# eltoto1219/vltk

Measured on AMD Instinct MI355X. Metric: images/sec FRCNN feature extraction, 800x1333 batch, higher is better.
Workload: dtype f16; 1 GPU; configs[1]: ResNet-101-C4 fp16 (the reference has no FPN: SURVEY.md D1), 32 synthetic 800x1333 images per GPU per step, R=300 RPN proposals through the Res5 head, max 100 detections/img, seeded synthetic weights; global_batch=32, parallelism=image-sharded x1, all-gather of output blocks

## Files before the change

include/vltk_hip.h:

```cpp
#ifndef VLTK_HIP_H
#define VLTK_HIP_H

#include <stddef.h>
#include <stdint.h>

#ifdef __cplusplus
extern "C" {
#endif

#define VK_OK 0
#define VK_EINVAL 1
#define VK_ENOTIMPL 2
#define VK_ENONFINITE 3
#define VK_EWEIGHTS 4
#define VK_EHIP 5
#define VK_ENOMEM 6

typedef enum { VK_F32 = 0, VK_F16 = 1, VK_I64 = 2, VK_I32 = 3, VK_BF16 = 4 } vk_dtype;
typedef enum { VK_ACT_NONE = 0, VK_ACT_RELU = 1, VK_ACT_GELU = 2 , VK_ACT_TANH = 3 } vk_act;

#define VK_MAX_ANCHOR_DIM 8
#define VK_MAX_NMS_THRESH 8

typedef struct vk_config {
    int32_t depth;
    int32_t num_groups;
    int32_t width_per_group;
    int32_t stem_out_channels;
    int32_t res2_out_channels;
    int32_t stride_in_1x1;
    int32_t caffe_maxpool;
    int32_t num_sizes;
    float   sizes[VK_MAX_ANCHOR_DIM];
    int32_t num_ratios;
    float   ratios[VK_MAX_ANCHOR_DIM];
    float   anchor_offset;
    int32_t rpn_hidden_channels;
    float   rpn_min_size;
    double  rpn_nms_thresh;
    int32_t pre_nms_topk;
    int32_t post_nms_topk;
    float   rpn_bbox_weights[4];
    int32_t num_classes;
    int32_t num_attrs;
    int32_t use_attr;
    int32_t pooler_resolution;
    int32_t res5_halve;
    int32_t cls_agnostic_bbox_reg;
    float   roi_bbox_weights[4];
    int32_t precision;
} vk_config;

typedef struct vk_roi_params {
    int32_t num_nms_thresh;
    double  nms_thresh[VK_MAX_NMS_THRESH];
    int32_t min_detections;
    int32_t max_detections;
} vk_roi_params;

#define VK_SELECT_CLASS_MAX 0
#define VK_SELECT_PER_CLASS 1
typedef struct vk_select_params {
    int32_t       mode;
    double        score_thresh;
    vk_roi_params roi;
} vk_select_params;

typedef struct vk_outputs {
    int64_t *obj_ids;
    float   *obj_probs;
    int64_t *attr_ids;
    float   *attr_probs;
    float   *boxes;
    int64_t *preds_per_image;
    float   *roi_features;
} vk_outputs;

#define VK_MAX_IGNOREY 64
typedef struct vk_ignorey {
    const void    *bands;
    const int32_t *counts;
    int32_t        max_per_image;
    int32_t        f64;
} vk_ignorey;

typedef struct vk_handle vk_handle;

const char *vk_last_error(void);
int vk_version(void);

int vk_create(const vk_config *cfg, int device, vk_handle **out);
int vk_load_weights(vk_handle *h, const char *name, const void *host_ptr,
                    const int64_t *shape, int ndim, vk_dtype dtype);
int vk_finalize(vk_handle *h);
int vk_destroy(vk_handle *h);

int vk_set_option(vk_handle *h, const char *key, int value);

int vk_num_weights(vk_handle *h, int *count);
int vk_weight_name(vk_handle *h, int index, const char **name);

int vk_forward(vk_handle *h, const float *images_dev, int N, int H, int W,
               const int32_t *image_hw, const float *scales_yx,
               const vk_roi_params *rp, const vk_outputs *out_dev, void *stream);

int vk_forward_begin(vk_handle *h, const float *images_dev, int N, int H, int W,
                     const int32_t *image_hw, const float *scales_yx,
                     const vk_roi_params *rp, const vk_outputs *out_dev, void *stream, int64_t *ticket);
int vk_forward_end(vk_handle *h, int64_t ticket);
int vk_forward_begin_ignorey(vk_handle *h, const float *images_dev, int N, int H, int W,
                             const int32_t *image_hw, const float *scales_yx,
                             const vk_roi_params *rp, const vk_outputs *out_dev, void *stream, int64_t *ticket,
                             const vk_ignorey *ignorey);
int vk_forward_begin_select(vk_handle *h, const float *images_dev, int N, int H, int W,
                            const int32_t *image_hw, const float *scales_yx,
                            const vk_select_params *sp, const vk_outputs *out_dev, void *stream, int64_t *ticket,
                            const vk_ignorey *ignorey);

int vk_forward_boxes_begin(vk_handle *h, const float *images_dev, int N, int H, int W,
                           const int32_t *image_hw, const float *scales_yx,
                           const float *boxes_dev, int B, const int32_t *counts,
                           const vk_outputs *out_dev, void *stream, int64_t *ticket);

int vk_given_boxes_ingest(const float *boxes_dev, const int32_t *counts_dev, const int32_t *image_hw_dev,
                          const float *scales_yx_dev, int N, int B, float *prop_boxes, float *rois, int32_t *levels,
                          int min_level, int max_level, float canonical_box_size, int canonical_level, int32_t *nonfinite,
                          void *stream);
int vk_given_box_outputs(const float *obj_prob, const int32_t *obj_cls, const float *attr_prob, const int32_t *attr_cls,
                         const float *prop_boxes, const int32_t *counts_dev, const float *scales_yx_dev, const float *feat,
                         int F, int N, int B, const vk_outputs *out_dev, void *stream);

int vk_get_stage(vk_handle *h, const char *name, const void **dev_ptr,
                 vk_dtype *dtype, int64_t *shape, int *ndim);

int vk_memcpy_d2d(void *dst_dev, const void *src_dev, size_t bytes, void *stream);

int vk_enable_stage_timing(vk_handle *h, int enable);
int vk_get_stage_timing(vk_handle *h, float *ms6);

#define VK_NUM_KERNEL_BUCKETS 12
int vk_enable_kernel_timing(vk_handle *h, int enable);
int vk_get_kernel_timing(vk_handle *h, int64_t *launches, double *ms, double *flops, double *bytes, int reset);


size_t vk_packed_weight_bytes(int cout, int cin, int kh, int kw, int groups, vk_dtype dt);
int vk_packed_cout(int cout);
int vk_conv_slice_channels(int cin, int groups);
int vk_pack_conv_weight(const float *w_oihw_host, const float *bn_host, const float *bias_host,
                        int cout, int cin, int kh, int kw, int groups, vk_dtype dt,
                        void *w_packed_host, float *bias_packed_host);

int vk_conv2d(const void *x, int N, int H, int W, int cin,
              const void *w_packed, const float *bias_packed, const void *residual,
              void *y, int cout, int ldy, int kh, int kw, int stride, int pad, int dil, int groups,
              int relu, vk_dtype dt, vk_dtype out_dt, void *stream);

#define VK_ROUTE_GENERIC 0
#define VK_ROUTE_RING 1
#define VK_ROUTE_DUO 2
#define VK_ROUTE_WS 3
#define VK_ROUTE_GEMM4 4
#define VK_ROUTE_PANEL 5
#define VK_ROUTE_BLK 6
int vk_conv_route(int N, int H, int W, int cin, int cin2, int has_residual, int fused_mean, int cout, int ldy, int kh, int kw,
                  int stride, int pad, int dil, int groups, int relu, vk_dtype dt, vk_dtype out_dt);

int vk_conv1x1_dual(const void *x1, int cin1, const void *x2, int cin2, long M,
                    const void *w_packed, const float *bias_packed, const void *residual,
                    void *y, int cout, int relu, void *stream);

int vk_bottleneck64(const void *x, int N, int H, int W, int cin, int proj,
                    const void *w1_packed, const float *b1_packed, const void *w2_packed, const float *b2_packed,
                    const void *w3_packed, const float *b3_packed, void *y, void *stream);

int vk_fuse_shortcut(int cin, int cin_shortcut, int cout, int stride, vk_dtype dt);
int vk_bottleneck64_eligible(int cin, int cmid, int cout, int stride, int dil, int groups, int proj, int fused_shortcut,
                             long N, int H, int W, vk_dtype dt);

size_t vk_conv1x1_meanpool_workspace_bytes(int N, int HW, int cout);
int vk_conv1x1_meanpool(const void *x, int N, int HW, int cin, const void *w_packed, const float *bias_packed,
                        const void *residual, int cout, int relu, float *out_mean,
                        void *workspace, size_t workspace_bytes, void *stream);


int vk_linear(const void *x, long M, int K, const void *w_packed, const float *bias_packed, const void *residual,
              void *y, int N, int ldy, int act, vk_dtype dt, vk_dtype out_dt, void *stream);
int vk_layernorm(const void *x, int ldx, const float *gamma, const float *beta, void *y, int ldy, int M, int C,
                 float eps, float scale, int accumulate, vk_dtype dt, void *stream);
int vk_embed_layernorm(const int64_t *input_ids, const int64_t *token_type_ids, int B, int L, const void *word,
                       const void *position, const void *token_type, const float *gamma, const float *beta,
                       void *y, int C, float eps, vk_dtype dt, void *stream);
int vk_attention(const void *q, int ldq, const void *k, int ldk, const void *v, int ldv, const float *mask,
                 void *out, int ldo, int B, int heads, int Lq, int Lk, int d, vk_dtype dt, void *stream);


int vk_roi_align(const void *const *maps, const int32_t *Hs, const int32_t *Ws, const float *scales, int levels,
                 int N, int C, const float *rois, const int32_t *roi_levels, int K, int P, int sampling_ratio,
                 int aligned, void *out, vk_dtype dt, void *stream);
int vk_assign_levels(const float *boxes, int ld, int K, int min_level, int max_level, float canonical_box_size,
                     int canonical_level, int32_t *levels_out, void *stream);
int vk_upsample2x_add(const void *lateral, const void *top, void *y, int N, int H, int W, int Ht, int Wt, int C,
                      vk_dtype dt, void *stream);
int vk_subsample2(const void *x, void *y, int N, int H, int W, int C, vk_dtype dt, void *stream);
int vk_relu_copy(const void *x, void *y, long n, vk_dtype dt, void *stream);

size_t vk_rpn_multilevel_workspace_bytes(int N, int levels, int pre_topk, int post_topk);
int vk_rpn_proposals_multilevel_ignorey(const float *const *logits, const int32_t *ld_logits, const float *const *deltas,
                                        const int32_t *ld_deltas, int levels, int N, const int32_t *Hs, const int32_t *Ws,
                                        int A, const float *const *cell_anchors, const int32_t *strides, float offset,
                                        const int32_t *image_hw, const float *bbox_weights4_host, float min_size,
                                        double nms_thresh, int pre_topk, int post_topk, float *out_boxes,
                                        float *out_logits, int32_t *out_counts, int32_t *nonfinite_flag, void *workspace,
                                        size_t workspace_bytes, void *stream, const vk_ignorey *ignorey);
int vk_rpn_proposals_ignorey(const float *logits, int ld_logits, const float *deltas, int ld_deltas,
                             int N, int Hf, int Wf, int A, const float *cell_anchors, int stride, float offset,
                             const int32_t *image_hw, const float *bbox_weights4_host, float min_size,
                             double nms_thresh, int pre_topk, int post_topk,
                             float *out_boxes, float *out_logits, int32_t *out_counts, int32_t *nonfinite_flag,
                             void *workspace, size_t workspace_bytes, void *stream, const vk_ignorey *ignorey);
int vk_rpn_proposals_multilevel(const float *const *logits, const int32_t *ld_logits, const float *const *deltas,
                                const int32_t *ld_deltas, int levels, int N, const int32_t *Hs, const int32_t *Ws, int A,
                                const float *const *cell_anchors, const int32_t *strides, float offset,
                                const int32_t *image_hw, const float *bbox_weights4_host, float min_size,
                                double nms_thresh, int pre_topk, int post_topk, float *out_boxes, float *out_logits,
                                int32_t *out_counts, int32_t *nonfinite_flag, void *workspace, size_t workspace_bytes,
                                void *stream);

int vk_nchw_to_nhwc(const float *x, int N, int C, int H, int W, void *y, vk_dtype dt, void *stream);
int vk_nhwc_to_nchw(const void *x, int N, int C, int H, int W, float *y, vk_dtype dt, void *stream);

size_t vk_packed_stem_bytes(int cout, vk_dtype dt);
int vk_pack_stem_weight(const float *w_oihw_host, const float *bn_host, int cout, vk_dtype dt,
                        void *w_packed_host, float *bias_packed_host);
int vk_stem(const float *x, int N, int H, int W, const void *w_packed, const float *bias_packed,
            int cout, int caffe_maxpool, void *y, vk_dtype dt, void *workspace, size_t workspace_bytes,
            void *stream);
size_t vk_stem_workspace_bytes(int N, int H, int W, int cout, vk_dtype dt);
void vk_stem_out_hw(int H, int W, int caffe_maxpool, int *Ho, int *Wo);

int vk_preprocess(const float *const *raw_dev_ptrs_host, const int32_t *raw_hw_host, const int32_t *new_hw_host,
                  int N, int Hmax, int Wmax, const float *mean3_host, const float *std3_host, float pad_value,
                  float *out_nchw_dev, void *stream);

int vk_maxpool3x3s2(const void *x, int N, int H, int W, int C, int caffe, void *y, vk_dtype dt, void *stream);

size_t vk_rpn_workspace_bytes(int N, int HWA, int pre_topk);
int vk_rpn_proposals(const float *logits, int ld_logits, const float *deltas, int ld_deltas,
                     int N, int Hf, int Wf, int A, const float *cell_anchors, int stride, float offset,
                     const int32_t *image_hw, const float *bbox_weights4_host, float min_size,
                     double nms_thresh, int pre_topk, int post_topk,
                     float *out_boxes, float *out_logits, int32_t *out_counts, int32_t *nonfinite_flag,
                     void *workspace, size_t workspace_bytes, void *stream);

int vk_nms(const float *boxes, const float *scores, int n, double thresh,
           int64_t *keep_out, int32_t *count_out, void *workspace, size_t workspace_bytes, void *stream);
size_t vk_nms_workspace_bytes(int n);

int vk_roi_pool(const void *feat, int N, int H, int W, int C, const float *rois, int K,
                float spatial_scale, int P, void *out, vk_dtype dt, void *stream);

int vk_mean_pool(const void *x, int K, int S, int C, float *out, vk_dtype dt, void *stream);

int vk_box_decode(const float *deltas, const float *boxes, int M, int k, const float *weights4_host,
                  float *out, void *stream);

int vk_make_rois(const float *boxes, int N, int R, float *rois, void *stream);
int vk_softmax_argmax(const float *logits, int ld, int K, int n_softmax, int n_argmax, float *prob_out,
                      int32_t *cls_out, int32_t *raw_argmax_out, void *stream);
int vk_concat_embed(const float *features, int F, const void *emb, int E, const int32_t *cls, int K, void *out,
                    vk_dtype dt, void *stream);
int vk_chosen_deltas(const void *x, int ldx, const void *w_rows, const float *bias, const int32_t *cls,
                     int cls_agnostic, int F, int K, float *out, vk_dtype dt, void *stream);

int vk_roi_outputs(const float *obj_logits, int ld_obj, const float *attr_logits, int ld_attr,
                   const float *box_deltas, int ld_box, int chosen_only,
                   const float *proposals, const int32_t *counts, const float *features, int F,
                   int N, int R, int C, int A, const int32_t *image_hw, const float *scales_yx_dev,
                   const float *weights4_host, const vk_roi_params *rp, const vk_outputs *out,
                   int64_t *keep_ids_out, int32_t *nonfinite_flag, void *stream);

int vk_class_boxes(const float *box_deltas, int ld_box, int cls_agnostic, const float *proposals, const int32_t *counts,
                   int N, int R, int C, const int32_t *image_hw, const float *weights4_host, float *out,
                   int32_t *nonfinite_flag, void *stream);
int vk_class_probs(const float *logits, int ld, int K, int n, float *out, int ld_out, void *stream);
int vk_per_class_select(const float *obj_scores, int ld_scores, const float *attr_logits, int ld_attr,
                        const float *box_deltas, int ld_box, int cls_agnostic,
                        const float *proposals, const int32_t *counts, const float *features, int F,
                        int N, int R, int C, int A, const int32_t *image_hw, const float *scales_yx_dev,
                        const float *weights4_host, const vk_select_params *sp, const vk_outputs *out,
                        int64_t *keep_ids_out, float *max_conf_out, int32_t *nonfinite_flag, void *stream);

#ifdef __cplusplus
}
#endif
#endif
```

vltk_amd/_lib.py:

```python
import ctypes as C
import os

_HERE = os.path.dirname(os.path.abspath(__file__))
LIB_PATH = os.path.join(_HERE, "libvltk_hip.so")
if os.environ.get("VLTK_AMD_LIB"):
    LIB_PATH = os.environ["VLTK_AMD_LIB"]
elif os.environ.get("VLTK_AMD_ABLATION_LIB") == "1":
    LIB_PATH = LIB_PATH.replace("libvltk_hip.so", "libvltk_hip_ablation.so")

VK_OK, VK_EINVAL, VK_ENOTIMPL, VK_ENONFINITE, VK_EWEIGHTS, VK_EHIP, VK_ENOMEM = range(7)
VK_F32, VK_F16, VK_I64, VK_I32, VK_BF16 = 0, 1, 2, 3, 4
VK_ACT_NONE, VK_ACT_RELU, VK_ACT_GELU, VK_ACT_TANH = 0, 1, 2, 3
VK_ROUTE_GENERIC, VK_ROUTE_RING, VK_ROUTE_DUO, VK_ROUTE_WS, VK_ROUTE_GEMM4, VK_ROUTE_PANEL, VK_ROUTE_BLK = range(7)
VK_MAX_ANCHOR_DIM = 8
VK_MAX_NMS_THRESH = 8
VK_MAX_IGNOREY = 64
VK_SELECT_CLASS_MAX, VK_SELECT_PER_CLASS = 0, 1

_EXC = {
    VK_EINVAL: ValueError,
    VK_ENOTIMPL: NotImplementedError,
    VK_ENONFINITE: AssertionError,
    VK_EWEIGHTS: OSError,
    VK_EHIP: RuntimeError,
    VK_ENOMEM: MemoryError,
}


class vk_config(C.Structure):
    _fields_ = [
        ("depth", C.c_int32), ("num_groups", C.c_int32), ("width_per_group", C.c_int32),
        ("stem_out_channels", C.c_int32), ("res2_out_channels", C.c_int32),
        ("stride_in_1x1", C.c_int32), ("caffe_maxpool", C.c_int32),
        ("num_sizes", C.c_int32), ("sizes", C.c_float * VK_MAX_ANCHOR_DIM),
        ("num_ratios", C.c_int32), ("ratios", C.c_float * VK_MAX_ANCHOR_DIM),
        ("anchor_offset", C.c_float), ("rpn_hidden_channels", C.c_int32),
        ("rpn_min_size", C.c_float), ("rpn_nms_thresh", C.c_double),
        ("pre_nms_topk", C.c_int32), ("post_nms_topk", C.c_int32),
        ("rpn_bbox_weights", C.c_float * 4),
        ("num_classes", C.c_int32), ("num_attrs", C.c_int32), ("use_attr", C.c_int32),
        ("pooler_resolution", C.c_int32), ("res5_halve", C.c_int32),
        ("cls_agnostic_bbox_reg", C.c_int32), ("roi_bbox_weights", C.c_float * 4),
        ("precision", C.c_int32),
    ]


class vk_roi_params(C.Structure):
    _fields_ = [
        ("num_nms_thresh", C.c_int32), ("nms_thresh", C.c_double * VK_MAX_NMS_THRESH),
        ("min_detections", C.c_int32), ("max_detections", C.c_int32),
    ]


class vk_select_params(C.Structure):
    _fields_ = [("mode", C.c_int32), ("score_thresh", C.c_double), ("roi", vk_roi_params)]


class vk_outputs(C.Structure):
    _fields_ = [
        ("obj_ids", C.c_void_p), ("obj_probs", C.c_void_p), ("attr_ids", C.c_void_p),
        ("attr_probs", C.c_void_p), ("boxes", C.c_void_p), ("preds_per_image", C.c_void_p),
        ("roi_features", C.c_void_p),
    ]


class vk_ignorey(C.Structure):
    _fields_ = [("bands", C.c_void_p), ("counts", C.c_void_p), ("max_per_image", C.c_int32), ("f64", C.c_int32)]


_P, _I, _F, _D, _SZ = C.c_void_p, C.c_int, C.c_float, C.c_double, C.c_size_t

SIGNATURES = {
    "vk_last_error": (C.c_char_p, []),
    "vk_version": (_I, []),
    "vk_create": (_I, [C.POINTER(vk_config), _I, C.POINTER(_P)]),
    "vk_load_weights": (_I, [_P, C.c_char_p, _P, C.POINTER(C.c_int64), _I, _I]),
    "vk_finalize": (_I, [_P]),
    "vk_destroy": (_I, [_P]),
    "vk_set_option": (_I, [_P, C.c_char_p, _I]),
    "vk_num_weights": (_I, [_P, C.POINTER(_I)]),
    "vk_weight_name": (_I, [_P, _I, C.POINTER(C.c_char_p)]),
    "vk_forward": (_I, [_P, _P, _I, _I, _I, _P, _P, C.POINTER(vk_roi_params), C.POINTER(vk_outputs), _P]),
    "vk_forward_begin": (_I, [_P, _P, _I, _I, _I, _P, _P, C.POINTER(vk_roi_params), C.POINTER(vk_outputs), _P,
                              C.POINTER(C.c_int64)]),
    "vk_forward_begin_ignorey": (_I, [_P, _P, _I, _I, _I, _P, _P, C.POINTER(vk_roi_params), C.POINTER(vk_outputs), _P,
                                      C.POINTER(C.c_int64), C.POINTER(vk_ignorey)]),
    "vk_forward_begin_select": (_I, [_P, _P, _I, _I, _I, _P, _P, C.POINTER(vk_select_params), C.POINTER(vk_outputs), _P,
                                     C.POINTER(C.c_int64), C.POINTER(vk_ignorey)]),
    "vk_forward_boxes_begin": (_I, [_P, _P, _I, _I, _I, _P, _P, _P, _I, _P, C.POINTER(vk_outputs), _P, C.POINTER(C.c_int64)]),
    "vk_forward_end": (_I, [_P, C.c_int64]),
    "vk_given_boxes_ingest": (_I, [_P, _P, _P, _P, _I, _I, _P, _P, _P, _I, _I, _F, _I, _P, _P]),
    "vk_given_box_outputs": (_I, [_P, _P, _P, _P, _P, _P, _P, _P, _I, _I, _I, C.POINTER(vk_outputs), _P]),
    "vk_get_stage": (_I, [_P, C.c_char_p, C.POINTER(_P), C.POINTER(_I), C.POINTER(C.c_int64), C.POINTER(_I)]),
    "vk_memcpy_d2d": (_I, [_P, _P, _SZ, _P]),
    "vk_enable_stage_timing": (_I, [_P, _I]),
    "vk_get_stage_timing": (_I, [_P, C.POINTER(_F)]),
    "vk_enable_kernel_timing": (_I, [_P, _I]),
    "vk_get_kernel_timing": (_I, [_P, C.POINTER(C.c_int64), C.POINTER(_D), C.POINTER(_D), C.POINTER(_D), _I]),
    "vk_packed_weight_bytes": (_SZ, [_I, _I, _I, _I, _I, _I]),
    "vk_conv_slice_channels": (_I, [_I, _I]),
    "vk_packed_cout": (_I, [_I]),
    "vk_pack_conv_weight": (_I, [_P, _P, _P, _I, _I, _I, _I, _I, _I, _P, _P]),
    "vk_conv_route": (_I, [_I] * 18),
    "vk_conv1x1_dual": (_I, [_P, _I, _P, _I, C.c_long, _P, _P, _P, _P, _I, _I, _P]),
    "vk_bottleneck64": (_I, [_P, _I, _I, _I, _I, _I, _P, _P, _P, _P, _P, _P, _P, _P]),
    "vk_fuse_shortcut": (_I, [_I, _I, _I, _I, _I]),
    "vk_bottleneck64_eligible": (_I, [_I, _I, _I, _I, _I, _I, _I, _I, C.c_long, _I, _I, _I]),
    "vk_conv1x1_meanpool_workspace_bytes": (_SZ, [_I, _I, _I]),
    "vk_conv1x1_meanpool": (_I, [_P, _I, _I, _I, _P, _P, _P, _I, _I, _P, _P, _SZ, _P]),
    "vk_linear": (_I, [_P, C.c_long, _I, _P, _P, _P, _P, _I, _I, _I, _I, _I, _P]),
    "vk_layernorm": (_I, [_P, _I, _P, _P, _P, _I, _I, _I, _F, _F, _I, _I, _P]),
    "vk_embed_layernorm": (_I, [_P, _P, _I, _I, _P, _P, _P, _P, _P, _P, _I, _F, _I, _P]),
    "vk_attention": (_I, [_P, _I, _P, _I, _P, _I, _P, _P, _I, _I, _I, _I, _I, _I, _I, _P]),
    "vk_roi_align": (_I, [_P, _P, _P, _P, _I, _I, _I, _P, _P, _I, _I, _I, _I, _P, _I, _P]),
    "vk_assign_levels": (_I, [_P, _I, _I, _I, _I, _F, _I, _P, _P]),
    "vk_upsample2x_add": (_I, [_P, _P, _P, _I, _I, _I, _I, _I, _I, _I, _P]),
    "vk_subsample2": (_I, [_P, _P, _I, _I, _I, _I, _I, _P]),
    "vk_relu_copy": (_I, [_P, _P, C.c_long, _I, _P]),
    "vk_rpn_multilevel_workspace_bytes": (_SZ, [_I, _I, _I, _I]),
    "vk_rpn_proposals_multilevel": (_I, [_P, _P, _P, _P, _I, _I, _P, _P, _I, _P, _P, _F, _P, _P, _F, _D, _I, _I, _P, _P, _P, _P, _P, _SZ, _P]),
    "vk_rpn_proposals_multilevel_ignorey": (_I, [_P, _P, _P, _P, _I, _I, _P, _P, _I, _P, _P, _F, _P, _P, _F, _D, _I, _I, _P, _P, _P, _P,
                                                 _P, _SZ, _P, C.POINTER(vk_ignorey)]),
    "vk_conv2d": (_I, [_P, _I, _I, _I, _I, _P, _P, _P, _P, _I, _I, _I, _I, _I, _I, _I, _I, _I, _I, _I, _P]),
    "vk_nchw_to_nhwc": (_I, [_P, _I, _I, _I, _I, _P, _I, _P]),
    "vk_nhwc_to_nchw": (_I, [_P, _I, _I, _I, _I, _P, _I, _P]),
    "vk_packed_stem_bytes": (_SZ, [_I, _I]),
    "vk_pack_stem_weight": (_I, [_P, _P, _I, _I, _P, _P]),
    "vk_stem": (_I, [_P, _I, _I, _I, _P, _P, _I, _I, _P, _I, _P, _SZ, _P]),
    "vk_stem_workspace_bytes": (_SZ, [_I, _I, _I, _I, _I]),
    "vk_stem_out_hw": (None, [_I, _I, _I, C.POINTER(_I), C.POINTER(_I)]),
    "vk_preprocess": (_I, [_P, _P, _P, _I, _I, _I, C.POINTER(_F), C.POINTER(_F), _F, _P, _P]),
    "vk_maxpool3x3s2": (_I, [_P, _I, _I, _I, _I, _I, _P, _I, _P]),
    "vk_rpn_workspace_bytes": (_SZ, [_I, _I, _I]),
    "vk_rpn_proposals": (_I, [_P, _I, _P, _I, _I, _I, _I, _I, _P, _I, _F, _P, C.POINTER(_F), _F, _D, _I, _I,
                              _P, _P, _P, _P, _P, _SZ, _P]),
    "vk_rpn_proposals_ignorey": (_I, [_P, _I, _P, _I, _I, _I, _I, _I, _P, _I, _F, _P, C.POINTER(_F), _F, _D, _I, _I,
                                      _P, _P, _P, _P, _P, _SZ, _P, C.POINTER(vk_ignorey)]),
    "vk_nms": (_I, [_P, _P, _I, _D, _P, _P, _P, _SZ, _P]),
    "vk_nms_workspace_bytes": (_SZ, [_I]),
    "vk_roi_pool": (_I, [_P, _I, _I, _I, _I, _P, _I, _F, _I, _P, _I, _P]),
    "vk_mean_pool": (_I, [_P, _I, _I, _I, _P, _I, _P]),
    "vk_box_decode": (_I, [_P, _P, _I, _I, C.POINTER(_F), _P, _P]),
    "vk_make_rois": (_I, [_P, _I, _I, _P, _P]),
    "vk_softmax_argmax": (_I, [_P, _I, _I, _I, _I, _P, _P, _P, _P]),
    "vk_concat_embed": (_I, [_P, _I, _P, _I, _P, _I, _P, _I, _P]),
    "vk_chosen_deltas": (_I, [_P, _I, _P, _P, _P, _I, _I, _I, _P, _I, _P]),
    "vk_roi_outputs": (_I, [_P, _I, _P, _I, _P, _I, _I, _P, _P, _P, _I, _I, _I, _I, _I, _P, _P, C.POINTER(_F),
                            C.POINTER(vk_roi_params), C.POINTER(vk_outputs), _P, _P, _P]),
    "vk_class_boxes": (_I, [_P, _I, _I, _P, _P, _I, _I, _I, _P, C.POINTER(_F), _P, _P, _P]),
    "vk_class_probs": (_I, [_P, _I, _I, _I, _P, _I, _P]),
    "vk_per_class_select": (_I, [_P, _I, _P, _I, _P, _I, _I, _P, _P, _P, _I, _I, _I, _I, _I, _P, _P, C.POINTER(_F),
                                 C.POINTER(vk_select_params), C.POINTER(vk_outputs), _P, _P, _P, _P]),
}

_lib = None


def load():
    global _lib
    if _lib is None:
        if not os.path.exists(LIB_PATH):
            raise RuntimeError(
                f"{LIB_PATH} not found: build it with `python -c 'import __graft_entry__ as g; g.build()'` "
                "(or `make -C vltk_amd/csrc`).  vltk_amd has no CPU fallback.")
        lib = C.CDLL(LIB_PATH)
        for name, (res, args) in SIGNATURES.items():
            fn = getattr(lib, name)
            fn.restype = res
            fn.argtypes = args
        _lib = lib
    return _lib


def check(status):
    if status != VK_OK:
        msg = load().vk_last_error().decode("utf-8", "replace")
        raise _EXC.get(status, RuntimeError)(msg)


def call(name, *args):
    check(getattr(load(), name)(*args))
```

vltk_amd/csrc/model.hip:

```cpp
#include <cmath>
#include <cstdlib>
#include <map>
#include <mutex>
#include <set>
#include <string>
#include <vector>

#include "vk_common.h"

namespace vk {

thread_local KernelTimer *g_timer = nullptr;

hipEvent_t KernelTimer::get() {
    if (pool.empty()) {
        hipEvent_t e = nullptr;
        (void)hipEventCreate(&e);
        all.push_back(e);
        return e;
    }
    hipEvent_t e = pool.back();
    pool.pop_back();
    return e;
}
void KernelTimer::collect() {
    const char *logp = getenv("VK_CONV_LOG");
    FILE *lf = logp ? fopen(logp, "a") : nullptr;
    std::vector<Rec> pending;
    for (auto &r : recs) {
        float t = 0.f;
        if (hipEventQuery(r.e1) != hipSuccess) {
            pending.push_back(r);
            continue;
        }
        if (hipEventElapsedTime(&t, r.e0, r.e1) == hipSuccess) {
            if (lf) fprintf(lf, "%d %d %d %d %d %d %.5f %.1f\n", r.bucket, r.M, r.cout, r.cin, r.k, r.stride, t, r.flops / (t * 1e-3) / 1e12);
            launches[r.bucket] += 1;
            ms[r.bucket] += t;
            flops[r.bucket] += r.flops;
            bytes[r.bucket] += r.bytes;
        }
        pool.push_back(r.e0);
        pool.push_back(r.e1);
    }
    if (lf) fclose(lf);
    recs.swap(pending);
    (void)hipGetLastError();
}
KernelTimer::~KernelTimer() {
    for (auto e : all) (void)hipEventDestroy(e);
}

int Timed::begin(hipStream_t stream) {
    if (!tm) return VK_OK;
    e0 = tm->get();
    e1 = tm->get();
    VK_CHECK_HIP(hipEventRecord(e0, stream));
    return VK_OK;
}
int Timed::end(hipStream_t stream, int bucket, double flops, int M, int cout, int cin, int k, int stride, double bytes) {
    if (!tm) return VK_OK;
    VK_CHECK_HIP(hipEventRecord(e1, stream));
    tm->recs.push_back({bucket, flops, e0, e1, M, cout, cin, k, stride, bytes});
    return VK_OK;
}

static std::atomic<DeviceState *> g_devices[VK_MAX_DEVICES];
static std::mutex g_devices_mu;

int device_state(DeviceState **out) {
    int dev = 0;
    VK_CHECK_HIP(hipGetDevice(&dev));
    VK_REQUIRE(dev >= 0 && dev < VK_MAX_DEVICES, VK_EINVAL, "device %d beyond VK_MAX_DEVICES", dev);
    DeviceState *d = g_devices[dev].load(std::memory_order_acquire);
    if (!d) {
        std::lock_guard<std::mutex> lock(g_devices_mu);
        d = g_devices[dev].load(std::memory_order_relaxed);
        if (!d) {
            hipDeviceProp_t prop;
            VK_CHECK_HIP(hipGetDeviceProperties(&prop, dev));
            char *p = nullptr;
            VK_CHECK_HIP(hipMalloc((void **)&p, 256 + 256 * sizeof(unsigned) + BN_TRASH_BYTES));
            VK_CHECK_HIP(hipMemset(p, 0, 256 + 256 * sizeof(unsigned)));
            d = new DeviceState;
            d->n_cu = prop.multiProcessorCount;
            d->zero_page = p;
            d->tile_ring = (unsigned *)(p + 256);
            d->bn_trash = p + 256 + 256 * sizeof(unsigned);
            d->tile_next = 0;
            g_devices[dev].store(d, std::memory_order_release);
        }
    }
    *out = d;
    return VK_OK;
}

static std::set<std::pair<int, const void *>> g_lds_set;
static std::mutex g_lds_mu;

int set_max_lds(const void *kernel, size_t bytes) {
    int dev = 0;
    VK_CHECK_HIP(hipGetDevice(&dev));
    std::lock_guard<std::mutex> lock(g_lds_mu);
    if (g_lds_set.count({dev, kernel})) return VK_OK;
    VK_CHECK_HIP(hipFuncSetAttribute(kernel, hipFuncAttributeMaxDynamicSharedMemorySize, (int)bytes));
    g_lds_set.insert({dev, kernel});
    return VK_OK;
}

static thread_local char g_err[1024] = "";
void set_error(const char *fmt, ...) {
    va_list ap;
    va_start(ap, fmt);
    vsnprintf(g_err, sizeof(g_err), fmt, ap);
    va_end(ap);
}

struct HostTensor {
    std::vector<int64_t> shape;
    std::vector<float> data;
    bool loaded = false;
};

struct ConvLayer {
    std::string prefix;
    int cin = 0, cout = 0, k = 1, stride = 1, pad = 0, dil = 1;
    bool bn = true, relu = false;
    void *w = nullptr;
    float *b = nullptr;
    int groups = 1;
    int dt = -1;
};

struct Block {
    ConvLayer conv1, conv2, conv3, shortcut;
    bool has_shortcut = false;
    bool fused_shortcut = false;
};

static const int kBlocks[3][4] = {{3, 4, 6, 3}, {3, 4, 23, 3}, {3, 8, 36, 3}};

}

using namespace vk;

struct vk_handle {
    vk_config cfg;
    int device = 0;
    vk_dtype dt = VK_F16;
    vk_dtype pdt = VK_F32;
    bool finalized = false;
    std::vector<std::string> names;
    std::map<std::string, HostTensor> host;

    ConvLayer stem;
    std::vector<Block> stages[3];
    std::vector<Block> res5;
    ConvLayer rpn_conv, rpn_heads;
    ConvLayer cls_score, fc_attr, attr_score;
    void *bbox_w = nullptr;
    float *bbox_b = nullptr;
    void *emb = nullptr;
    float *cell_anchors = nullptr;
    int A = 0, res4_c = 0, res5_c = 0, hid = 0, emb_dim = 0;
    std::vector<void *> owned;

    char *arena = nullptr;
    size_t arena_bytes = 0;
    char *pc_arena = nullptr;
    size_t pc_arena_bytes = 0;
    const void *bbox_lin_w = nullptr;
    const float *bbox_lin_b = nullptr;
    int head_chunk = 9600;
    int backbone_streams = 2;
    int backbone_split_min_batch = 8;
    int head_streams = 1;
    int head_split_min_rois = 512;

    struct Stage {
        const void *ptr;
        vk_dtype dt;
        int64_t shape[4];
        int ndim;
    };
    std::map<std::string, Stage> stages_out;
    KernelTimer *ktimer = nullptr;
    bool timing = false;
    hipEvent_t ev[6] = {nullptr, nullptr, nullptr, nullptr, nullptr, nullptr};
    hipStream_t side = nullptr;
    hipEvent_t ev_fork = nullptr, ev_join = nullptr;
    hipStream_t more_sides[2] = {nullptr, nullptr};
    hipEvent_t more_joins[2] = {nullptr, nullptr};
    bool ev_valid = false;
    static constexpr int VK_MAX_INFLIGHT = 4;
    int32_t *flag_host = nullptr;
    char *meta_host = nullptr;
    size_t meta_cap = 0;
    hipEvent_t ev_done[VK_MAX_INFLIGHT] = {nullptr, nullptr, nullptr, nullptr};
    int64_t next_ticket = 0, oldest_open = 0;
};

namespace vk {

static void add_conv_names(std::vector<std::string> &n, const std::string &p, bool bn) {
    n.push_back(p + ".weight");
    if (bn) {
        n.push_back(p + ".norm.weight");
        n.push_back(p + ".norm.bias");
        n.push_back(p + ".norm.running_mean");
        n.push_back(p + ".norm.running_var");
    } else {
        n.push_back(p + ".bias");
    }
}

static Block make_block(const std::string &p, int cin, int cmid, int cout, int stride, int dil, bool stride_in_1x1,
                        int groups, std::vector<std::string> &names) {
    Block b;
    const int s1 = stride_in_1x1 ? stride : 1, s3 = stride_in_1x1 ? 1 : stride;
    b.has_shortcut = cin != cout;
    if (b.has_shortcut) {
        b.shortcut = ConvLayer{p + ".shortcut", cin, cout, 1, stride, 0, 1, true, false};
        add_conv_names(names, b.shortcut.prefix, true);
    }
    b.conv1 = ConvLayer{p + ".conv1", cin, cmid, 1, s1, 0, 1, true, true};
    b.conv2 = ConvLayer{p + ".conv2", cmid, cmid, 3, s3, dil, dil, true, true};
    b.conv2.groups = groups;
    b.conv3 = ConvLayer{p + ".conv3", cmid, cout, 1, 1, 0, 1, true, true};
    add_conv_names(names, b.conv1.prefix, true);
    add_conv_names(names, b.conv2.prefix, true);
    add_conv_names(names, b.conv3.prefix, true);
    return b;
}

static int dev_alloc(vk_handle *h, size_t bytes, void **out) {
    void *p = nullptr;
    VK_CHECK_HIP(hipMalloc(&p, bytes ? bytes : 16));
    h->owned.push_back(p);
    *out = p;
    return VK_OK;
}

static int upload(vk_handle *h, const void *host, size_t bytes, void **out) {
    VK_TRY(dev_alloc(h, bytes, out));
    VK_CHECK_HIP(hipMemcpy(*out, host, bytes, hipMemcpyHostToDevice));
    return VK_OK;
}

static const HostTensor *get_t(vk_handle *h, const std::string &name, std::vector<int64_t> shape) {
    auto it = h->host.find(name);
    if (it == h->host.end() || !it->second.loaded) {
        set_error("missing weight '%s' (strict load)", name.c_str());
        return nullptr;
    }
    if (it->second.shape != shape) {
        std::string got, want;
        for (auto v : it->second.shape) got += std::to_string(v) + ",";
        for (auto v : shape) want += std::to_string(v) + ",";
        set_error("weight '%s' has shape [%s], expected [%s]", name.c_str(), got.c_str(), want.c_str());
        return nullptr;
    }
    return &it->second;
}

static int finalize_conv(vk_handle *h, ConvLayer &L) {
    const HostTensor *w = get_t(h, L.prefix + ".weight", {L.cout, L.cin / L.groups, L.k, L.k});
    if (!w) return VK_EWEIGHTS;
    std::vector<float> bn;
    const float *bnp = nullptr, *bias = nullptr;
    if (L.bn) {
        const char *parts[4] = {".norm.weight", ".norm.bias", ".norm.running_mean", ".norm.running_var"};
        bn.resize(4 * (size_t)L.cout);
        for (int i = 0; i < 4; ++i) {
            const HostTensor *t = get_t(h, L.prefix + parts[i], {L.cout});
            if (!t) return VK_EWEIGHTS;
            memcpy(bn.data() + (size_t)i * L.cout, t->data.data(), sizeof(float) * L.cout);
        }
        bnp = bn.data();
    } else {
        const HostTensor *t = get_t(h, L.prefix + ".bias", {L.cout});
        if (!t) return VK_EWEIGHTS;
        bias = t->data.data();
    }
    const vk_dtype ldt = L.dt >= 0 ? (vk_dtype)L.dt : h->dt;
    const size_t wb = vk_packed_weight_bytes(L.cout, L.cin, L.k, L.k, L.groups, ldt);
    std::vector<char> packed(wb);
    std::vector<float> pb(vk_packed_cout(L.cout));
    VK_TRY(vk_pack_conv_weight(w->data.data(), bnp, bias, L.cout, L.cin, L.k, L.k, L.groups, ldt, packed.data(), pb.data()));
    VK_TRY(upload(h, packed.data(), wb, &L.w));
    VK_TRY(upload(h, pb.data(), pb.size() * sizeof(float), (void **)&L.b));
    return VK_OK;
}

static int pack_conv_host(vk_handle *h, const ConvLayer &L, std::vector<char> &packed, std::vector<float> &pb) {
    const HostTensor *w = get_t(h, L.prefix + ".weight", {L.cout, L.cin / L.groups, L.k, L.k});
    if (!w) return VK_EWEIGHTS;
    std::vector<float> bn(4 * (size_t)L.cout);
    const char *parts[4] = {".norm.weight", ".norm.bias", ".norm.running_mean", ".norm.running_var"};
    for (int i = 0; i < 4; ++i) {
        const HostTensor *t = get_t(h, L.prefix + parts[i], {L.cout});
        if (!t) return VK_EWEIGHTS;
        memcpy(bn.data() + (size_t)i * L.cout, t->data.data(), sizeof(float) * L.cout);
    }
    packed.resize(vk_packed_weight_bytes(L.cout, L.cin, L.k, L.k, L.groups, h->dt));
    pb.resize(vk_packed_cout(L.cout));
    return vk_pack_conv_weight(w->data.data(), bn.data(), nullptr, L.cout, L.cin, L.k, L.k, L.groups, h->dt, packed.data(), pb.data());
}

static int finalize_block(vk_handle *h, Block &b) {
    VK_TRY(finalize_conv(h, b.conv1));
    VK_TRY(finalize_conv(h, b.conv2));
    b.fused_shortcut = b.has_shortcut && vk_fuse_shortcut(b.conv3.cin, b.shortcut.cin, b.conv3.cout, b.shortcut.stride, h->dt);
    if (!b.fused_shortcut) {
        if (b.has_shortcut) VK_TRY(finalize_conv(h, b.shortcut));
        return finalize_conv(h, b.conv3);
    }
    std::vector<char> w3, wsc;
    std::vector<float> b3, bsc;
    VK_TRY(pack_conv_host(h, b.conv3, w3, b3));
    VK_TRY(pack_conv_host(h, b.shortcut, wsc, bsc));
    const size_t r3 = (size_t)b.conv3.cin * 2, rsc = (size_t)b.shortcut.cin * 2, rows = b3.size();
    std::vector<char> cat(rows * (r3 + rsc));
    for (size_t r = 0; r < rows; ++r) {
        memcpy(cat.data() + r * (r3 + rsc), w3.data() + r * r3, r3);
        memcpy(cat.data() + r * (r3 + rsc) + r3, wsc.data() + r * rsc, rsc);
        b3[r] += bsc[r];
    }
    VK_TRY(upload(h, cat.data(), cat.size(), &b.conv3.w));
    VK_TRY(upload(h, b3.data(), b3.size() * sizeof(float), (void **)&b.conv3.b));
    return VK_OK;
}

static void to_dt(const float *src, size_t n, vk_dtype dt, void *dst) {
    if (dt == VK_F16) {
        _Float16 *d = (_Float16 *)dst;
        for (size_t i = 0; i < n; ++i) d[i] = (_Float16)src[i];
    } else if (dt == VK_BF16) {
        uint16_t *d = (uint16_t *)dst;
        for (size_t i = 0; i < n; ++i) {
            uint32_t u;
            memcpy(&u, &src[i], 4);
            if ((u & 0x7fffffffu) > 0x7f800000u)
                d[i] = (uint16_t)((u >> 16) | 0x40);
            else
                d[i] = (uint16_t)((u + 0x7fffu + ((u >> 16) & 1u)) >> 16);
        }
    } else {
        memcpy(dst, src, n * sizeof(float));
    }
}

static bool fused_mean_ok(const vk_handle *h, int P, size_t rows) {
    static const bool off = getenv("VK_NO_FUSED_MEAN") != nullptr;
    const long mid5 = (long)h->cfg.num_groups * h->cfg.width_per_group * 8;
    return !off && h->dt == VK_F16 && h->cfg.res5_halve == 0 && P * P >= 128 && P * P <= 255 && h->res5_c % 256 == 0 &&
           (long)rows * mid5 * 2 < (1L << 32);
}

struct Carver {
    char *base;
    size_t off = 0;
    explicit Carver(char *b) : base(b) {}
    void *take(size_t bytes) {
        void *p = base ? base + off : nullptr;
        off += align_up(bytes ? bytes : 16, 256);
        return p;
    }
};

struct Plan {
    int N, H, W, Hp, Wp, H1, W1, Hs[3], Ws[3], Hf, Wf, R, K, P, chunk;
    void *img_pad, *stem_out, *bufA, *bufB, *bufSC, *bufT1, *bufT2;
    void *rpn_hid;
    float *rpn_out, *prop_boxes, *prop_logits, *rois;
    int32_t *prop_counts, *image_hw, *nonfinite;
    float *scales;
    void *bands;
    int32_t *band_counts;
    void *rpn_ws;
    size_t rpn_ws_bytes;
    void *pooled, *h_t1, *h_t2, *h_a, *h_b, *h_sc;
    float *pool_part;
    float *feat;
    void *featT, *concat, *attr_hid;
    float *cls_logits, *attr_logits, *obj_prob, *attr_prob, *chosen;
    int32_t *obj_cls, *attr_cls, *max_class;
    int64_t *keep_ids;
    size_t total;
};

static void conv_out_hw(int H, int W, int k, int s, int p, int d, int *Ho, int *Wo) {
    *Ho = (H + 2 * p - (d * (k - 1) + 1)) / s + 1;
    *Wo = (W + 2 * p - (d * (k - 1) + 1)) / s + 1;
}

static Plan make_plan(vk_handle *h, char *base, int N, int H, int W, int D, int R) {
    Plan p;
    memset(&p, 0, sizeof(p));
    const vk_config &c = h->cfg;
    const size_t es = dtype_size(h->dt);
    p.N = N;
    p.H = H;
    p.W = W;
    conv_out_hw(H, W, 7, 2, 3, 1, &p.H1, &p.W1);
    p.Hp = std::max(H + 6, 2 * p.H1 + 6);
    p.Wp = std::max(W + 6, 2 * p.W1 + 6);
    p.Wp = (p.Wp + 1) & ~1;
    int h2, w2;
    vk_stem_out_hw(H, W, c.caffe_maxpool, &h2, &w2);
    p.Hs[0] = h2;
    p.Ws[0] = w2;
    for (int s = 1; s < 3; ++s) conv_out_hw(p.Hs[s - 1], p.Ws[s - 1], 1, 2, 0, 1, &p.Hs[s], &p.Ws[s]);
    p.Hf = p.Hs[2];
    p.Wf = p.Ws[2];
    p.R = R;
    p.K = N * p.R;
    p.P = c.pooler_resolution;
    p.chunk = std::min(h->head_chunk > 0 ? h->head_chunk : p.K, p.K);

    Carver cv(base);
    p.img_pad = cv.take((size_t)N * p.Hp * p.Wp * 4 * es);
    p.stem_out = cv.take((size_t)N * p.H1 * p.W1 * c.stem_out_channels * es);
    size_t max_out = 0, max_mid = 0;
    int cout = c.res2_out_channels, cmid = c.num_groups * c.width_per_group;
    for (int s = 0; s < 3; ++s) {
        const size_t px_out = (size_t)N * p.Hs[s] * p.Ws[s];
        const size_t px_in = s == 0 ? px_out : (size_t)N * p.Hs[s - 1] * p.Ws[s - 1];
        max_out = std::max(max_out, px_out * cout * es);
        max_mid = std::max(max_mid, (c.stride_in_1x1 ? px_out : px_in) * cmid * es);
        cout *= 2;
        cmid *= 2;
    }
    p.bufA = cv.take(max_out);
    p.bufB = cv.take(max_out);
    p.bufSC = cv.take(max_out);
    p.bufT1 = cv.take(max_mid);
    p.bufT2 = cv.take(max_mid);
    const size_t Mf = (size_t)N * p.Hf * p.Wf;
    p.rpn_hid = cv.take(Mf * h->hid * es);
    p.rpn_out = (float *)cv.take(Mf * (size_t)((5 * h->A + 7) / 8 * 8) * sizeof(float));
    p.prop_boxes = (float *)cv.take((size_t)p.K * 4 * sizeof(float));
    p.prop_logits = (float *)cv.take((size_t)p.K * sizeof(float));
    p.rois = (float *)cv.take((size_t)p.K * 5 * sizeof(float));
    p.prop_counts = (int32_t *)cv.take((size_t)N * sizeof(int32_t));
    p.image_hw = (int32_t *)cv.take((size_t)N * 2 * sizeof(int32_t));
    p.scales = (float *)cv.take((size_t)N * 2 * sizeof(float));
    p.nonfinite = (int32_t *)cv.take(sizeof(int32_t));
    p.rpn_ws_bytes = vk_rpn_workspace_bytes(N, p.Hf * p.Wf * h->A, c.pre_nms_topk);
    p.rpn_ws = cv.take(p.rpn_ws_bytes);
    const size_t rows = (size_t)p.chunk * p.P * p.P;
    const int mid5 = c.num_groups * c.width_per_group * 8;
    p.pooled = cv.take(rows * h->res4_c * es);
    p.h_t1 = cv.take(rows * mid5 * es);
    p.h_t2 = cv.take(rows * mid5 * es);
    p.h_a = cv.take(rows * h->res5_c * es);
    p.h_b = cv.take(rows * h->res5_c * es);
    p.h_sc = cv.take(rows * h->res5_c * es);
    p.pool_part = nullptr;
    if (fused_mean_ok(h, p.P, rows)) p.pool_part = (float *)cv.take(conv_duo_pool_part_bytes((long)rows + 128, h->res5_c));
    p.feat = (float *)cv.take((size_t)p.K * h->res5_c * sizeof(float));
    const size_t pes = dtype_size(h->pdt);
    p.featT = cv.take((size_t)p.K * h->res5_c * pes);
    p.concat = cv.take((size_t)p.K * (h->res5_c + h->emb_dim) * pes);
    p.attr_hid = cv.take((size_t)p.K * (h->res5_c / 4) * pes);
    p.cls_logits = (float *)cv.take((size_t)p.K * ((c.num_classes + 1 + 7) / 8 * 8) * sizeof(float));
    p.attr_logits = (float *)cv.take((size_t)p.K * ((c.num_attrs + 1 + 7) / 8 * 8) * sizeof(float));
    p.obj_prob = (float *)cv.take((size_t)p.K * sizeof(float));
    p.attr_prob = (float *)cv.take((size_t)p.K * sizeof(float));
    p.chosen = (float *)cv.take((size_t)p.K * 4 * sizeof(float));
    p.obj_cls = (int32_t *)cv.take((size_t)p.K * sizeof(int32_t));
    p.attr_cls = (int32_t *)cv.take((size_t)p.K * sizeof(int32_t));
    p.max_class = (int32_t *)cv.take((size_t)p.K * sizeof(int32_t));
    p.keep_ids = (int64_t *)cv.take((size_t)N * D * sizeof(int64_t));
    p.bands = cv.take((size_t)N * VK_MAX_IGNOREY * 2 * sizeof(double));
    p.band_counts = (int32_t *)cv.take((size_t)N * sizeof(int32_t));
    p.total = cv.off;
    return p;
}

static int run_conv(vk_handle *h, const ConvLayer &L, const void *x, int N, int H, int W, const void *res, void *y,
                    bool relu, vk_dtype out_dt, int ldy, hipStream_t s, int *Ho = nullptr, int *Wo = nullptr,
                    const void *x2 = nullptr, int cin2 = 0, float *pool_part = nullptr, bool concurrent = false) {
    ConvArgs a;
    memset(&a, 0, sizeof(a));
    a.concurrent = concurrent ? 1 : 0;
    a.x = x;
    a.x2 = x2;
    a.Cin2 = cin2;
    a.pool_part = pool_part;
    a.w = L.w;
    a.bias = L.b;
    a.res = res;
    a.y = y;
    a.N = N;
    a.H = H;
    a.W = W;
    a.Cin = L.cin;
    conv_out_hw(H, W, L.k, L.stride, L.pad, L.dil, &a.Ho, &a.Wo);
    a.Cout = L.cout;
    a.ldy = ldy > 0 ? ldy : (L.cout + 7) / 8 * 8;
    a.kh = a.kw = L.k;
    a.stride = L.stride;
    a.pad = L.pad;
    a.dil = L.dil;
    a.groups = L.groups;
    a.relu = relu;
    a.stem = 0;
    a.dt = L.dt >= 0 ? (vk_dtype)L.dt : h->dt;
    a.out_dt = out_dt;
    if (Ho) *Ho = a.Ho;
    if (Wo) *Wo = a.Wo;
    return launch_conv(a, s);
}

static int run_block(vk_handle *h, const Block &b, const void *x, int N, int H, int W, void *t1, void *t2, void *sc,
                     void *y, hipStream_t s, int *Ho, int *Wo, float *pool_part = nullptr, int n0 = 0, int nb = -1) {
    int h1, w1, h2, w2;
    const bool cc = nb >= 0;
    if (nb >= 0) {
        const size_t es = dtype_size(h->dt);
        int ho, wo;
        conv_out_hw(H, W, b.conv1.k, b.conv1.stride, b.conv1.pad, b.conv1.dil, &h1, &w1);
        conv_out_hw(h1, w1, b.conv2.k, b.conv2.stride, b.conv2.pad, b.conv2.dil, &h2, &w2);
        conv_out_hw(h2, w2, 1, 1, 0, 1, &ho, &wo);
        x = (const char *)x + (size_t)n0 * H * W * b.conv1.cin * es;
        t1 = (char *)t1 + (size_t)n0 * h1 * w1 * b.conv1.cout * es;
        t2 = (char *)t2 + (size_t)n0 * h2 * w2 * b.conv2.cout * es;
        sc = (char *)sc + (size_t)n0 * ho * wo * b.conv3.cout * es;
        y = (char *)y + (size_t)n0 * ho * wo * b.conv3.cout * es;
        N = nb;
    }
    if (!pool_part && vk_bottleneck64_eligible(b.conv1.cin, b.conv1.cout, b.conv3.cout, b.conv1.stride * b.conv2.stride, b.conv2.dil,
                                               b.conv2.groups, b.has_shortcut, b.fused_shortcut, N, H, W, h->dt)) {
        if (Ho) *Ho = H;
        if (Wo) *Wo = W;
        return launch_bneck_fused(x, N, H, W, b.conv1.cin, b.has_shortcut, b.conv1.w, b.conv1.b, b.conv2.w, b.conv2.b, b.conv3.w, b.conv3.b, y,
                                  cc, s);
    }
    const void *res = x;
    if (b.has_shortcut && !b.fused_shortcut) {
        VK_TRY(run_conv(h, b.shortcut, x, N, H, W, nullptr, sc, false, h->dt, 0, s, nullptr, nullptr, nullptr, 0, nullptr, cc));
        res = sc;
    }
    VK_TRY(run_conv(h, b.conv1, x, N, H, W, nullptr, t1, true, h->dt, 0, s, &h1, &w1, nullptr, 0, nullptr, cc));
    VK_TRY(run_conv(h, b.conv2, t1, N, h1, w1, nullptr, t2, true, h->dt, 0, s, &h2, &w2, nullptr, 0, nullptr, cc));
    if (b.fused_shortcut)
        return run_conv(h, b.conv3, t2, N, h2, w2, nullptr, y, true, h->dt, 0, s, Ho, Wo, x, b.shortcut.cin, pool_part, cc);
    VK_TRY(run_conv(h, b.conv3, t2, N, h2, w2, res, y, true, h->dt, 0, s, Ho, Wo, nullptr, 0, pool_part, cc));
    return VK_OK;
}

static void set_stage(vk_handle *h, const char *name, const void *ptr, vk_dtype dt, std::initializer_list<int64_t> shape) {
    vk_handle::Stage st;
    st.ptr = ptr;
    st.dt = dt;
    st.ndim = 0;
    for (auto v : shape) st.shape[st.ndim++] = v;
    h->stages_out[name] = st;
}

}

extern "C" {

const char *vk_last_error(void) { return g_err; }
int vk_version(void) { return 1; }

int vk_packed_cout(int cout) { return (cout + CONV_COUT_ALIGN - 1) / CONV_COUT_ALIGN * CONV_COUT_ALIGN; }

int vk_conv_slice_channels(int cin, int groups) {
    if (groups <= 1) return cin;
    if (cin <= 0 || cin % groups != 0) return -1;
    const int cpg = cin / groups;
    if (cpg & (cpg - 1)) return -1;
    return std::min(std::max(cpg, 64), cin);
}

size_t vk_packed_weight_bytes(int cout, int cin, int kh, int kw, int groups, vk_dtype dt) {
    const int sw = vk_conv_slice_channels(cin, groups);
    return sw <= 0 ? 0 : (size_t)vk_packed_cout(cout) * kh * kw * sw * dtype_size(dt);
}

int vk_pack_conv_weight(const float *w, const float *bn, const float *bias, int cout, int cin, int kh, int kw, int groups,
                        vk_dtype dt, void *w_packed, float *bias_packed) {
    VK_REQUIRE(dt == VK_F16 || dt == VK_F32 || dt == VK_BF16, VK_EINVAL, "pack: dtype must be f16, bf16 or f32");
    VK_REQUIRE(groups >= 1, VK_EINVAL, "pack: groups=%d", groups);
    const int sw = vk_conv_slice_channels(cin, groups);
    VK_REQUIRE(sw > 0, VK_EINVAL, "pack: cin=%d / groups=%d must be a power of two", cin, groups);
    VK_REQUIRE(groups == 1 || cin == cout, VK_EINVAL, "pack: grouped convolution needs cin == cout (got %d, %d)", cin, cout);
    VK_REQUIRE((sw * (int)dtype_size(dt)) % CONV_KTILE_BYTES == 0, VK_EINVAL,
               "pack: %d channels per tap is not a whole number of 128-byte K-tiles for this dtype", sw);
    const int cp = vk_packed_cout(cout);
    const int cpg = cin / groups;
    const size_t K = (size_t)kh * kw * sw;
    std::vector<float> row(K);
    for (int co = 0; co < cp; ++co) {
        double s = 1.0;
        float b = 0.f;
        std::fill(row.begin(), row.end(), 0.f);
        if (co < cout) {
            if (bn) {
                const double g = bn[co], be = bn[cout + co], mu = bn[2 * (size_t)cout + co], var = bn[3 * (size_t)cout + co];
                s = g / std::sqrt(var + 1e-5);
                b = (float)(be - mu * s);
            } else if (bias) {
                b = bias[co];
            }
            const int slice0 = groups == 1 ? 0 : (co / 64 * 64) / sw * sw;
            const int g0 = groups == 1 ? 0 : co / cpg * cpg;
            for (int c = 0; c < cpg; ++c)
                for (int y = 0; y < kh; ++y)
                    for (int x = 0; x < kw; ++x)
                        row[((size_t)y * kw + x) * sw + (g0 + c - slice0)] =
                            (float)((double)w[(((size_t)co * cpg + c) * kh + y) * kw + x] * s);
        }
        bias_packed[co] = b;
        to_dt(row.data(), K, dt, (char *)w_packed + (size_t)co * K * dtype_size(dt));
    }
    return VK_OK;
}

size_t vk_packed_stem_bytes(int cout, vk_dtype dt) {
    const int ktiles = dt == VK_F16 ? 4 : 7;
    return (size_t)vk_packed_cout(cout) * ktiles * CONV_KTILE_BYTES;
}

int vk_pack_stem_weight(const float *w, const float *bn, int cout, vk_dtype dt, void *w_packed, float *bias_packed) {
    VK_REQUIRE(dt == VK_F16 || dt == VK_F32, VK_EINVAL, "pack_stem: dtype must be f16 or f32");
    const int cp = vk_packed_cout(cout);
    const int ktiles = dt == VK_F16 ? 4 : 7;
    const size_t K = (size_t)ktiles * CONV_KTILE_BYTES / dtype_size(dt);
    std::vector<float> row(K);
    for (int co = 0; co < cp; ++co) {
        std::fill(row.begin(), row.end(), 0.f);
        float b = 0.f;
        if (co < cout) {
            double s = 1.0;
            if (bn) {
                const double g = bn[co], be = bn[cout + co], mu = bn[2 * (size_t)cout + co], var = bn[3 * (size_t)cout + co];
                s = g / std::sqrt(var + 1e-5);
                b = (float)(be - mu * s);
            }
            for (int c = 0; c < 3; ++c)
                for (int y = 0; y < 7; ++y)
                    for (int x = 0; x < 7; ++x)
                        row[(size_t)y * 32 + x * 4 + c] = (float)((double)w[(((size_t)co * 3 + c) * 7 + y) * 7 + x] * s);
        }
        bias_packed[co] = b;
        to_dt(row.data(), K, dt, (char *)w_packed + (size_t)co * K * dtype_size(dt));
    }
    return VK_OK;
}

static void fill_conv_args(ConvArgs &a, int N, int H, int W, int cin, int cout, int ldy, int k, int stride, int pad, int dil, int groups,
                           int relu, vk_dtype dt, vk_dtype out_dt) {
    memset(&a, 0, sizeof(a));
    a.N = N;
    a.H = H;
    a.W = W;
    a.Cin = cin;
    conv_out_hw(H, W, k, stride, pad, dil, &a.Ho, &a.Wo);
    a.Cout = cout;
    a.ldy = ldy;
    a.kh = a.kw = k;
    a.stride = stride;
    a.pad = pad;
    a.dil = dil;
    a.groups = groups;
    a.relu = relu;
    a.dt = dt;
    a.out_dt = out_dt;
}

int vk_conv2d(const void *x, int N, int H, int W, int cin, const void *w_packed, const float *bias_packed,
              const void *residual, void *y, int cout, int ldy, int kh, int kw, int stride, int pad, int dil, int groups,
              int relu, vk_dtype dt, vk_dtype out_dt, void *stream) {
    VK_REQUIRE(kh == kw && kh >= 1 && stride >= 1 && dil >= 1 && pad >= 0 && groups >= 1, VK_EINVAL, "conv2d: bad geometry");
    ConvArgs a;
    fill_conv_args(a, N, H, W, cin, cout, ldy, kh, stride, pad, dil, groups, relu, dt, out_dt);
    VK_REQUIRE(a.Ho > 0 && a.Wo > 0 && N > 0, VK_EINVAL, "conv2d: empty output");
    a.x = x;
    a.w = w_packed;
    a.bias = bias_packed;
    a.res = residual;
    a.y = y;
    return launch_conv(a, (hipStream_t)stream);
}

int vk_conv_route(int N, int H, int W, int cin, int cin2, int has_residual, int fused_mean, int cout, int ldy, int kh, int kw,
                  int stride, int pad, int dil, int groups, int relu, vk_dtype dt, vk_dtype out_dt) {
    if (!(kh == kw && kh >= 1 && stride >= 1 && dil >= 1 && pad >= 0 && groups >= 1 && cin2 >= 0)) {
        set_error("conv_route: bad geometry");
        return -VK_EINVAL;
    }
    static const char here = 0;
    ConvArgs a;
    fill_conv_args(a, N, H, W, cin, cout, ldy, kh, stride, pad, dil, groups, relu, dt, out_dt);
    if (!(a.Ho > 0 && a.Wo > 0 && N > 0)) {
        set_error("conv_route: empty output");
        return -VK_EINVAL;
    }
    a.x = a.w = &here;
    a.res = has_residual ? &here : nullptr;
    a.x2 = cin2 > 0 ? &here : nullptr;
    a.Cin2 = cin2;
    a.pool_part = fused_mean ? (float *)&here : nullptr;
    return conv_route_checked(a);
}

int vk_conv1x1_dual(const void *x1, int cin1, const void *x2, int cin2, long M, const void *w_packed, const float *bias_packed,
                    const void *residual, void *y, int cout, int relu, void *stream) {
    VK_REQUIRE(x1 && x2 && M > 0 && M < (1L << 31), VK_EINVAL, "conv1x1_dual: bad arguments");
    ConvArgs a;
    fill_conv_args(a, 1, 1, (int)M, cin1, cout, cout, 1, 1, 0, 1, 1, relu, VK_F16, VK_F16);
    a.x = x1;
    a.x2 = x2;
    a.Cin2 = cin2;
    a.w = w_packed;
    a.bias = bias_packed;
    a.res = residual;
    a.y = y;
    return launch_conv(a, (hipStream_t)stream);
}

int vk_linear(const void *x, long M, int K, const void *w_packed, const float *bias_packed, const void *residual, void *y, int N, int ldy,
              int act, vk_dtype dt, vk_dtype out_dt, void *stream) {
    VK_REQUIRE(x && w_packed && bias_packed && y && M > 0 && M < (1L << 31), VK_EINVAL, "linear: bad arguments");
    ConvArgs a;
    fill_conv_args(a, 1, 1, (int)M, K, N, ldy, 1, 1, 0, 1, 1, act, dt, out_dt);
    a.x = x;
    a.w = w_packed;
    a.bias = bias_packed;
    a.res = residual;
    a.y = y;
    return launch_conv(a, (hipStream_t)stream);
}

int vk_fuse_shortcut(int cin, int cin_shortcut, int cout, int stride, vk_dtype dt) {
    static const bool off = getenv("VK_NO_FUSED_SHORTCUT") != nullptr;
    return !off && dt == VK_F16 && stride == 1 && cout % 256 == 0 && cin % 32 == 0 && cin_shortcut % 32 == 0;
}

int vk_bottleneck64_eligible(int cin, int cmid, int cout, int stride, int dil, int groups, int proj, int fused_shortcut, long N,
                             int H, int W, vk_dtype dt) {
    return stride == 1 && dil == 1 && (!proj || fused_shortcut) &&
           bneck_fused_eligible(cin, cmid, cout, stride, groups, proj != 0, N, H, W, dt);
}

int vk_bottleneck64(const void *x, int N, int H, int W, int cin, int proj, const void *w1, const float *b1, const void *w2,
                    const float *b2, const void *w3, const float *b3, void *y, void *stream) {
    VK_REQUIRE(x && w1 && b1 && w2 && b2 && w3 && b3 && y && N > 0 && H > 0 && W > 0, VK_EINVAL, "bottleneck64: bad arguments");
    VK_REQUIRE((cin == 256 && !proj) || (cin == 64 && proj), VK_EINVAL, "bottleneck64: cin must be 256 (identity) or 64 (projection)");
    VK_REQUIRE(bneck_fused_eligible(cin, 64, 256, 1, 1, proj != 0, N, H, W, VK_F16) || getenv("VK_BNECK_FUSED"), VK_EINVAL,
               "bottleneck64: tensor beyond the 32-bit byte offsets");
    VK_REQUIRE((long)N * H * W * 512 < (1L << 32) - (1L << 20), VK_EINVAL, "bottleneck64: tensor beyond the 32-bit byte offsets");
    return launch_bneck_fused(x, N, H, W, cin, proj != 0, w1, b1, w2, b2, w3, b3, y, false, (hipStream_t)stream);
}

size_t vk_conv1x1_meanpool_workspace_bytes(int N, int HW, int cout) { return conv_duo_pool_part_bytes((long)N * HW, cout); }

int vk_conv1x1_meanpool(const void *x, int N, int HW, int cin, const void *w_packed, const float *bias_packed,
                        const void *residual, int cout, int relu, float *out_mean, void *workspace, size_t workspace_bytes,
                        void *stream) {
    VK_REQUIRE(x && out_mean && workspace && N > 0 && HW > 0, VK_EINVAL, "conv1x1_meanpool: bad arguments");
    VK_REQUIRE(workspace_bytes >= vk_conv1x1_meanpool_workspace_bytes(N, HW, cout), VK_EINVAL, "conv1x1_meanpool: workspace too small");
    ConvArgs a;
    fill_conv_args(a, N, 1, HW, cin, cout, cout, 1, 1, 0, 1, 1, relu, VK_F16, VK_F16);
    a.x = x;
    a.w = w_packed;
    a.bias = bias_packed;
    a.res = residual;
    a.pool_part = (float *)workspace;
    VK_TRY(launch_conv(a, (hipStream_t)stream));
    return launch_pool_finish((const float *)workspace, N, HW, cin, cout, false, out_mean, (hipStream_t)stream);
}

static void stem_geom(int H, int W, int *H1, int *W1, int *Hp, int *Wp) {
    conv_out_hw(H, W, 7, 2, 3, 1, H1, W1);
    *Hp = std::max(H + 6, 2 * *H1 + 6);
    *Wp = (std::max(W + 6, 2 * *W1 + 6) + 1) & ~1;
}

size_t vk_stem_workspace_bytes(int N, int H, int W, int cout, vk_dtype dt) {
    int H1, W1, Hp, Wp;
    stem_geom(H, W, &H1, &W1, &Hp, &Wp);
    return align_up((size_t)N * Hp * Wp * 4 * dtype_size(dt), 256) + align_up((size_t)N * H1 * W1 * cout * dtype_size(dt), 256);
}

static int stem_impl(const float *x, int N, int H, int W, const void *w, const float *b, int cout, int caffe, void *y,
                     vk_dtype dt, void *img_pad, void *stem_out, hipStream_t s, int32_t *nonfinite = nullptr) {
    int H1, W1, Hp, Wp;
    stem_geom(H, W, &H1, &W1, &Hp, &Wp);
    VK_TRY(launch_stem_pack(x, img_pad, N, H, W, Hp, Wp, dt, s, nonfinite));
    if (stem_pool_eligible(cout, dt)) return launch_stem_pool(img_pad, N, Hp, Wp, H1, W1, w, b, caffe, y, s);
    ConvArgs a;
    memset(&a, 0, sizeof(a));
    a.x = img_pad;
    a.w = w;
    a.bias = b;
    a.y = stem_out;
    a.N = N;
    a.H = Hp;
    a.W = Wp;
    a.Cin = 4;
    a.Ho = H1;
    a.Wo = W1;
    a.Cout = cout;
    a.ldy = (cout + 7) / 8 * 8;
    a.kh = a.kw = 7;
    a.stride = 2;
    a.pad = 0;
    a.dil = 1;
    a.relu = 1;
    a.stem = 1;
    a.dt = a.out_dt = dt;
    VK_TRY(launch_conv(a, s));
    return launch_maxpool(stem_out, y, N, H1, W1, cout, caffe, dt, s);
}

int vk_stem(const float *x, int N, int H, int W, const void *w_packed, const float *bias_packed, int cout,
            int caffe_maxpool, void *y, vk_dtype dt, void *workspace, size_t workspace_bytes, void *stream) {
    VK_REQUIRE(dt == VK_F16 || dt == VK_F32, VK_EINVAL, "stem: bad dtype");
    VK_REQUIRE(cout % 8 == 0, VK_EINVAL, "stem: cout must be a multiple of 8");
    VK_REQUIRE(H >= 16 && W >= 16, VK_EINVAL, "stem: image %dx%d too small", H, W);
    VK_REQUIRE(workspace && workspace_bytes >= vk_stem_workspace_bytes(N, H, W, cout, dt), VK_EINVAL, "stem: workspace too small");
    int H1, W1, Hp, Wp;
    stem_geom(H, W, &H1, &W1, &Hp, &Wp);
    char *img_pad = (char *)workspace;
    char *stem_out = img_pad + align_up((size_t)N * Hp * Wp * 4 * dtype_size(dt), 256);
    return stem_impl(x, N, H, W, w_packed, bias_packed, cout, caffe_maxpool, y, dt, img_pad, stem_out, (hipStream_t)stream);
}

int vk_create(const vk_config *cfg, int device, vk_handle **out) {
    VK_REQUIRE(cfg && out, VK_EINVAL, "create: null argument");
    VK_REQUIRE(cfg->depth == 50 || cfg->depth == 101 || cfg->depth == 152, VK_EINVAL, "create: depth %d unsupported", cfg->depth);
    VK_REQUIRE(cfg->num_groups >= 1 && cfg->width_per_group >= 1 &&
                   (cfg->num_groups == 1 || (cfg->width_per_group & (cfg->width_per_group - 1)) == 0),
               VK_EINVAL, "create: NUM_GROUPS=%d needs WIDTH_PER_GROUP (%d) to be a power of two", cfg->num_groups, cfg->width_per_group);
    VK_REQUIRE(cfg->stride_in_1x1 != 0 || cfg->res5_halve != 0, VK_EINVAL,
               "create: STRIDE_IN_1X1=false with RES5HALVE=false leaves a stride-2 conv2 in res5 (frcnn.py:1351-1355): "
               "the reference's residual add fails on the shapes");
    VK_REQUIRE(cfg->precision == VK_F16 || cfg->precision == VK_F32, VK_EINVAL, "create: precision must be VK_F16 or VK_F32");
    VK_REQUIRE(cfg->num_sizes >= 1 && cfg->num_sizes <= VK_MAX_ANCHOR_DIM && cfg->num_ratios >= 1 &&
                   cfg->num_ratios <= VK_MAX_ANCHOR_DIM, VK_EINVAL, "create: bad anchor configuration");
    VK_REQUIRE(cfg->pre_nms_topk >= 1 && cfg->pre_nms_topk <= 8192, VK_EINVAL, "create: PRE_NMS_TOPK_TEST must be in 1..8192");
    VK_REQUIRE(cfg->post_nms_topk >= 1 && cfg->post_nms_topk <= 1024 && cfg->post_nms_topk <= cfg->pre_nms_topk, VK_EINVAL,
               "create: POST_NMS_TOPK_TEST must be in 1..min(1024, PRE_NMS_TOPK_TEST)");
    VK_REQUIRE(cfg->use_attr != 0, VK_EINVAL, "create: ROI_BOX_HEAD.ATTR=false is not supported");
    VK_REQUIRE(cfg->stem_out_channels == 64, VK_EINVAL, "create: STEM_OUT_CHANNELS must be 64");
    VK_CHECK_HIP(hipSetDevice(device));
    vk_handle *h = new vk_handle();
    h->cfg = *cfg;
    h->device = device;
    h->dt = (vk_dtype)cfg->precision;
    if (getenv("VK_PREDICTOR_FP16")) h->pdt = h->dt;
    const char *env = getenv("VK_HEAD_CHUNK");
    if (env && atoi(env) > 0) h->head_chunk = atoi(env);
    if (const char *bs = getenv("VK_BACKBONE_STREAMS"))
        if (bs[0] >= '1' && bs[0] <= '4') h->backbone_streams = bs[0] - '0';
    if (const char *hs = getenv("VK_HEAD_STREAMS"))
        if (hs[0] == '1' || hs[0] == '2') h->head_streams = hs[0] - '0';
    const int di = cfg->depth == 50 ? 0 : (cfg->depth == 101 ? 1 : 2);
    add_conv_names(h->names, "backbone.stem.conv1", true);
    h->stem = ConvLayer{"backbone.stem.conv1", 3, cfg->stem_out_channels, 7, 2, 3, 1, true, true};
    int cin = cfg->stem_out_channels, cout = cfg->res2_out_channels, cmid = cfg->num_groups * cfg->width_per_group;
    const char *sn[3] = {"res2", "res3", "res4"};
    for (int s = 0; s < 3; ++s) {
        for (int b = 0; b < kBlocks[di][s]; ++b) {
            const int stride = (b == 0 && s > 0) ? 2 : 1;
            h->stages[s].push_back(make_block(std::string("backbone.") + sn[s] + "." + std::to_string(b), cin, cmid, cout,
                                              stride, 1, cfg->stride_in_1x1 != 0, cfg->num_groups, h->names));
            cin = cout;
        }
        cout *= 2;
        cmid *= 2;
    }
    h->res4_c = cin;
    h->A = cfg->num_sizes * cfg->num_ratios;
    h->names.push_back("proposal_generator.anchor_generator.cell_anchors.0");
    h->hid = cfg->rpn_hidden_channels == -1 ? h->res4_c : cfg->rpn_hidden_channels;
    h->rpn_conv = ConvLayer{"proposal_generator.rpn_head.conv", h->res4_c, h->hid, 3, 1, 1, 1, false, true};
    add_conv_names(h->names, h->rpn_conv.prefix, false);
    add_conv_names(h->names, "proposal_generator.rpn_head.objectness_logits", false);
    add_conv_names(h->names, "proposal_generator.rpn_head.anchor_deltas", false);
    h->rpn_heads = ConvLayer{"proposal_generator.rpn_head.(objectness_logits|anchor_deltas)", h->hid, 5 * h->A, 1, 1, 0, 1, false, false};
    h->res5_c = cfg->res2_out_channels * 8;
    const int mid5 = cfg->num_groups * cfg->width_per_group * 8;
    cin = h->res4_c;
    for (int b = 0; b < 3; ++b) {
        const bool halve = cfg->res5_halve != 0;
        h->res5.push_back(make_block("roi_heads.res5." + std::to_string(b), cin, mid5, h->res5_c, (halve && b == 0) ? 2 : 1,
                                     halve ? 1 : 2, cfg->stride_in_1x1 != 0, cfg->num_groups, h->names));
        cin = h->res5_c;
    }
    const int C = cfg->num_classes, F = h->res5_c;
    h->emb_dim = F / 8;
    const std::string bp = "roi_heads.box_predictor.";
    h->cls_score = ConvLayer{bp + "cls_score", F, C + 1, 1, 1, 0, 1, false, false};
    h->fc_attr = ConvLayer{bp + "fc_attr", F + h->emb_dim, F / 4, 1, 1, 0, 1, false, true};
    h->attr_score = ConvLayer{bp + "attr_score", F / 4, cfg->num_attrs + 1, 1, 1, 0, 1, false, false};
    for (const char *n : {"cls_score", "bbox_pred"}) add_conv_names(h->names, bp + n, false);
    h->names.push_back(bp + "cls_embedding.weight");
    for (const char *n : {"fc_attr", "attr_score"}) add_conv_names(h->names, bp + n, false);
    *out = h;
    return VK_OK;
}

int vk_num_weights(vk_handle *h, int *count) {
    VK_REQUIRE(h && count, VK_EINVAL, "null argument");
    *count = (int)h->names.size();
    return VK_OK;
}

int vk_weight_name(vk_handle *h, int index, const char **name) {
    VK_REQUIRE(h && name && index >= 0 && index < (int)h->names.size(), VK_EINVAL, "weight index out of range");
    *name = h->names[index].c_str();
    return VK_OK;
}

int vk_load_weights(vk_handle *h, const char *name, const void *host_ptr, const int64_t *shape, int ndim, vk_dtype dtype) {
    VK_REQUIRE(h && name && host_ptr && (shape || ndim == 0), VK_EINVAL, "load_weights: null argument");
    VK_REQUIRE(!h->finalized, VK_EINVAL, "load_weights: model already finalized");
    std::string key(name);
    size_t pos;
    if ((pos = key.find("gamma")) != std::string::npos) key.replace(pos, 5, "weight");
    if ((pos = key.find("beta")) != std::string::npos) key.replace(pos, 4, "bias");
    if (key.size() > 19 && key.compare(key.size() - 19, 19, "num_batches_tracked") == 0) return VK_OK;
    bool known = false;
    for (auto &n : h->names) known |= (n == key);
    VK_REQUIRE(known, VK_EWEIGHTS, "unexpected key '%s' in state_dict (strict load)", key.c_str());
    VK_REQUIRE(dtype == VK_F32, VK_EINVAL, "load_weights: '%s' must be float32", key.c_str());
    HostTensor t;
    size_t n = 1;
    for (int i = 0; i < ndim; ++i) {
        t.shape.push_back(shape[i]);
        n *= (size_t)shape[i];
    }
    t.data.assign((const float *)host_ptr, (const float *)host_ptr + n);
    t.loaded = true;
    h->host[key] = std::move(t);
    return VK_OK;
}

int vk_finalize(vk_handle *h) {
    VK_REQUIRE(h, VK_EINVAL, "finalize: null handle");
    VK_REQUIRE(!h->finalized, VK_EINVAL, "finalize: already finalized");
    VK_CHECK_HIP(hipSetDevice(h->device));
    for (auto &n : h->names) {
        auto it = h->host.find(n);
        VK_REQUIRE(it != h->host.end() && it->second.loaded, VK_EWEIGHTS, "missing key '%s' in state_dict (strict load)", n.c_str());
    }
    const vk_config &c = h->cfg;
    {
        const HostTensor *w = get_t(h, "backbone.stem.conv1.weight", {c.stem_out_channels, 3, 7, 7});
        if (!w) return VK_EWEIGHTS;
        std::vector<float> bn(4 * (size_t)c.stem_out_channels);
        const char *parts[4] = {".norm.weight", ".norm.bias", ".norm.running_mean", ".norm.running_var"};
        for (int i = 0; i < 4; ++i) {
            const HostTensor *t = get_t(h, std::string("backbone.stem.conv1") + parts[i], {c.stem_out_channels});
            if (!t) return VK_EWEIGHTS;
            memcpy(bn.data() + (size_t)i * c.stem_out_channels, t->data.data(), sizeof(float) * c.stem_out_channels);
        }
        std::vector<char> packed(vk_packed_stem_bytes(c.stem_out_channels, h->dt));
        std::vector<float> pb(vk_packed_cout(c.stem_out_channels));
        VK_TRY(vk_pack_stem_weight(w->data.data(), bn.data(), c.stem_out_channels, h->dt, packed.data(), pb.data()));
        VK_TRY(upload(h, packed.data(), packed.size(), &h->stem.w));
        VK_TRY(upload(h, pb.data(), pb.size() * sizeof(float), (void **)&h->stem.b));
    }
    for (int s = 0; s < 3; ++s)
        for (auto &b : h->stages[s]) VK_TRY(finalize_block(h, b));
    for (auto &b : h->res5) VK_TRY(finalize_block(h, b));
    VK_TRY(finalize_conv(h, h->rpn_conv));
    {
        const int A = h->A, hid = h->hid;
        const HostTensor *wo = get_t(h, "proposal_generator.rpn_head.objectness_logits.weight", {A, hid, 1, 1});
        const HostTensor *bo = get_t(h, "proposal_generator.rpn_head.objectness_logits.bias", {A});
        const HostTensor *wd = get_t(h, "proposal_generator.rpn_head.anchor_deltas.weight", {4 * A, hid, 1, 1});
        const HostTensor *bd = get_t(h, "proposal_generator.rpn_head.anchor_deltas.bias", {4 * A});
        if (!wo || !bo || !wd || !bd) return VK_EWEIGHTS;
        std::vector<float> w(wo->data), b(bo->data);
        w.insert(w.end(), wd->data.begin(), wd->data.end());
        b.insert(b.end(), bd->data.begin(), bd->data.end());
        std::vector<char> packed(vk_packed_weight_bytes(5 * A, hid, 1, 1, 1, h->dt));
        std::vector<float> pb(vk_packed_cout(5 * A));
        VK_TRY(vk_pack_conv_weight(w.data(), nullptr, b.data(), 5 * A, hid, 1, 1, 1, h->dt, packed.data(), pb.data()));
        VK_TRY(upload(h, packed.data(), packed.size(), &h->rpn_heads.w));
        VK_TRY(upload(h, pb.data(), pb.size() * sizeof(float), (void **)&h->rpn_heads.b));
        const HostTensor *ca = get_t(h, "proposal_generator.anchor_generator.cell_anchors.0", {A, 4});
        if (!ca) return VK_EWEIGHTS;
        VK_TRY(upload(h, ca->data.data(), ca->data.size() * sizeof(float), (void **)&h->cell_anchors));
    }
    const std::string bp = "roi_heads.box_predictor.";
    for (ConvLayer *L : {&h->cls_score, &h->fc_attr, &h->attr_score}) {
        auto it = h->host.find(L->prefix + ".weight");
        if (it != h->host.end() && it->second.shape.size() == 2) {
            it->second.shape.push_back(1);
            it->second.shape.push_back(1);
        }
        L->dt = h->pdt;
        VK_TRY(finalize_conv(h, *L));
    }
    {
        const int C = c.num_classes, F = h->res5_c;
        const int nb = c.cls_agnostic_bbox_reg ? 1 : C;
        const HostTensor *w = get_t(h, bp + "bbox_pred.weight", {4 * nb, F});
        const HostTensor *b = get_t(h, bp + "bbox_pred.bias", {4 * nb});
        const HostTensor *e = get_t(h, bp + "cls_embedding.weight", {C + 1, h->emb_dim});
        if (!w || !b || !e) return VK_EWEIGHTS;
        std::vector<char> tmp(w->data.size() * dtype_size(h->pdt));
        to_dt(w->data.data(), w->data.size(), h->pdt, tmp.data());
        VK_TRY(upload(h, tmp.data(), tmp.size(), &h->bbox_w));
        VK_TRY(upload(h, b->data.data(), b->data.size() * sizeof(float), (void **)&h->bbox_b));
        tmp.resize(e->data.size() * dtype_size(h->pdt));
        to_dt(e->data.data(), e->data.size(), h->pdt, tmp.data());
        VK_TRY(upload(h, tmp.data(), tmp.size(), &h->emb));
    }
    h->host.clear();
    h->finalized = true;
    return VK_OK;
}

int vk_set_option(vk_handle *h, const char *key, int value) {
    VK_REQUIRE(h && key, VK_EINVAL, "set_option: null argument");
    if (!strcmp(key, "head_chunk")) {
        VK_REQUIRE(value >= 0, VK_EINVAL, "head_chunk must be >= 0 (0 = all RoIs at once)");
        h->head_chunk = value;
        return VK_OK;
    }
    if (!strcmp(key, "backbone_streams")) {
        VK_REQUIRE(value >= 1 && value <= 4, VK_EINVAL, "backbone_streams must be 1..4");
        h->backbone_streams = value;
        return VK_OK;
    }
    if (!strcmp(key, "head_streams")) {
        VK_REQUIRE(value == 1 || value == 2, VK_EINVAL, "head_streams must be 1 or 2");
        h->head_streams = value;
        return VK_OK;
    }
    if (!strcmp(key, "head_split_min_rois")) {
        VK_REQUIRE(value >= 2, VK_EINVAL, "head_split_min_rois must be >= 2");
        h->head_split_min_rois = value;
        return VK_OK;
    }
    if (!strcmp(key, "backbone_split_min_batch")) {
        VK_REQUIRE(value >= 2, VK_EINVAL, "backbone_split_min_batch must be >= 2");
        h->backbone_split_min_batch = value;
        return VK_OK;
    }
    VK_REQUIRE(false, VK_EINVAL, "unknown option '%s'", key);
}

int vk_destroy(vk_handle *h) {
    if (!h) return VK_OK;
    (void)hipSetDevice(h->device);
    (void)hipDeviceSynchronize();
    for (void *p : h->owned) (void)hipFree(p);
    if (h->arena) (void)hipFree(h->arena);
    if (h->pc_arena) (void)hipFree(h->pc_arena);
    for (auto &e : h->ev)
        if (e) (void)hipEventDestroy(e);
    for (auto &e : h->ev_done)
        if (e) (void)hipEventDestroy(e);
    if (h->flag_host) (void)hipHostFree(h->flag_host);
    if (h->meta_host) (void)hipHostFree(h->meta_host);
    if (h->ev_fork) (void)hipEventDestroy(h->ev_fork);
    if (h->ev_join) (void)hipEventDestroy(h->ev_join);
    if (h->side) (void)hipStreamDestroy(h->side);
    for (int i = 0; i < 2; ++i) {
        if (h->more_joins[i]) (void)hipEventDestroy(h->more_joins[i]);
        if (h->more_sides[i]) (void)hipStreamDestroy(h->more_sides[i]);
    }
    delete h->ktimer;
    delete h;
    return VK_OK;
}

int vk_enable_stage_timing(vk_handle *h, int enable) {
    VK_REQUIRE(h, VK_EINVAL, "null handle");
    h->timing = enable != 0;
    if (h->timing && !h->ev[0])
        for (auto &e : h->ev) VK_CHECK_HIP(hipEventCreate(&e));
    return VK_OK;
}

int vk_get_stage_timing(vk_handle *h, float *ms6) {
    VK_REQUIRE(h && ms6, VK_EINVAL, "null argument");
    VK_REQUIRE(h->timing && h->ev_valid, VK_EINVAL, "stage timing was not recorded");
    VK_CHECK_HIP(hipEventSynchronize(h->ev[5]));
    for (int i = 0; i < 5; ++i) VK_CHECK_HIP(hipEventElapsedTime(&ms6[i], h->ev[i], h->ev[i + 1]));
    VK_CHECK_HIP(hipEventElapsedTime(&ms6[5], h->ev[0], h->ev[5]));
    return VK_OK;
}

int vk_memcpy_d2d(void *dst_dev, const void *src_dev, size_t bytes, void *stream) {
    VK_REQUIRE(dst_dev && src_dev, VK_EINVAL, "memcpy_d2d: null pointer");
    VK_CHECK_HIP(hipMemcpyAsync(dst_dev, src_dev, bytes, hipMemcpyDeviceToDevice, (hipStream_t)stream));
    return VK_OK;
}

int vk_get_stage(vk_handle *h, const char *name, const void **dev_ptr, vk_dtype *dtype, int64_t *shape, int *ndim) {
    VK_REQUIRE(h && name && dev_ptr && dtype && shape && ndim, VK_EINVAL, "null argument");
    auto it = h->stages_out.find(name);
    VK_REQUIRE(it != h->stages_out.end(), VK_EINVAL, "unknown stage '%s' (or no forward has run)", name);
    *dev_ptr = it->second.ptr;
    *dtype = it->second.dt;
    *ndim = it->second.ndim;
    for (int i = 0; i < it->second.ndim; ++i) shape[i] = it->second.shape[i];
    return VK_OK;
}

int vk_forward(vk_handle *h, const float *images_dev, int N, int H, int W, const int32_t *image_hw,
               const float *scales_yx, const vk_roi_params *rp, const vk_outputs *out, void *stream) {
    int64_t ticket = -1;
    VK_TRY(vk_forward_begin(h, images_dev, N, H, W, image_hw, scales_yx, rp, out, stream, &ticket));
    return vk_forward_end(h, ticket);
}

}

namespace vk {


static int fwd_open(vk_handle *h, int N, int H, int W, int R, int D, const int32_t *image_hw, const float *scales_yx,
                    const int32_t *counts, const vk_ignorey *ig, hipStream_t s, Plan *out) {
    Plan need = make_plan(h, nullptr, N, H, W, D, R);
    if (need.total > h->arena_bytes) {
        if (h->arena) {
            VK_CHECK_HIP(hipDeviceSynchronize());
            VK_CHECK_HIP(hipFree(h->arena));
            h->arena = nullptr;
            h->arena_bytes = 0;
        }
        VK_CHECK_HIP(hipMalloc((void **)&h->arena, need.total));
        h->arena_bytes = need.total;
    }
    Plan &p = *out;
    p = make_plan(h, h->arena, N, H, W, D, R);
    h->stages_out.clear();
    if (h->timing) VK_CHECK_HIP(hipEventRecord(h->ev[0], s));

    const size_t hw_bytes = sizeof(int32_t) * 2 * (size_t)N, sc_bytes = sizeof(float) * 2 * (size_t)N;
    const size_t cnt_bytes = sizeof(int32_t) * (size_t)N;
    const size_t band_off = align_up(hw_bytes + sc_bytes + 2 * cnt_bytes, 8);
    const size_t band_bytes = ig ? (size_t)N * ig->max_per_image * 2 * (ig->f64 ? sizeof(double) : sizeof(float)) : 0;
    const size_t meta_need = ig ? band_off + band_bytes : hw_bytes + sc_bytes + cnt_bytes;
    if (meta_need > h->meta_cap) {
        VK_CHECK_HIP(hipDeviceSynchronize());
        if (h->meta_host) VK_CHECK_HIP(hipHostFree(h->meta_host));
        h->meta_host = nullptr;
        h->meta_cap = align_up(meta_need, 4096);
        VK_CHECK_HIP(hipHostMalloc((void **)&h->meta_host, h->meta_cap * vk_handle::VK_MAX_INFLIGHT, hipHostMallocDefault));
    }
    char *meta = h->meta_host + (size_t)(h->next_ticket % vk_handle::VK_MAX_INFLIGHT) * h->meta_cap;
    memcpy(meta, image_hw, hw_bytes);
    VK_CHECK_HIP(hipMemcpyAsync(p.image_hw, meta, hw_bytes, hipMemcpyHostToDevice, s));
    if (scales_yx) {
        memcpy(meta + hw_bytes, scales_yx, sc_bytes);
        VK_CHECK_HIP(hipMemcpyAsync(p.scales, meta + hw_bytes, sc_bytes, hipMemcpyHostToDevice, s));
    }
    if (counts) {
        memcpy(meta + hw_bytes + sc_bytes, counts, sizeof(int32_t) * (size_t)N);
        VK_CHECK_HIP(hipMemcpyAsync(p.prop_counts, meta + hw_bytes + sc_bytes, sizeof(int32_t) * (size_t)N, hipMemcpyHostToDevice, s));
    }
    if (ig) {
        memcpy(meta + hw_bytes + sc_bytes + cnt_bytes, ig->counts, cnt_bytes);
        VK_CHECK_HIP(hipMemcpyAsync(p.band_counts, meta + hw_bytes + sc_bytes + cnt_bytes, cnt_bytes, hipMemcpyHostToDevice, s));
        memcpy(meta + band_off, ig->bands, band_bytes);
        VK_CHECK_HIP(hipMemcpyAsync(p.bands, meta + band_off, band_bytes, hipMemcpyHostToDevice, s));
    }
    VK_CHECK_HIP(hipMemsetAsync(p.nonfinite, 0, sizeof(int32_t), s));
    return VK_OK;
}

static int fwd_backbone(vk_handle *h, const Plan &p, const float *images_dev, hipStream_t s, const void **res4_out) {
    const vk_config &c = h->cfg;
    const int N = p.N;
    VK_TRY(stem_impl(images_dev, N, p.H, p.W, h->stem.w, h->stem.b, c.stem_out_channels, c.caffe_maxpool, p.bufA, h->dt,
                     p.img_pad, p.stem_out, s, p.nonfinite));
    void *cur = p.bufA, *nxt = p.bufB;
    int ch = p.Hs[0], cw = p.Ws[0];
    for (int st = 0; st < 3; ++st) {
        const bool split = h->backbone_streams >= 2 && st >= 1 && N >= h->backbone_streams && N >= h->backbone_split_min_batch && h->dt == VK_F16;
        const int ns = split ? h->backbone_streams : 1;
        hipStream_t gs_[4] = {s, nullptr, nullptr, nullptr};
        hipEvent_t gj_[4] = {nullptr, nullptr, nullptr, nullptr};
        if (split) {
            if (!h->side) {
                VK_CHECK_HIP(hipStreamCreateWithFlags(&h->side, hipStreamNonBlocking));
                VK_CHECK_HIP(hipEventCreateWithFlags(&h->ev_fork, hipEventDisableTiming));
                VK_CHECK_HIP(hipEventCreateWithFlags(&h->ev_join, hipEventDisableTiming));
            }
            for (int i = 0; i < ns - 2; ++i)
                if (!h->more_sides[i]) {
                    VK_CHECK_HIP(hipStreamCreateWithFlags(&h->more_sides[i], hipStreamNonBlocking));
                    VK_CHECK_HIP(hipEventCreateWithFlags(&h->more_joins[i], hipEventDisableTiming));
                }
            gs_[1] = h->side;
            gj_[1] = h->ev_join;
            for (int i = 2; i < ns; ++i) {
                gs_[i] = h->more_sides[i - 2];
                gj_[i] = h->more_joins[i - 2];
            }
            VK_CHECK_HIP(hipEventRecord(h->ev_fork, s));
            for (int i = 1; i < ns; ++i) VK_CHECK_HIP(hipStreamWaitEvent(gs_[i], h->ev_fork, 0));
        }
        for (auto &b : h->stages[st]) {
            int ho, wo;
            if (split) {
                for (int i = 0; i < ns; ++i) {
                    const int n0 = (int)((long)N * i / ns), n1 = (int)((long)N * (i + 1) / ns);
                    VK_TRY(run_block(h, b, cur, N, ch, cw, p.bufT1, p.bufT2, p.bufSC, nxt, gs_[i], &ho, &wo, nullptr, n0, n1 - n0));
                }
            } else {
                VK_TRY(run_block(h, b, cur, N, ch, cw, p.bufT1, p.bufT2, p.bufSC, nxt, s, &ho, &wo));
            }
            std::swap(cur, nxt);
            ch = ho;
            cw = wo;
        }
        if (split) {
            for (int i = 1; i < ns; ++i) {
                VK_CHECK_HIP(hipEventRecord(gj_[i], gs_[i]));
                VK_CHECK_HIP(hipStreamWaitEvent(s, gj_[i], 0));
            }
        }
    }
    VK_REQUIRE(ch == p.Hf && cw == p.Wf, VK_EINVAL, "internal: res4 geometry mismatch (%dx%d vs %dx%d)", ch, cw, p.Hf, p.Wf);
    *res4_out = cur;
    set_stage(h, "res4", cur, h->dt, {N, p.Hf, p.Wf, h->res4_c});
    if (h->timing) VK_CHECK_HIP(hipEventRecord(h->ev[1], s));
    return VK_OK;
}

static int fwd_head(vk_handle *h, const Plan &p, const void *res4, hipStream_t s) {
    const vk_config &c = h->cfg;
    const int N = p.N, P = p.P;
    auto ensure_side = [&]() -> int {
        if (!h->side) {
            VK_CHECK_HIP(hipStreamCreateWithFlags(&h->side, hipStreamNonBlocking));
            VK_CHECK_HIP(hipEventCreateWithFlags(&h->ev_fork, hipEventDisableTiming));
            VK_CHECK_HIP(hipEventCreateWithFlags(&h->ev_join, hipEventDisableTiming));
        }
        return VK_OK;
    };
    const size_t es5 = dtype_size(h->dt);
    for (int k0 = 0; k0 < p.K; k0 += p.chunk) {
        const int kc = std::min(p.chunk, p.K - k0);
        const bool split = h->head_streams == 2 && kc >= 2 && kc >= h->head_split_min_rois && h->dt == VK_F16;
        const int ka = split ? kc / 2 : kc;
        if (split) {
            VK_TRY(ensure_side());
            VK_CHECK_HIP(hipEventRecord(h->ev_fork, s));
            VK_CHECK_HIP(hipStreamWaitEvent(h->side, h->ev_fork, 0));
        }
        const void *x = p.pooled;
        int hh = P, ww = P;
        for (int half = 0; half < (split ? 2 : 1); ++half) {
            const int n0 = half ? ka : 0, nb = half ? kc - ka : ka;
            hipStream_t hs = half ? h->side : s;
            VK_TRY(vk_roi_pool(res4, N, p.Hf, p.Wf, h->res4_c, p.rois + 5 * (size_t)(k0 + n0), nb, 1.0f / 16.0f, P,
                               (char *)p.pooled + (size_t)n0 * P * P * h->res4_c * es5, h->dt, hs));
            float *pp = p.pool_part ? (float *)((char *)p.pool_part + (half ? conv_duo_pool_part_bytes((long)ka * P * P, h->res5_c) : 0)) : nullptr;
            void *a = p.h_a, *b2 = p.h_b;
            x = p.pooled;
            hh = P;
            ww = P;
            for (size_t bi = 0; bi < h->res5.size(); ++bi) {
                int ho, wo;
                const bool last = bi + 1 == h->res5.size();
                VK_TRY(run_block(h, h->res5[bi], x, kc, hh, ww, p.h_t1, p.h_t2, p.h_sc, a, hs, &ho, &wo, last ? pp : nullptr,
                                 split ? n0 : 0, split ? nb : -1));
                hh = ho;
                ww = wo;
                x = a;
                std::swap(a, b2);
            }
            if (p.pool_part)
                VK_TRY(launch_pool_finish(pp, nb, hh * ww, h->res5.back().conv3.cin, h->res5_c, h->res5.back().fused_shortcut,
                                          p.feat + (size_t)(k0 + n0) * h->res5_c, hs));
        }
        if (split) {
            VK_CHECK_HIP(hipEventRecord(h->ev_join, h->side));
            VK_CHECK_HIP(hipStreamWaitEvent(s, h->ev_join, 0));
        }
        if (!p.pool_part) VK_TRY(vk_mean_pool(x, kc, hh * ww, h->res5_c, p.feat + (size_t)k0 * h->res5_c, h->dt, s));
    }
    if (p.chunk >= p.K) set_stage(h, "pooled", p.pooled, h->dt, {p.K, P, P, h->res4_c});
    set_stage(h, "feature_pooled", p.feat, VK_F32, {p.K, h->res5_c});

    const int C = c.num_classes, F = h->res5_c, E = h->emb_dim, AT = c.num_attrs;
    const int ld_cls = (C + 1 + 7) / 8 * 8, ld_attr = (AT + 1 + 7) / 8 * 8;
    VK_TRY(launch_concat_embed(p.feat, nullptr, nullptr, F, 0, p.K, p.featT, h->pdt, s));
    VK_TRY(run_conv(h, h->cls_score, p.featT, p.K, 1, 1, nullptr, p.cls_logits, false, VK_F32, ld_cls, s));
    VK_TRY(launch_softmax_argmax(p.cls_logits, ld_cls, p.K, C + 1, C, p.obj_prob, p.obj_cls, p.max_class, s));
    VK_TRY(launch_concat_embed(p.feat, h->emb, p.max_class, F, E, p.K, p.concat, h->pdt, s));
    VK_TRY(run_conv(h, h->fc_attr, p.concat, p.K, 1, 1, nullptr, p.attr_hid, true, h->pdt, 0, s));
    VK_TRY(run_conv(h, h->attr_score, p.attr_hid, p.K, 1, 1, nullptr, p.attr_logits, false, VK_F32, ld_attr, s));
    VK_TRY(launch_softmax_argmax(p.attr_logits, ld_attr, p.K, AT, AT, p.attr_prob, p.attr_cls, nullptr, s));
    set_stage(h, "obj_logits", p.cls_logits, VK_F32, {p.K, ld_cls});
    set_stage(h, "attr_logits", p.attr_logits, VK_F32, {p.K, ld_attr});
    return VK_OK;
}

static int fwd_close(vk_handle *h, const int32_t *nonfinite, hipStream_t s, int64_t *ticket) {
    if (h->timing && nonfinite) {
        VK_CHECK_HIP(hipEventRecord(h->ev[5], s));
        h->ev_valid = true;
    }
    if (!h->flag_host) {
        VK_CHECK_HIP(hipHostMalloc((void **)&h->flag_host, sizeof(int32_t) * vk_handle::VK_MAX_INFLIGHT, hipHostMallocDefault));
        for (auto &e : h->ev_done) VK_CHECK_HIP(hipEventCreateWithFlags(&e, hipEventDisableTiming));
    }
    const int slot = (int)(h->next_ticket % vk_handle::VK_MAX_INFLIGHT);
    if (nonfinite)
        VK_CHECK_HIP(hipMemcpyAsync(&h->flag_host[slot], nonfinite, sizeof(int32_t), hipMemcpyDeviceToHost, s));
    else
        h->flag_host[slot] = 0;
    VK_CHECK_HIP(hipEventRecord(h->ev_done[slot], s));
    *ticket = h->next_ticket++;
    return VK_OK;
}

struct TimerScope {
    explicit TimerScope(KernelTimer *t) { g_timer = t; }
    ~TimerScope() { g_timer = nullptr; }
};

}

extern "C" {

int vk_forward_begin(vk_handle *h, const float *images_dev, int N, int H, int W, const int32_t *image_hw,
                     const float *scales_yx, const vk_roi_params *rp, const vk_outputs *out, void *stream, int64_t *ticket) {
    return vk_forward_begin_ignorey(h, images_dev, N, H, W, image_hw, scales_yx, rp, out, stream, ticket, nullptr);
}

static int check_select_params(const vk_select_params *sp, const char *who) {
    const vk_roi_params &rp = sp->roi;
    VK_REQUIRE(rp.num_nms_thresh == 1, VK_EINVAL, "%s: per-class selection takes one NMS threshold, got a list of %d", who, rp.num_nms_thresh);
    VK_REQUIRE(sp->score_thresh >= 0.0 && sp->score_thresh <= 1.0, VK_EINVAL, "%s: score_thresh=%g must be in [0, 1]", who, sp->score_thresh);
    VK_REQUIRE(rp.min_detections <= rp.max_detections, VK_EINVAL, "%s: min_detections=%d exceeds max_detections=%d", who,
               rp.min_detections, rp.max_detections);
    return VK_OK;
}

static int fwd_per_class(vk_handle *h, const Plan &p, const vk_select_params *sp, const float *scales_dev, const vk_outputs *out,
                         hipStream_t s) {
    const vk_config &c = h->cfg;
    const int C = c.num_classes, F = h->res5_c, K = p.K, D = sp->roi.max_detections;
    const int nrow = 4 * (c.cls_agnostic_bbox_reg ? 1 : C);
    const int ld_cls = (C + 1 + 7) / 8 * 8, ld_box = (nrow + 7) / 8 * 8;
    if (!h->bbox_lin_w) {
        const int cp = vk_packed_cout(nrow);
        if (cp == nrow) {
            h->bbox_lin_w = h->bbox_w;
            h->bbox_lin_b = h->bbox_b;
        } else {
            const size_t row = (size_t)F * dtype_size(h->pdt);
            void *w = nullptr, *b = nullptr;
            VK_TRY(dev_alloc(h, (size_t)cp * row, &w));
            VK_TRY(dev_alloc(h, (size_t)cp * sizeof(float), &b));
            VK_CHECK_HIP(hipMemsetAsync(w, 0, (size_t)cp * row, s));
            VK_CHECK_HIP(hipMemsetAsync(b, 0, (size_t)cp * sizeof(float), s));
            VK_CHECK_HIP(hipMemcpyAsync(w, h->bbox_w, (size_t)nrow * row, hipMemcpyDeviceToDevice, s));
            VK_CHECK_HIP(hipMemcpyAsync(b, h->bbox_b, (size_t)nrow * sizeof(float), hipMemcpyDeviceToDevice, s));
            h->bbox_lin_w = w;
            h->bbox_lin_b = (const float *)b;
        }
    }
    Carver cv(nullptr);
    const size_t o_scores = cv.off;
    cv.take((size_t)K * ld_cls * sizeof(float));
    const size_t o_deltas = cv.off;
    cv.take((size_t)K * ld_box * sizeof(float));
    const size_t o_best = cv.off;
    cv.take((size_t)K * sizeof(unsigned long long));
    const size_t o_conf = cv.off;
    cv.take((size_t)K * sizeof(float));
    if (cv.off > h->pc_arena_bytes) {
        if (h->pc_arena) {
            VK_CHECK_HIP(hipDeviceSynchronize());
            VK_CHECK_HIP(hipFree(h->pc_arena));
            h->pc_arena = nullptr;
            h->pc_arena_bytes = 0;
        }
        VK_CHECK_HIP(hipMalloc((void **)&h->pc_arena, cv.off));
        h->pc_arena_bytes = cv.off;
    }
    float *scores = (float *)(h->pc_arena + o_scores), *deltas = (float *)(h->pc_arena + o_deltas);
    float *max_conf = (float *)(h->pc_arena + o_conf);

    VK_TRY(launch_class_probs(p.cls_logits, ld_cls, K, C + 1, scores, ld_cls, s));
    ConvArgs g;
    fill_conv_args(g, 1, 1, K, F, nrow, ld_box, 1, 1, 0, 1, 1, 0, h->pdt, VK_F32);
    g.x = p.featT;
    g.w = h->bbox_lin_w;
    g.bias = h->bbox_lin_b;
    g.y = deltas;
    VK_TRY(launch_conv(g, s));
    set_stage(h, "obj_scores", scores, VK_F32, {K, ld_cls});
    set_stage(h, "box_deltas", deltas, VK_F32, {K, ld_box});
    set_stage(h, "attr_prob", p.attr_prob, VK_F32, {K});
    if (h->timing) VK_CHECK_HIP(hipEventRecord(h->ev[4], s));

    PerClassArgs a;
    memset(&a, 0, sizeof(a));
    a.scores = scores;
    a.ld_scores = ld_cls;
    a.deltas = deltas;
    a.ld_box = ld_box;
    a.agnostic = c.cls_agnostic_bbox_reg ? 1 : 0;
    a.proposals = p.prop_boxes;
    a.counts = p.prop_counts;
    a.features = p.feat;
    a.attr_prob = p.attr_prob;
    a.attr_cls = p.attr_cls;
    a.F = F;
    a.R = p.R;
    a.D = D;
    a.C = C;
    a.image_hw = p.image_hw;
    a.scales_yx = scales_dev;
    a.wx = c.roi_bbox_weights[0];
    a.wy = c.roi_bbox_weights[1];
    a.ww = c.roi_bbox_weights[2];
    a.wh = c.roi_bbox_weights[3];
    a.clampv = (float)std::log(1000.0 / 16.0);
    a.thresh = sp->roi.nms_thresh[0];
    a.score_thresh = sp->score_thresh;
    a.mind = sp->roi.min_detections;
    a.maxd = sp->roi.max_detections;
    a.best = (unsigned long long *)(h->pc_arena + o_best);
    a.max_conf = max_conf;
    a.out = *out;
    a.keep_ids = p.keep_ids;
    a.nonfinite = p.nonfinite;
    VK_TRY(launch_per_class_select(a, p.N, s));
    set_stage(h, "max_conf", max_conf, VK_F32, {p.N, p.R});
    set_stage(h, "keep_ids", p.keep_ids, VK_I64, {p.N, D});
    return VK_OK;
}

static int forward_detect(vk_handle *h, const float *images_dev, int N, int H, int W, const int32_t *image_hw,
                          const float *scales_yx, const vk_roi_params *rp, const vk_select_params *sel, const vk_outputs *out,
                          void *stream, int64_t *ticket, const vk_ignorey *ignorey);

int vk_forward_begin_ignorey(vk_handle *h, const float *images_dev, int N, int H, int W, const int32_t *image_hw,
                             const float *scales_yx, const vk_roi_params *rp, const vk_outputs *out, void *stream, int64_t *ticket,
                             const vk_ignorey *ignorey) {
    return forward_detect(h, images_dev, N, H, W, image_hw, scales_yx, rp, nullptr, out, stream, ticket, ignorey);
}

int vk_forward_begin_select(vk_handle *h, const float *images_dev, int N, int H, int W, const int32_t *image_hw,
                            const float *scales_yx, const vk_select_params *sp, const vk_outputs *out, void *stream, int64_t *ticket,
                            const vk_ignorey *ignorey) {
    VK_REQUIRE(sp, VK_EINVAL, "forward: null argument");
    VK_REQUIRE(sp->mode == VK_SELECT_CLASS_MAX || sp->mode == VK_SELECT_PER_CLASS, VK_EINVAL, "forward: unknown selection mode %d", sp->mode);
    if (sp->mode == VK_SELECT_PER_CLASS) VK_TRY(check_select_params(sp, "forward"));
    return forward_detect(h, images_dev, N, H, W, image_hw, scales_yx, &sp->roi, sp->mode == VK_SELECT_PER_CLASS ? sp : nullptr, out,
                          stream, ticket, ignorey);
}

static int forward_detect(vk_handle *h, const float *images_dev, int N, int H, int W, const int32_t *image_hw,
                          const float *scales_yx, const vk_roi_params *rp, const vk_select_params *sel, const vk_outputs *out,
                          void *stream, int64_t *ticket, const vk_ignorey *ignorey) {
    VK_REQUIRE(h && images_dev && image_hw && rp && out && ticket, VK_EINVAL, "forward: null argument");
    const vk_ignorey *ig = scales_yx && ignorey && ignorey->max_per_image > 0 ? ignorey : nullptr;
    if (ig) {
        VK_REQUIRE(ig->max_per_image <= VK_MAX_IGNOREY, VK_EINVAL, "ignorey: max_per_image=%d must be in 0..%d", ig->max_per_image,
                   VK_MAX_IGNOREY);
        VK_REQUIRE(ig->bands && ig->counts, VK_EINVAL, "ignorey: null bands / counts");
        VK_REQUIRE(ig->f64 == 0 || ig->f64 == 1, VK_EINVAL, "ignorey: f64=%d must be 0 or 1", ig->f64);
        for (int n = 0; n < N; ++n) {
            const int J = ig->counts[n];
            VK_REQUIRE(J >= 0 && J <= ig->max_per_image, VK_EINVAL, "ignorey: counts[%d]=%d must be in 0..%d", n, J, ig->max_per_image);
            for (int k = 0; k < 2 * J; ++k) {
                const size_t at = ((size_t)n * ig->max_per_image) * 2 + k;
                const double v = ig->f64 ? static_cast<const double *>(ig->bands)[at] : (double)static_cast<const float *>(ig->bands)[at];
                VK_REQUIRE(std::isfinite(v) && std::fabs(v) < 2147483648.0, VK_EINVAL, "ignorey: image %d band %d holds %g (must be finite, "
                           "|value| < 2^31)", n, k / 2, v);
            }
        }
    }
    VK_REQUIRE(h->next_ticket - h->oldest_open < vk_handle::VK_MAX_INFLIGHT, VK_EINVAL,
               "forward_begin: %d forwards are already in flight; end the oldest first", vk_handle::VK_MAX_INFLIGHT);
    VK_REQUIRE(h->finalized, VK_EINVAL, "forward: vk_finalize has not been called");
    VK_REQUIRE(N >= 1 && H >= 32 && W >= 32, VK_EINVAL, "forward: bad input size N=%d H=%d W=%d", N, H, W);
    VK_REQUIRE(rp->num_nms_thresh >= 1 && rp->num_nms_thresh <= VK_MAX_NMS_THRESH, VK_EINVAL, "forward: 1..%d nms thresholds", VK_MAX_NMS_THRESH);
    VK_REQUIRE(rp->max_detections >= 1 && rp->max_detections <= h->cfg.post_nms_topk, VK_EINVAL,
               "forward: max_detections=%d must be in 1..POST_NMS_TOPK_TEST", rp->max_detections);
    for (int n = 0; n < N; ++n)
        VK_REQUIRE(image_hw[2 * n] >= 1 && image_hw[2 * n + 1] >= 1, VK_EINVAL, "forward: image_shapes[%d]=(%d,%d) must be positive",
                   n, image_hw[2 * n], image_hw[2 * n + 1]);
    VK_CHECK_HIP(hipSetDevice(h->device));
    hipStream_t s = (hipStream_t)stream;
    const vk_config &c = h->cfg;
    const int D = rp->max_detections;
    TimerScope timer_scope(h->ktimer);
    const bool tm = h->timing;

    Plan p;
    VK_TRY(fwd_open(h, N, H, W, c.post_nms_topk, D, image_hw, scales_yx, nullptr, ig, s, &p));
    const void *res4 = nullptr;
    VK_TRY(fwd_backbone(h, p, images_dev, s, &res4));

    const int ld_rpn = (5 * h->A + 7) / 8 * 8;
    VK_TRY(run_conv(h, h->rpn_conv, res4, N, p.Hf, p.Wf, nullptr, p.rpn_hid, true, h->dt, 0, s));
    VK_TRY(run_conv(h, h->rpn_heads, p.rpn_hid, N, p.Hf, p.Wf, nullptr, p.rpn_out, false, VK_F32, ld_rpn, s));
    set_stage(h, "rpn_out", p.rpn_out, VK_F32, {N, p.Hf, p.Wf, ld_rpn});
    if (tm) VK_CHECK_HIP(hipEventRecord(h->ev[2], s));

    vk_ignorey ig_dev{};
    if (ig) {
        ig_dev.bands = p.bands;
        ig_dev.counts = p.band_counts;
        ig_dev.max_per_image = ig->max_per_image;
        ig_dev.f64 = ig->f64;
    }
    VK_TRY(vk_rpn_proposals_ignorey(p.rpn_out, ld_rpn, p.rpn_out + h->A, ld_rpn, N, p.Hf, p.Wf, h->A, h->cell_anchors, 16,
                                    c.anchor_offset, p.image_hw, c.rpn_bbox_weights, c.rpn_min_size, c.rpn_nms_thresh,
                                    c.pre_nms_topk, c.post_nms_topk, p.prop_boxes, p.prop_logits, p.prop_counts, p.nonfinite,
                                    p.rpn_ws, p.rpn_ws_bytes, s, ig ? &ig_dev : nullptr));
    VK_TRY(launch_make_rois(p.prop_boxes, N, p.R, p.rois, s));
    set_stage(h, "proposal_boxes", p.prop_boxes, VK_F32, {N, p.R, 4});
    set_stage(h, "proposal_logits", p.prop_logits, VK_F32, {N, p.R});
    set_stage(h, "proposal_counts", p.prop_counts, VK_I32, {N});
    if (tm) VK_CHECK_HIP(hipEventRecord(h->ev[3], s));

    VK_TRY(fwd_head(h, p, res4, s));
    if (sel) {
        VK_TRY(fwd_per_class(h, p, sel, scales_yx ? p.scales : nullptr, out, s));
        return fwd_close(h, p.nonfinite, s, ticket);
    }
    const int F = h->res5_c;
    VK_TRY(launch_chosen_deltas(p.featT, F, h->bbox_w, h->bbox_b, p.obj_cls, c.cls_agnostic_bbox_reg, F, p.K, p.chosen, h->pdt, s));
    set_stage(h, "chosen_deltas", p.chosen, VK_F32, {p.K, 4});
    if (tm) VK_CHECK_HIP(hipEventRecord(h->ev[4], s));

    RoiFinalArgs a;
    memset(&a, 0, sizeof(a));
    a.obj_prob = p.obj_prob;
    a.obj_cls = p.obj_cls;
    a.attr_prob = p.attr_prob;
    a.attr_cls = p.attr_cls;
    a.box_deltas = p.chosen;
    a.ld_box = 4;
    a.delta_mode = 1;
    a.proposals = p.prop_boxes;
    a.counts = p.prop_counts;
    a.features = p.feat;
    a.F = F;
    a.R = p.R;
    a.D = D;
    a.image_hw = p.image_hw;
    a.scales_yx = scales_yx ? p.scales : nullptr;
    a.wx = c.roi_bbox_weights[0];
    a.wy = c.roi_bbox_weights[1];
    a.ww = c.roi_bbox_weights[2];
    a.wh = c.roi_bbox_weights[3];
    a.clampv = (float)std::log(1000.0 / 16.0);
    a.n_thresh = rp->num_nms_thresh;
    for (int i = 0; i < rp->num_nms_thresh; ++i) a.thresh[i] = rp->nms_thresh[i];
    a.mind = rp->min_detections;
    a.maxd = rp->max_detections;
    a.out = *out;
    a.keep_ids = p.keep_ids;
    a.nonfinite = p.nonfinite;
    VK_TRY(launch_roi_final(a, N, s));
    set_stage(h, "keep_ids", p.keep_ids, VK_I64, {N, D});
    return fwd_close(h, p.nonfinite, s, ticket);
}

int vk_forward_boxes_begin(vk_handle *h, const float *images_dev, int N, int H, int W, const int32_t *image_hw,
                           const float *scales_yx, const float *boxes_dev, int B, const int32_t *counts, const vk_outputs *out,
                           void *stream, int64_t *ticket) {
    VK_REQUIRE(images_dev && image_hw && counts && out && ticket, VK_EINVAL, "forward_boxes: null argument");
    VK_REQUIRE(N >= 1 && H >= 32 && W >= 32, VK_EINVAL, "forward_boxes: bad input size N=%d H=%d W=%d", N, H, W);
    VK_REQUIRE(B >= 0 && B <= 1024, VK_EINVAL, "forward_boxes: B=%d boxes per image must be in 0..1024", B);
    VK_REQUIRE(B == 0 || boxes_dev, VK_EINVAL, "forward_boxes: null boxes with B=%d", B);
    VK_REQUIRE(out->preds_per_image, VK_EINVAL, "forward_boxes: null preds_per_image");
    VK_REQUIRE(B == 0 || (out->obj_ids && out->obj_probs && out->attr_ids && out->attr_probs && out->boxes && out->roi_features),
               VK_EINVAL, "forward_boxes: null output array");
    VK_REQUIRE(B == 0 || ((uintptr_t)out->roi_features & 15) == 0, VK_EINVAL, "forward_boxes: roi_features must be 16-byte aligned");
    for (int n = 0; n < N; ++n) {
        VK_REQUIRE(counts[n] >= 0 && counts[n] <= B, VK_EINVAL, "forward_boxes: counts[%d]=%d must be in 0..B=%d", n, counts[n], B);
        VK_REQUIRE(image_hw[2 * n] >= 1 && image_hw[2 * n + 1] >= 1, VK_EINVAL,
                   "forward_boxes: image_shapes[%d]=(%d,%d) must be positive", n, image_hw[2 * n], image_hw[2 * n + 1]);
    }
    VK_REQUIRE(h, VK_EINVAL, "forward_boxes: null handle");
    VK_REQUIRE(h->next_ticket - h->oldest_open < vk_handle::VK_MAX_INFLIGHT, VK_EINVAL,
               "forward_boxes_begin: %d forwards are already in flight; end the oldest first", vk_handle::VK_MAX_INFLIGHT);
    VK_REQUIRE(h->finalized, VK_EINVAL, "forward_boxes: vk_finalize has not been called");
    VK_CHECK_HIP(hipSetDevice(h->device));
    hipStream_t s = (hipStream_t)stream;
    if (B == 0) {
        h->stages_out.clear();
        h->ev_valid = false;
        VK_CHECK_HIP(hipMemsetAsync(out->preds_per_image, 0, sizeof(int64_t) * (size_t)N, s));
        return fwd_close(h, nullptr, s, ticket);
    }
    TimerScope timer_scope(h->ktimer);
    const bool tm = h->timing;

    Plan p;
    VK_TRY(fwd_open(h, N, H, W, B, B, image_hw, scales_yx, counts, nullptr, s, &p));
    const void *res4 = nullptr;
    VK_TRY(fwd_backbone(h, p, images_dev, s, &res4));
    if (tm) VK_CHECK_HIP(hipEventRecord(h->ev[2], s));

    VK_TRY(launch_given_boxes_ingest(boxes_dev, p.prop_counts, p.image_hw, scales_yx ? p.scales : nullptr, N, B, p.prop_boxes,
                                     p.rois, p.nonfinite, s));
    set_stage(h, "proposal_boxes", p.prop_boxes, VK_F32, {N, B, 4});
    set_stage(h, "proposal_counts", p.prop_counts, VK_I32, {N});
    if (tm) VK_CHECK_HIP(hipEventRecord(h->ev[3], s));

    VK_TRY(fwd_head(h, p, res4, s));
    if (tm) VK_CHECK_HIP(hipEventRecord(h->ev[4], s));

    VK_TRY(launch_given_box_outputs(p.obj_prob, p.obj_cls, p.attr_prob, p.attr_cls, p.prop_boxes, p.prop_counts,
                                    scales_yx ? p.scales : nullptr, p.feat, h->res5_c, N, B, *out, s));
    return fwd_close(h, p.nonfinite, s, ticket);
}

int vk_forward_end(vk_handle *h, int64_t ticket) {
    VK_REQUIRE(h, VK_EINVAL, "forward_end: null handle");
    VK_REQUIRE(ticket == h->oldest_open && ticket < h->next_ticket, VK_EINVAL,
               "forward_end: ticket %lld is not the oldest forward in flight (%lld)", (long long)ticket, (long long)h->oldest_open);
    const int slot = (int)(ticket % vk_handle::VK_MAX_INFLIGHT);
    h->oldest_open++;
    VK_CHECK_HIP(hipSetDevice(h->device));
    VK_CHECK_HIP(hipEventSynchronize(h->ev_done[slot]));
    if (h->ktimer) h->ktimer->collect();
    VK_REQUIRE(h->flag_host[slot] == 0, VK_ENONFINITE, "Box tensor contains infinite or NaN!");
    return VK_OK;
}

int vk_enable_kernel_timing(vk_handle *h, int enable) {
    VK_REQUIRE(h, VK_EINVAL, "null handle");
    if (enable && !h->ktimer) h->ktimer = new KernelTimer();
    if (!enable && h->ktimer) {
        delete h->ktimer;
        h->ktimer = nullptr;
    }
    return VK_OK;
}

int vk_get_kernel_timing(vk_handle *h, int64_t *launches, double *ms, double *flops, double *bytes, int reset) {
    VK_REQUIRE(h && launches && ms && flops && bytes, VK_EINVAL, "null argument");
    VK_REQUIRE(h->ktimer, VK_EINVAL, "kernel timing is not enabled");
    for (int i = 0; i < VK_NUM_KERNEL_BUCKETS; ++i) {
        launches[i] = h->ktimer->launches[i];
        ms[i] = h->ktimer->ms[i];
        flops[i] = h->ktimer->flops[i];
        bytes[i] = h->ktimer->bytes[i];
        if (reset) {
            h->ktimer->bytes[i] = 0;
            h->ktimer->launches[i] = 0;
            h->ktimer->ms[i] = 0;
            h->ktimer->flops[i] = 0;
        }
    }
    return VK_OK;
}

int vk_make_rois(const float *boxes, int N, int R, float *rois, void *stream) {
    VK_REQUIRE(boxes && rois && N > 0 && R > 0, VK_EINVAL, "make_rois: bad arguments");
    return launch_make_rois(boxes, N, R, rois, (hipStream_t)stream);
}

int vk_softmax_argmax(const float *logits, int ld, int K, int n_softmax, int n_argmax, float *prob_out, int32_t *cls_out,
                      int32_t *raw_argmax_out, void *stream) {
    VK_REQUIRE(logits && prob_out && cls_out && K >= 0 && n_softmax >= 1 && n_argmax >= 1 && n_argmax <= n_softmax && ld >= n_softmax,
               VK_EINVAL, "softmax_argmax: bad arguments");
    return launch_softmax_argmax(logits, ld, K, n_softmax, n_argmax, prob_out, cls_out, raw_argmax_out, (hipStream_t)stream);
}

int vk_concat_embed(const float *features, int F, const void *emb, int E, const int32_t *cls, int K, void *out, vk_dtype dt,
                    void *stream) {
    VK_REQUIRE(features && out && F > 0 && E >= 0 && K >= 0 && (E == 0 || (emb && cls)), VK_EINVAL, "concat_embed: bad arguments");
    VK_REQUIRE(dt == VK_F16 || dt == VK_F32, VK_EINVAL, "concat_embed: dtype must be f16 or f32");
    return launch_concat_embed(features, emb, cls, F, E, K, out, dt, (hipStream_t)stream);
}

int vk_chosen_deltas(const void *x, int ldx, const void *w_rows, const float *bias, const int32_t *cls, int cls_agnostic, int F,
                     int K, float *out, vk_dtype dt, void *stream) {
    VK_REQUIRE(x && w_rows && bias && out && (cls || cls_agnostic) && F > 0 && ldx >= F && K >= 0, VK_EINVAL, "chosen_deltas: bad arguments");
    VK_REQUIRE(dt == VK_F16 || dt == VK_F32, VK_EINVAL, "chosen_deltas: dtype must be f16 or f32");
    return launch_chosen_deltas(x, ldx, w_rows, bias, cls, cls_agnostic, F, K, out, dt, (hipStream_t)stream);
}

int vk_roi_outputs(const float *obj_logits, int ld_obj, const float *attr_logits, int ld_attr, const float *box_deltas,
                   int ld_box, int chosen_only, const float *proposals, const int32_t *counts, const float *features, int F,
                   int N, int R, int C, int A, const int32_t *image_hw, const float *scales_yx_dev,
                   const float *weights4_host, const vk_roi_params *rp, const vk_outputs *out, int64_t *keep_ids_out,
                   int32_t *nonfinite_flag, void *stream) {
    VK_REQUIRE(obj_logits && box_deltas && proposals && counts && features && image_hw && rp && out && nonfinite_flag, VK_EINVAL,
               "roi_outputs: null argument");
    VK_REQUIRE(rp->num_nms_thresh >= 1 && rp->num_nms_thresh <= VK_MAX_NMS_THRESH, VK_EINVAL, "roi_outputs: 1..%d nms thresholds", VK_MAX_NMS_THRESH);
    hipStream_t s = (hipStream_t)stream;
    const int K = N * R;
    char *scratch = nullptr;
    const size_t per = align_up((size_t)K * 4, 256);
    VK_CHECK_HIP(hipMalloc((void **)&scratch, per * 4));
    float *obj_prob = (float *)scratch, *attr_prob = (float *)(scratch + per);
    int32_t *obj_cls = (int32_t *)(scratch + 2 * per), *attr_cls = (int32_t *)(scratch + 3 * per);
    int st = launch_softmax_argmax(obj_logits, ld_obj, K, C + 1, C, obj_prob, obj_cls, nullptr, s);
    if (st == VK_OK && attr_logits) st = launch_softmax_argmax(attr_logits, ld_attr, K, A, A, attr_prob, attr_cls, nullptr, s);
    if (st == VK_OK) {
        RoiFinalArgs a;
        memset(&a, 0, sizeof(a));
        a.obj_prob = obj_prob;
        a.obj_cls = obj_cls;
        a.attr_prob = attr_logits ? attr_prob : nullptr;
        a.attr_cls = attr_logits ? attr_cls : nullptr;
        a.box_deltas = box_deltas;
        a.ld_box = ld_box;
        a.delta_mode = chosen_only ? 1 : 0;
        a.proposals = proposals;
        a.counts = counts;
        a.features = features;
        a.F = F;
        a.R = R;
        a.D = rp->max_detections;
        a.image_hw = image_hw;
        a.scales_yx = scales_yx_dev;
        a.wx = weights4_host[0];
        a.wy = weights4_host[1];
        a.ww = weights4_host[2];
        a.wh = weights4_host[3];
        a.clampv = (float)std::log(1000.0 / 16.0);
        a.n_thresh = rp->num_nms_thresh;
        for (int i = 0; i < rp->num_nms_thresh; ++i) a.thresh[i] = rp->nms_thresh[i];
        a.mind = rp->min_detections;
        a.maxd = rp->max_detections;
        a.out = *out;
        a.keep_ids = keep_ids_out;
        a.nonfinite = nonfinite_flag;
        st = launch_roi_final(a, N, s);
    }
    hipError_t e = hipStreamSynchronize(s);
    (void)hipFree(scratch);
    if (st != VK_OK) return st;
    VK_CHECK_HIP(e);
    return VK_OK;
}

int vk_class_probs(const float *logits, int ld, int K, int n, float *out, int ld_out, void *stream) {
    VK_REQUIRE(logits && out && K >= 0 && n >= 1 && ld >= n && ld_out >= n, VK_EINVAL, "class_probs: bad arguments");
    return launch_class_probs(logits, ld, K, n, out, ld_out, (hipStream_t)stream);
}

int vk_class_boxes(const float *box_deltas, int ld_box, int cls_agnostic, const float *proposals, const int32_t *counts, int N, int R,
                   int C, const int32_t *image_hw, const float *weights4_host, float *out, int32_t *nonfinite_flag, void *stream) {
    VK_REQUIRE(box_deltas && proposals && counts && image_hw && weights4_host && out, VK_EINVAL, "class_boxes: null argument");
    PerClassArgs a;
    memset(&a, 0, sizeof(a));
    a.deltas = box_deltas;
    a.ld_box = ld_box;
    a.agnostic = cls_agnostic ? 1 : 0;
    a.proposals = proposals;
    a.counts = counts;
    a.R = R;
    a.C = C;
    a.image_hw = image_hw;
    a.wx = weights4_host[0];
    a.wy = weights4_host[1];
    a.ww = weights4_host[2];
    a.wh = weights4_host[3];
    a.clampv = (float)std::log(1000.0 / 16.0);
    a.nonfinite = nonfinite_flag;
    return launch_class_boxes(a, N, out, (hipStream_t)stream);
}

int vk_per_class_select(const float *obj_scores, int ld_scores, const float *attr_logits, int ld_attr, const float *box_deltas,
                        int ld_box, int cls_agnostic, const float *proposals, const int32_t *counts, const float *features, int F,
                        int N, int R, int C, int A, const int32_t *image_hw, const float *scales_yx_dev,
                        const float *weights4_host, const vk_select_params *sp, const vk_outputs *out, int64_t *keep_ids_out,
                        float *max_conf_out, int32_t *nonfinite_flag, void *stream) {
    VK_REQUIRE(obj_scores && box_deltas && proposals && counts && features && image_hw && weights4_host && sp && out && nonfinite_flag,
               VK_EINVAL, "per_class_select: null argument");
    VK_REQUIRE(sp->mode == VK_SELECT_PER_CLASS, VK_EINVAL, "per_class_select: mode=%d is not VK_SELECT_PER_CLASS", sp->mode);
    VK_TRY(check_select_params(sp, "per_class_select"));
    VK_REQUIRE(N >= 1 && N <= 65535 && R >= 1 && R <= 1024 && C >= 1, VK_EINVAL, "per_class_select: N=%d R=%d C=%d (R at most 1024)", N, R, C);
    VK_REQUIRE(sp->roi.max_detections >= 1 && sp->roi.max_detections <= R, VK_EINVAL, "per_class_select: max_detections=%d must be in 1..R=%d",
               sp->roi.max_detections, R);
    VK_REQUIRE(F >= 4 && F % 4 == 0, VK_EINVAL, "per_class_select: F=%d must be a positive multiple of 4", F);
    VK_REQUIRE(!attr_logits || (A >= 1 && ld_attr >= A), VK_EINVAL, "per_class_select: A=%d ld_attr=%d", A, ld_attr);
    hipStream_t s = (hipStream_t)stream;
    const int K = N * R;
    char *scratch = nullptr;
    const size_t per = align_up((size_t)K * 8, 256);
    VK_CHECK_HIP(hipMalloc((void **)&scratch, per * 3));
    float *attr_prob = (float *)(scratch + per);
    int32_t *attr_cls = (int32_t *)(scratch + 2 * per);
    int st = VK_OK;
    if (attr_logits) st = launch_softmax_argmax(attr_logits, ld_attr, K, A, A, attr_prob, attr_cls, nullptr, s);
    if (st == VK_OK) {
        PerClassArgs a;
        memset(&a, 0, sizeof(a));
        a.scores = obj_scores;
        a.ld_scores = ld_scores;
        a.deltas = box_deltas;
        a.ld_box = ld_box;
        a.agnostic = cls_agnostic ? 1 : 0;
        a.proposals = proposals;
        a.counts = counts;
        a.features = features;
        a.attr_prob = attr_logits ? attr_prob : nullptr;
        a.attr_cls = attr_logits ? attr_cls : nullptr;
        a.F = F;
        a.R = R;
        a.D = sp->roi.max_detections;
        a.C = C;
        a.image_hw = image_hw;
        a.scales_yx = scales_yx_dev;
        a.wx = weights4_host[0];
        a.wy = weights4_host[1];
        a.ww = weights4_host[2];
        a.wh = weights4_host[3];
        a.clampv = (float)std::log(1000.0 / 16.0);
        a.thresh = sp->roi.nms_thresh[0];
        a.score_thresh = sp->score_thresh;
        a.mind = sp->roi.min_detections;
        a.maxd = sp->roi.max_detections;
        a.best = (unsigned long long *)scratch;
        a.max_conf = max_conf_out;
        a.out = *out;
        a.keep_ids = keep_ids_out;
        a.nonfinite = nonfinite_flag;
        st = launch_per_class_select(a, N, s);
    }
    hipError_t e = hipStreamSynchronize(s);
    (void)hipFree(scratch);
    if (st != VK_OK) return st;
    VK_CHECK_HIP(e);
    return VK_OK;
}

}
```

vltk_amd/frcnn.py:

```python
import ctypes as C
import os
import warnings
from collections import OrderedDict

import numpy as np
import torch

from . import _lib as L
from .config import CONFIG_NAME, WEIGHTS_NAME, Config
from .layers import DTYPES, TORCH_DTYPES, stream
from .parallel import OutputBlock, output_spec


SELECTIONS = ("class_max", "per_class")


class ROIOutputs:

    def __init__(self, cfg):
        self.score_thresh = cfg.ROI_HEADS.SCORE_THRESH_TEST
        self.min_detections = cfg.MIN_DETECTIONS
        self.max_detections = cfg.MAX_DETECTIONS
        nms_thresh = cfg.ROI_HEADS.NMS_THRESH_TEST
        self.nms_thresh = list(nms_thresh) if isinstance(nms_thresh, (list, tuple)) else [nms_thresh]
        self.selection = "class_max"

    def params(self):
        thr = list(self.nms_thresh)
        if len(thr) > L.VK_MAX_NMS_THRESH:
            raise ValueError(f"at most {L.VK_MAX_NMS_THRESH} NMS thresholds")
        rp = L.vk_roi_params()
        rp.num_nms_thresh = len(thr)
        for i, t in enumerate(thr):
            rp.nms_thresh[i] = float(t)
        rp.min_detections, rp.max_detections = int(self.min_detections), int(self.max_detections)
        return rp

    def select_params(self):
        sel = getattr(self, "selection", "class_max")
        if sel not in SELECTIONS:
            raise ValueError(f"roi_outputs.selection={sel!r} must be one of {SELECTIONS}")
        if sel == "class_max":
            return None
        thr = list(self.nms_thresh)
        if len(thr) != 1:
            raise ValueError(f'selection="per_class" takes one nms_thresh, got the list {thr}')
        if int(self.min_detections) > int(self.max_detections):
            raise ValueError(f"min_detections={int(self.min_detections)} exceeds max_detections={int(self.max_detections)}")
        score = float(self.score_thresh)
        if not 0.0 <= score <= 1.0:
            raise ValueError(f"score_thresh={score} must be in [0, 1]")
        sp = L.vk_select_params()
        sp.mode, sp.score_thresh, sp.roi = L.VK_SELECT_PER_CLASS, score, self.params()
        return sp


def _c_config(cfg, dt):
    c = L.vk_config()
    r = cfg.RESNETS
    c.depth, c.num_groups, c.width_per_group = r.DEPTH, r.NUM_GROUPS, r.WIDTH_PER_GROUP
    c.stem_out_channels, c.res2_out_channels = r.STEM_OUT_CHANNELS, r.RES2_OUT_CHANNELS
    c.stride_in_1x1 = int(bool(r.STRIDE_IN_1X1))
    c.caffe_maxpool = int(bool(cfg.MODEL.MAX_POOL))
    sizes, ratios = cfg.ANCHOR_GENERATOR.SIZES, cfg.ANCHOR_GENERATOR.ASPECT_RATIOS
    if len(sizes) != 1 or len(ratios) != 1:
        raise ValueError("only the single-level (C4) anchor generator is supported")
    c.num_sizes, c.num_ratios = len(sizes[0]), len(ratios[0])
    for i, v in enumerate(sizes[0]):
        c.sizes[i] = v
    for i, v in enumerate(ratios[0]):
        c.ratios[i] = v
    c.anchor_offset = cfg.ANCHOR_GENERATOR.OFFSET
    c.rpn_hidden_channels = cfg.PROPOSAL_GENERATOR.HIDDEN_CHANNELS
    c.rpn_min_size = cfg.PROPOSAL_GENERATOR.MIN_SIZE
    c.rpn_nms_thresh = cfg.RPN.NMS_THRESH
    c.pre_nms_topk, c.post_nms_topk = cfg.RPN.PRE_NMS_TOPK_TEST, cfg.RPN.POST_NMS_TOPK_TEST
    for i, v in enumerate(cfg.RPN.BBOX_REG_WEIGHTS):
        c.rpn_bbox_weights[i] = v
    c.num_classes, c.num_attrs = cfg.ROI_HEADS.NUM_CLASSES, cfg.ROI_BOX_HEAD.NUM_ATTRS
    c.use_attr = int(bool(cfg.ROI_BOX_HEAD.ATTR))
    c.pooler_resolution = cfg.ROI_BOX_HEAD.POOLER_RESOLUTION
    c.res5_halve = int(bool(cfg.ROI_BOX_HEAD.RES5HALVE))
    c.cls_agnostic_bbox_reg = int(bool(cfg.ROI_BOX_HEAD.CLS_AGNOSTIC_BBOX_REG))
    for i, v in enumerate(cfg.ROI_BOX_HEAD.BBOX_REG_WEIGHTS):
        c.roi_bbox_weights[i] = v
    c.precision = dt
    return c


MAX_GIVEN_BOXES = 1024


def _validate_proposals(proposals, N):
    if isinstance(proposals, (torch.Tensor, np.ndarray)):
        t = torch.as_tensor(proposals)
        if t.dim() != 3 or t.shape[2] != 4:
            raise ValueError(f"proposals as one array must be [N, K, 4], got shape {tuple(t.shape)}")
        if t.shape[0] != N:
            raise ValueError(f"proposals: {t.shape[0]} images of boxes for {N} images")
        if t.shape[1] > MAX_GIVEN_BOXES:
            raise ValueError(f"proposals: {t.shape[1]} boxes per image, at most {MAX_GIVEN_BOXES}")
        return t, np.full(N, t.shape[1], dtype=np.int32)
    items = list(proposals)
    if len(items) != N:
        raise ValueError(f"proposals: {len(items)} images of boxes for {N} images")
    ts = []
    for i, b in enumerate(items):
        t = b if isinstance(b, torch.Tensor) else torch.as_tensor(np.asarray(b, dtype=np.float32))
        if t.numel() == 0 and t.dim() == 1:
            t = t.reshape(0, 4)
        if t.dim() != 2 or t.shape[1] != 4:
            raise ValueError(f"proposals[{i}] must be [K, 4], got {tuple(t.shape)}")
        if t.shape[0] > MAX_GIVEN_BOXES:
            raise ValueError(f"proposals[{i}]: {t.shape[0]} boxes, at most {MAX_GIVEN_BOXES}")
        ts.append(t)
    return ts, np.asarray([t.shape[0] for t in ts], dtype=np.int32).reshape(N)


def pack_proposals(proposals, N, device=None):
    ts, counts = _validate_proposals(proposals, N)
    if isinstance(ts, torch.Tensor):
        return ts.to(device=device, dtype=torch.float32).contiguous(), counts
    B = int(counts.max(initial=0))
    if all(t.device.type == "cpu" for t in ts):
        host = np.zeros((N, B, 4), dtype=np.float32)
        for i, t in enumerate(ts):
            host[i, :t.shape[0]] = t.detach().to(torch.float32).numpy()
        return torch.from_numpy(host).to(device), counts
    out = torch.zeros((N, B, 4), dtype=torch.float32, device=device)
    for i, t in enumerate(ts):
        out[i, :t.shape[0]] = t.detach().to(device=out.device, dtype=torch.float32)
    return out, counts


MAX_IGNOREY = L.VK_MAX_IGNOREY


def _validate_ignorey(ignorey, N):
    if isinstance(ignorey, (torch.Tensor, np.ndarray)):
        t = torch.as_tensor(ignorey)
        if t.dim() != 3 or t.shape[2] != 2:
            raise ValueError(f"ignorey as one array must be [N, J, 2], got shape {tuple(t.shape)}")
        if t.shape[0] != N:
            raise ValueError(f"ignorey: {t.shape[0]} images of bands for {N} images")
        items = list(t.detach().cpu())
    else:
        items = list(ignorey)
        if len(items) != N:
            raise ValueError(f"ignorey: {len(items)} images of bands for {N} images")
    ts = []
    for i, b in enumerate(items):
        t = torch.as_tensor(b).detach().cpu()
        if t.numel() == 0 and t.dim() == 1:
            t = t.reshape(0, 2)
        if t.dim() != 2 or t.shape[1] != 2:
            raise ValueError(f"ignorey[{i}] must be [J, 2] (y0, y1 rows), got {tuple(t.shape)}")
        if t.shape[0] > MAX_IGNOREY:
            raise ValueError(f"ignorey[{i}]: {t.shape[0]} bands, at most {MAX_IGNOREY}")
        if t.dtype == torch.bool or t.is_complex():
            raise ValueError(f"ignorey[{i}]: dtype {t.dtype} is not a real number")
        ts.append(t)
    return ts, any(t.dtype == torch.float64 for t in ts)


def pack_ignorey(ignorey, scales_yx, N):
    ts, f64 = _validate_ignorey(ignorey, N)
    if scales_yx is None:
        warnings.warn("ignorey is ignored without scales_yx, as in the reference (frcnn.py:328)", UserWarning, stacklevel=3)
        return None
    counts = np.asarray([t.shape[0] for t in ts], dtype=np.int32).reshape(N)
    J = int(counts.max(initial=0))
    if J == 0:
        return None
    dt = torch.float64 if f64 else torch.float32
    sc = torch.from_numpy(np.ascontiguousarray(np.asarray(scales_yx, dtype=np.float32).reshape(N, 2)))
    bands = np.zeros((N, J, 2), dtype=np.float64 if f64 else np.float32)
    for n, t in enumerate(ts):
        if t.shape[0] == 0:
            continue
        g = (t.to(dt) * 1 / sc[n, 1]).numpy()
        if not (np.isfinite(g).all() and (np.abs(g) < 2.0 ** 31).all()):
            raise ValueError(f"ignorey[{n}]: bands / scales_yx[{n}][1] must be finite and below 2^31 in magnitude, got {g.tolist()}")
        bands[n, :t.shape[0]] = g
    return bands, counts, f64


def check_given_width(width, max_detections):
    if max_detections is not None and int(max_detections) < width:
        raise ValueError(f"max_detections={int(max_detections)} is smaller than the {width} boxes given for one image; "
                         "given boxes are never truncated")


class _Ticket:

    __slots__ = ("ticket", "block", "images", "done", "error")

    def __init__(self, ticket, block, images):
        self.ticket, self.block = ticket, block
        self.images = images
        self.done, self.error = False, None


class PendingForward:

    def __init__(self, model, state, hw, given_width=None):
        self.model, self._state, self.hw = model, state, hw
        self.given_width = given_width

    @classmethod
    def finished(cls, model, block, hw, given_width=None):
        st = _Ticket(-1, block, None)
        st.done = True
        return cls(model, st, hw, given_width)

    @property
    def ticket(self):
        return self._state.ticket

    @property
    def block(self):
        return self._state.block

    def wait_raw(self):
        st = self._state
        if not st.done:
            self.model._end(st)
        if st.error is not None:
            raise st.error
        self.model._last_padded = st.block
        return st.block

    def wait(self, **kwargs):
        if self.given_width is not None:
            check_given_width(self.given_width, kwargs.get("max_detections"))
        return FRCNN._format(self.wait_raw(), self.hw, **kwargs)

    def __del__(self):
        try:
            if not self._state.done and self.model._h:
                self.model._close_through(self._state)
        except Exception:
            pass


class FRCNN:
    given_boxes = True

    def __new__(cls, cfg=None, *a, **k):
        if cls is FRCNN and cfg is not None and len(cfg.RPN.IN_FEATURES) > 1:
            from .frcnn_fpn import FRCNNFPN
            return object.__new__(FRCNNFPN)
        return object.__new__(cls)

    def __init__(self, cfg, precision=None, device=None):
        self._init_host(cfg, precision, device)
        self._h = C.c_void_p()
        L.call("vk_create", C.byref(_c_config(cfg, self.dt)), self.device.index, C.byref(self._h))

    def _init_host(self, cfg, precision, device):
        if not torch.cuda.is_available():
            raise RuntimeError("vltk_amd.FRCNN needs an AMD GPU (HIP device); there is no CPU fallback")
        L.load()
        self.config = cfg
        self.min_detections = cfg.min_detections
        self.max_detections = cfg.max_detections
        dev = torch.device(device if device is not None else cfg.MODEL.DEVICE)
        if dev.type != "cuda" or dev.index is None:
            dev = torch.device("cuda", torch.cuda.current_device())
        self.device = dev
        self.precision = precision or os.environ.get("VLTK_AMD_PRECISION", "fp16")
        if self.precision not in ("fp16", "fp32"):
            raise KeyError(self.precision)
        self.dt, self.tdt = DTYPES[self.precision]
        self.roi_outputs = ROIOutputs(cfg)
        self.training = False
        self._open = []
        self._finalized = False

    def eval(self):
        self.training = False
        return self

    def train(self, mode=True):
        self.training = bool(mode)
        return self

    def to(self, *a, **k):
        return self

    def __del__(self):
        h = getattr(self, "_h", None)
        if h:
            try:
                L.load().vk_destroy(h)
            except Exception:
                pass
            self._h = None

    def expected_keys(self):
        n = C.c_int()
        L.call("vk_num_weights", self._h, C.byref(n))
        out = []
        for i in range(n.value):
            s = C.c_char_p()
            L.call("vk_weight_name", self._h, i, C.byref(s))
            out.append(s.value.decode())
        return out

    def load_state_dict(self, state_dict, strict=True):
        if self._finalized:
            raise RuntimeError("weights were already loaded into this model")
        for k, v in state_dict.items():
            a = v.detach().cpu().numpy() if isinstance(v, torch.Tensor) else np.asarray(v)
            if a.dtype == np.int64:
                dt = L.VK_I64
            else:
                a = np.ascontiguousarray(a, dtype=np.float32)
                dt = L.VK_F32
            shape = (C.c_int64 * max(a.ndim, 1))(*a.shape)
            L.call("vk_load_weights", self._h, k.encode(), a.ctypes.data_as(C.c_void_p), shape, a.ndim, dt)
        L.call("vk_finalize", self._h)
        self._finalized = True
        return self

    @classmethod
    def from_pretrained(cls, pretrained_model_name_or_path, *model_args, **kwargs):
        config = kwargs.pop("config", None)
        state_dict = kwargs.pop("state_dict", None)
        precision = kwargs.pop("precision", None)
        if not isinstance(config, Config):
            config = Config.from_pretrained(config if config is not None else pretrained_model_name_or_path)
        if state_dict is None:
            path = pretrained_model_name_or_path
            if os.path.isdir(path):
                path = os.path.join(path, WEIGHTS_NAME)
                if not os.path.isfile(path):
                    raise EnvironmentError(
                        "Error no file named {} found in directory {} ".format(WEIGHTS_NAME, pretrained_model_name_or_path))
            elif not os.path.isfile(path):
                raise EnvironmentError(f"Can't load weights for '{pretrained_model_name_or_path}'.")
            try:
                state_dict = torch.load(path, map_location="cpu", weights_only=True)
            except Exception:
                raise OSError("Unable to load weights from pytorch checkpoint file. ")
        model = cls(config, precision=precision)
        model.load_state_dict(state_dict)
        return model.eval()

    def set_option(self, key, value):
        L.call("vk_set_option", self._h, key.encode(), int(value))

    def enable_stage_timing(self, on=True):
        L.call("vk_enable_stage_timing", self._h, int(on))

    def stage_timing_ms(self):
        ms = (C.c_float * 6)()
        L.call("vk_get_stage_timing", self._h, ms)
        return dict(zip(("backbone", "rpn_head", "proposals", "roi_heads", "predictor_outputs", "total"), list(ms)))

    def enable_kernel_timing(self, on=True):
        L.call("vk_enable_kernel_timing", self._h, int(on))

    def kernel_timing(self, reset=False):
        n = (C.c_int64 * 12)()
        ms = (C.c_double * 12)()
        fl = (C.c_double * 12)()
        by = (C.c_double * 12)()
        L.call("vk_get_kernel_timing", self._h, n, ms, fl, by, int(reset))
        names = ("conv_mfma256", "conv_mfma_f16", "conv_mfma_f16_f32out", "other", "conv3x3_panel", "conv_duo", "two_stream_backbone", "conv3x3_blk", "conv_ws",
                 "conv_mfma256_dual", "conv_gemm4", "bneck64")
        return {k: {"launches": int(n[i]), "ms": float(ms[i]), "flops": float(fl[i]), "bytes": float(by[i])}
                for i, k in enumerate(names)}

    def get_stage(self, name):
        ptr, dt, nd = C.c_void_p(), C.c_int(), C.c_int()
        shape = (C.c_int64 * 4)()
        L.call("vk_get_stage", self._h, name.encode(), C.byref(ptr), C.byref(dt), shape, C.byref(nd))
        shp = [int(shape[i]) for i in range(nd.value)]
        out = torch.empty(shp, dtype=TORCH_DTYPES[dt.value], device=self.device)
        nbytes = out.numel() * out.element_size()
        L.call("vk_memcpy_d2d", out.data_ptr(), ptr.value, nbytes, stream(self.device))
        torch.cuda.synchronize(self.device)
        return out

    def __call__(self, *a, **k):
        return self.forward(*a, **k)

    def forward(self, images, image_shapes, gt_boxes=None, proposals=None, scales_yx=None, ignorey=None, **kwargs):
        if proposals is not None and self.given_boxes:
            counts = _validate_proposals(proposals, len(images))[1]
            check_given_width(int(counts.max(initial=0)), kwargs.get("max_detections"))
        return self.forward_async(images, image_shapes, gt_boxes, proposals, scales_yx, ignorey).wait(**kwargs)

    def _prepare(self, images, image_shapes, proposals, scales_yx, ignorey):
        if self.training:
            raise NotImplementedError()
        if ignorey is not None and proposals is not None:
            raise ValueError("ignorey removes / trims RPN proposals: there are none with proposals=")
        if not self._finalized:
            raise RuntimeError("no weights loaded: call load_state_dict / from_pretrained first")
        images = torch.as_tensor(images)
        if images.dim() != 4 or images.shape[1] != 3:
            raise ValueError(f"images must be [N,3,H,W], got {tuple(images.shape)}")
        N = images.shape[0]
        sc = None
        if scales_yx is not None:
            sc = np.ascontiguousarray(np.asarray(torch.as_tensor(scales_yx).cpu(), dtype=np.float32).reshape(N, 2))
        ig = pack_ignorey(ignorey, sc, N) if ignorey is not None else None
        given = pack_proposals(proposals, N, self.device) if proposals is not None else None
        images = images.to(device=self.device, dtype=torch.float32).contiguous()
        hw = np.ascontiguousarray(np.asarray(torch.as_tensor(image_shapes).cpu()).reshape(N, 2), dtype=np.int32)
        return images, hw, sc, given, ig

    def forward_async(self, images, image_shapes, gt_boxes=None, proposals=None, scales_yx=None, ignorey=None):
        images, hw, sc, given, ig = self._prepare(images, image_shapes, proposals, scales_yx, ignorey)
        N, _, H, W = images.shape
        F = self.config.RESNETS.RES2_OUT_CHANNELS * 8
        dev, s = self.device, stream(self.device)
        scp = sc.ctypes.data_as(C.c_void_p) if sc is not None else None
        ticket = C.c_int64(-1)
        if given is not None:
            boxes, counts = given
            B = boxes.shape[1]
            bufs = OutputBlock(output_spec(N, B, F), device=dev)
            out = L.vk_outputs(*[bufs[k].data_ptr() for k in bufs])
            L.call("vk_forward_boxes_begin", self._h, images.data_ptr(), N, H, W, hw.ctypes.data_as(C.c_void_p), scp,
                   boxes.data_ptr() if B else None, B, counts.ctypes.data_as(C.c_void_p), C.byref(out), s, C.byref(ticket))
            st = _Ticket(ticket.value, bufs, (images, boxes))
            self._open.append(st)
            return PendingForward(self, st, hw, given_width=B)
        sp = self.roi_outputs.select_params()
        rp = self.roi_outputs.params()
        bufs = OutputBlock(output_spec(N, rp.max_detections, F), device=dev)
        out = L.vk_outputs(*[bufs[k].data_ptr() for k in bufs])
        if sp is not None:
            igs = None
            if ig is not None:
                bands, bcounts, f64 = ig
                igs = C.byref(L.vk_ignorey(bands.ctypes.data, bcounts.ctypes.data, bands.shape[1], int(f64)))
            L.call("vk_forward_begin_select", self._h, images.data_ptr(), N, H, W, hw.ctypes.data_as(C.c_void_p), scp,
                   C.byref(sp), C.byref(out), s, C.byref(ticket), igs)
        elif ig is None:
            L.call("vk_forward_begin", self._h, images.data_ptr(), N, H, W, hw.ctypes.data_as(C.c_void_p), scp, C.byref(rp),
                   C.byref(out), s, C.byref(ticket))
        else:
            bands, bcounts, f64 = ig
            igs = L.vk_ignorey(bands.ctypes.data, bcounts.ctypes.data, bands.shape[1], int(f64))
            L.call("vk_forward_begin_ignorey", self._h, images.data_ptr(), N, H, W, hw.ctypes.data_as(C.c_void_p), scp,
                   C.byref(rp), C.byref(out), s, C.byref(ticket), C.byref(igs))
        st = _Ticket(ticket.value, bufs, images)
        self._open.append(st)
        return PendingForward(self, st, hw)

    def _end(self, st):
        try:
            L.call("vk_forward_end", self._h, C.c_int64(st.ticket))
        except ValueError:
            raise
        except Exception as e:
            st.error = e
        st.done, st.images = True, None
        if st in self._open:
            self._open.remove(st)

    def _close_through(self, st):
        while self._open:
            head = self._open[0]
            self._end(head)
            if head is st:
                break

    inference = forward

    def forward_padded(self):
        return self._last_padded

    @staticmethod
    def _format(bufs, hw, padding=None, max_detections=None, return_tensors=None, pad_value=0, location=None, **_):
        assert return_tensors in {"pt", "np", None}
        assert padding in {"max_detections", "max_batch", None}
        ppi = bufs["preds_per_image"].cpu()
        counts = ppi.tolist()
        N = len(counts)
        keys = ("obj_ids", "obj_probs", "attr_ids", "attr_probs", "boxes", "roi_features")
        if padding is None and return_tensors is None:
            out = OrderedDict((k, [bufs[k][i, :counts[i]] for i in range(N)]) for k in keys[:5])
            out["preds_per_image"] = ppi
            out["roi_features"] = [bufs["roi_features"][i, :counts[i]] for i in range(N)]
            return OrderedDict((k, out[k]) for k in
                               ("obj_ids", "obj_probs", "attr_ids", "attr_probs", "boxes", "preds_per_image", "roi_features"))
        D = bufs["obj_ids"].shape[1]
        if padding == "max_detections":
            width = int(max_detections) if max_detections is not None else D
        elif padding == "max_batch":
            width = max(counts) if counts else 0
        else:
            width = None

        def fix(t):
            if width is None:
                if len(set(counts)) > 1:
                    raise ValueError("return_tensors without padding needs equal detections per image")
                t = t[:, :counts[0]] if counts else t
            elif width <= t.shape[1]:
                t = t[:, :width].clone()
            else:
                pad = torch.zeros((t.shape[0], width - t.shape[1]) + tuple(t.shape[2:]), dtype=t.dtype, device=t.device)
                t = torch.cat([t, pad], dim=1)
            if pad_value != 0 and width is not None:
                for i, c in enumerate(counts):
                    t[i, c:] = pad_value
            if location == "cpu" or return_tensors == "np":
                t = t.cpu()
            return t.numpy() if return_tensors == "np" else t

        out = OrderedDict((k, fix(bufs[k])) for k in keys)
        sizes = torch.as_tensor(hw.astype(np.int64))
        out["preds_per_image"] = ppi.numpy() if return_tensors == "np" else ppi
        out["sizes"] = sizes.numpy() if return_tensors == "np" else sizes
        nb = out["boxes"].copy() if return_tensors == "np" else out["boxes"].clone()
        hwf = hw.astype(np.float32)
        if return_tensors == "np":
            nb[:, :, 0::2] /= hwf[:, 1].reshape(-1, 1, 1)
            nb[:, :, 1::2] /= hwf[:, 0].reshape(-1, 1, 1)
        else:
            s = torch.as_tensor(hwf, device=nb.device)
            nb[:, :, 0::2] /= s[:, 1].view(-1, 1, 1)
            nb[:, :, 1::2] /= s[:, 0].view(-1, 1, 1)
        out["normalized_boxes"] = nb
        return OrderedDict((k, out[k]) for k in ("obj_ids", "obj_probs", "attr_ids", "attr_probs", "boxes", "sizes",
                                                 "preds_per_image", "roi_features", "normalized_boxes"))
```

vltk_amd/pipeline.py:

```python
import queue
import threading

import numpy as np
import torch
import torch.distributed as dist

from .extraction import ExtractionWriter
from .parallel import OutputBlock, gather_outputs_async, output_spec, shard_indices

_STOP = object()


def _world(group=None):
    if dist.is_available() and dist.is_initialized():
        return dist.get_rank(group), dist.get_world_size(group)
    return 0, 1


class ExtractionPipeline:

    def __init__(self, model, preprocess, savefile, batch_size=32, visual_dim=2048, dataset=None, processor_args=None,
                 model_config=None, group=None, depth=2, boxes=None, ignorey=None):
        self.model, self.preprocess = model, preprocess
        self.boxes = None if boxes is None else {str(k): v for k, v in boxes.items()}
        self.ignorey = None if ignorey is None else {str(k): v for k, v in ignorey.items()}
        self.B, self.F = int(batch_size), int(visual_dim)
        self.D = int(model.roi_outputs.max_detections)
        self.group = group
        self.rank, self.world = _world(group)
        self.depth = max(2, int(depth))
        self.savefile = savefile
        self.writer = None
        if self.rank == 0:
            self.writer = ExtractionWriter(savefile, self.D, self.F, dataset=dataset, processor_args=processor_args,
                                           model_config=model_config)
        self.spec = output_spec(self.B, self.D, self.F)
        self.images_done = 0

    def _load(self, items, n_steps, q):
        try:
            it = iter(items)
            last = None
            for _ in range(n_steps):
                ids, raws = [], []
                for _ in range(self.B):
                    nxt = next(it, None)
                    if nxt is None:
                        break
                    ids.append(str(nxt[0]))
                    raws.append(np.ascontiguousarray(nxt[1]))
                    last = raws[-1]
                n_valid = len(ids)
                if last is None:
                    raise ValueError("a rank received no image at all: fewer images than ranks")
                while len(raws) < self.B:
                    raws.append(last)
                q.put((ids, raws, n_valid))
            q.put(_STOP)
        except BaseException as e:
            q.put(e)

    def _write(self, q, free):
        try:
            while True:
                job = q.get()
                if job is _STOP:
                    return
                slot, host, event, ids_per_rank = job
                event.synchronize()
                nb = host.numel() // self.world
                for r in range(self.world):
                    ids = ids_per_rank[r]
                    if ids:
                        blk = OutputBlock(self.spec, flat=host[r * nb:(r + 1) * nb])
                        n = len(ids)
                        boxes = np.round(blk["boxes"][:n].numpy())
                        self.writer.write_batch(ids, blk["obj_ids"][:n].numpy().astype(np.float32),
                                                blk["attr_ids"][:n].numpy().astype(np.float32), boxes,
                                                blk["roi_features"][:n].numpy())
                free.put(slot)
        except BaseException as e:
            self._writer_error = e
            while True:
                job = q.get()
                if job is _STOP:
                    return
                free.put(job[0])

    def run(self, items, n_items=None):
        if n_items is None:
            if self.world > 1:
                raise ValueError("n_items (the global image count) is required with more than one rank")
            n_items = len(items)
        spans = [shard_indices(n_items, r, self.world) for r in range(self.world)]
        if n_items < self.world:
            raise ValueError(f"{n_items} image(s) for {self.world} ranks: every rank needs at least one image")
        n_steps = max((hi - lo + self.B - 1) // self.B for lo, hi in spans)
        dev = self.model.device
        load_q = queue.Queue(maxsize=2)
        loader = threading.Thread(target=self._load, args=(items, n_steps, load_q), daemon=True)
        loader.start()
        write_q, free = queue.Queue(), queue.Queue()
        self._writer_error = None
        wthread = None
        host, gbuf = [], []
        nbytes = OutputBlock(self.spec, device="cpu").flat.numel()
        if self.rank == 0:
            for s in range(self.depth):
                h = torch.empty(self.world * nbytes, dtype=torch.uint8)
                host.append(h.pin_memory() if dev.type == "cuda" else h)
                free.put(s)
            wthread = threading.Thread(target=self._write, args=(write_q, free), daemon=True)
            wthread.start()
        if self.world > 1:
            gbuf = [torch.empty(self.world * nbytes, dtype=torch.uint8, device=dev) for _ in range(self.depth)]
        on_gpu = dev.type == "cuda"
        copy_stream = torch.cuda.Stream(device=dev) if on_gpu else None
        upload_stream = torch.cuda.Stream(device=dev) if on_gpu else None

        def finish(p, ids, n_valid, step):
            blk = p.wait_raw()
            if self.boxes is not None:
                blk = self._widen(blk)
            slot = step % self.depth
            if self.rank == 0:
                slot = free.get()
                if self._writer_error is not None:
                    raise self._writer_error
            handle = gather_outputs_async(blk, self.group, out=gbuf[slot] if gbuf else None)
            flat, _ = handle.wait_flat()
            if self.rank == 0:
                if copy_stream is not None:
                    copy_stream.wait_stream(torch.cuda.current_stream(dev))
                    with torch.cuda.stream(copy_stream):
                        host[slot].copy_(flat, non_blocking=True)
                        flat.record_stream(copy_stream)
                        ev = torch.cuda.Event()
                        ev.record(copy_stream)
                else:
                    host[slot].copy_(flat)
                    ev = _DoneEvent()
                ids_per_rank = []
                for r, (lo, hi) in enumerate(spans):
                    a, b = min(lo + step * self.B, hi), min(lo + (step + 1) * self.B, hi)
                    ids_per_rank.append(ids[:n_valid] if r == self.rank else self._ids_of(r, a, b))
                write_q.put((slot, host[slot], ev, ids_per_rank))
            self.images_done += n_valid

        try:
            prev = None
            for step in range(n_steps):
                job = load_q.get()
                if isinstance(job, BaseException):
                    raise job
                ids, raws, n_valid = job
                if on_gpu:
                    with torch.cuda.stream(upload_stream):
                        dev_raws = [torch.from_numpy(r).to(dev) for r in raws]
                    torch.cuda.current_stream(dev).wait_stream(upload_stream)
                    for t in dev_raws:
                        t.record_stream(torch.cuda.current_stream(dev))
                else:
                    dev_raws = [torch.from_numpy(r) for r in raws]
                _, images, sizes, scales_yx = self.preprocess(dev_raws, list(range(self.B)))
                kw = {}
                if self.boxes is not None:
                    kw["proposals"] = [self.boxes[i] for i in ids] + [self.boxes[ids[-1]]] * (self.B - n_valid)
                if self.ignorey is not None:
                    none = np.zeros((0, 2), dtype=np.float32)
                    kw["ignorey"] = [self.ignorey.get(i, none) for i in ids] + [self.ignorey.get(ids[-1], none)] * (self.B - n_valid)
                if hasattr(self.model, "forward_async"):
                    p = self.model.forward_async(images, sizes, scales_yx=scales_yx, **kw)
                else:
                    self.model(images, sizes, scales_yx=scales_yx, **kw)
                    p = _Finished(self.model.forward_padded())
                if prev is not None:
                    finish(*prev)
                prev = (p, ids, n_valid, step)
            if prev is not None:
                finish(*prev)
        finally:
            if wthread is not None:
                write_q.put(_STOP)
                wthread.join()
        if self._writer_error is not None:
            raise self._writer_error
        return self.writer.close() if self.rank == 0 else None

    def _widen(self, blk):
        w = blk["obj_ids"].shape[1]
        if w == self.D:
            return blk
        if w > self.D:
            raise ValueError(f"{w} boxes for one image, more than max_detections={self.D}")
        out = OutputBlock(self.spec, device=blk["obj_ids"].device)
        out.flat.zero_()
        for k, v in blk.items():
            if k == "preds_per_image":
                out[k].copy_(v)
            else:
                out[k][:, :w].copy_(v)
        return out

    def set_global_ids(self, ids):
        self._global_ids = [str(i) for i in ids]
        return self

    def _ids_of(self, rank, a, b):
        g = getattr(self, "_global_ids", None)
        if g is None:
            raise ValueError("with more than one rank, rank 0 needs the global id list: call set_global_ids(all_ids)")
        return g[a:b]


class _DoneEvent:
    def synchronize(self):
        pass


class _Finished:

    def __init__(self, block):
        self.block = block

    def wait_raw(self):
        return self.block


def extract_images(model, preprocess, items, savedir, split="train", dataset=None, batch_size=32, processor_args=None,
                   group=None, global_ids=None, n_items=None):
    import os
    cfgd = model.config.to_dict() if hasattr(getattr(model, "config", None), "to_dict") else None
    pipe = ExtractionPipeline(model, preprocess, os.path.join(savedir, f"{split}.arrow"), batch_size=batch_size,
                              visual_dim=getattr(model, "visual_dim", 2048), dataset=dataset, processor_args=processor_args,
                              model_config=cfgd, group=group)
    if global_ids is not None:
        pipe.set_global_ids(global_ids)
    return pipe.run(items, n_items=n_items)
```

Baseline: 485.6 images/sec.

## Run overlapping forwards on two lanes with double-buffered arenas

Adds a second working set (activation arena and predictor arena) and per-lane streams and events, so that when a forward begins while another is still open it alternates onto a separate non-blocking stream with its own arena. This lets consecutive batches overlap on the GPU instead of serializing on the caller's stream, and fences results back to the caller stream at forward_end. The cost is doubled workspace memory and extra cross-stream event waits. The extraction pipeline explicitly sets lanes to 1, so the benchmark path may not use it. Option handling is also refactored into check/default/get helpers.

Result: faster. 493.9 images/sec, median of 6 (+1.7%).

```diff
diff --git a/include/vltk_hip.h b/include/vltk_hip.h
--- a/include/vltk_hip.h
+++ b/include/vltk_hip.h
@@ -96,6 +96,9 @@
 int vk_destroy(vk_handle *h);
 
 int vk_set_option(vk_handle *h, const char *key, int value);
+int vk_get_option(vk_handle *h, const char *key, int *value);
+int vk_option_check(const char *key, int value);
+int vk_option_default(const char *key, int *value);
 
 int vk_num_weights(vk_handle *h, int *count);
 int vk_weight_name(vk_handle *h, int index, const char **name);
diff --git a/vltk_amd/_lib.py b/vltk_amd/_lib.py
--- a/vltk_amd/_lib.py
+++ b/vltk_amd/_lib.py
@@ -78,6 +78,9 @@
     "vk_finalize": (_I, [_P]),
     "vk_destroy": (_I, [_P]),
     "vk_set_option": (_I, [_P, C.c_char_p, _I]),
+    "vk_get_option": (_I, [_P, C.c_char_p, C.POINTER(_I)]),
+    "vk_option_check": (_I, [C.c_char_p, _I]),
+    "vk_option_default": (_I, [C.c_char_p, C.POINTER(_I)]),
     "vk_num_weights": (_I, [_P, C.POINTER(_I)]),
     "vk_weight_name": (_I, [_P, _I, C.POINTER(C.c_char_p)]),
     "vk_forward": (_I, [_P, _P, _I, _I, _I, _P, _P, C.POINTER(vk_roi_params), C.POINTER(vk_outputs), _P]),
diff --git a/vltk_amd/csrc/model.hip b/vltk_amd/csrc/model.hip
--- a/vltk_amd/csrc/model.hip
+++ b/vltk_amd/csrc/model.hip
@@ -144,6 +144,11 @@
 
 using namespace vk;
 
+static constexpr struct {
+    int head_chunk = 9600, backbone_streams = 2, backbone_split_min_batch = 8, head_streams = 1, head_split_min_rois = 512;
+    int forward_lanes = 2;
+} kDefaults;
+
 struct vk_handle {
     vk_config cfg;
     int device = 0;
@@ -165,17 +170,30 @@
     int A = 0, res4_c = 0, res5_c = 0, hid = 0, emb_dim = 0;
     std::vector<void *> owned;
 
-    char *arena = nullptr;
-    size_t arena_bytes = 0;
-    char *pc_arena = nullptr;
-    size_t pc_arena_bytes = 0;
+    struct WorkSet {
+        char *arena = nullptr;
+        size_t arena_bytes = 0;
+        char *pc_arena = nullptr;
+        size_t pc_arena_bytes = 0;
+    } sets[2];
+    struct Lane {
+        hipStream_t main = nullptr;
+        hipEvent_t ev_fork = nullptr, ev_join = nullptr;
+        hipEvent_t more_joins[2] = {nullptr, nullptr};
+    } lanes[2];
+    int forward_lanes = kDefaults.forward_lanes;
+    bool two_sets = false;
+    bool two_sets_failed = false;
+    int64_t lane_forwards = 0;
+    int cur_set = 0;
+    hipStream_t cur_caller = nullptr;
     const void *bbox_lin_w = nullptr;
     const float *bbox_lin_b = nullptr;
-    int head_chunk = 9600;
-    int backbone_streams = 2;
-    int backbone_split_min_batch = 8;
-    int head_streams = 1;
-    int head_split_min_rois = 512;
+    int head_chunk = kDefaults.head_chunk;
+    int backbone_streams = kDefaults.backbone_streams;
+    int backbone_split_min_batch = kDefaults.backbone_split_min_batch;
+    int head_streams = kDefaults.head_streams;
+    int head_split_min_rois = kDefaults.head_split_min_rois;
 
     struct Stage {
         const void *ptr;
@@ -188,15 +206,17 @@
     bool timing = false;
     hipEvent_t ev[6] = {nullptr, nullptr, nullptr, nullptr, nullptr, nullptr};
     hipStream_t side = nullptr;
-    hipEvent_t ev_fork = nullptr, ev_join = nullptr;
     hipStream_t more_sides[2] = {nullptr, nullptr};
-    hipEvent_t more_joins[2] = {nullptr, nullptr};
     bool ev_valid = false;
     static constexpr int VK_MAX_INFLIGHT = 4;
     int32_t *flag_host = nullptr;
     char *meta_host = nullptr;
     size_t meta_cap = 0;
     hipEvent_t ev_done[VK_MAX_INFLIGHT] = {nullptr, nullptr, nullptr, nullptr};
+    hipEvent_t ev_in[VK_MAX_INFLIGHT] = {nullptr, nullptr, nullptr, nullptr};
+    hipStream_t slot_stream[VK_MAX_INFLIGHT] = {nullptr, nullptr, nullptr, nullptr};
+    hipStream_t slot_caller[VK_MAX_INFLIGHT] = {nullptr, nullptr, nullptr, nullptr};
+    int slot_set[VK_MAX_INFLIGHT] = {-1, -1, -1, -1};
     int64_t next_ticket = 0, oldest_open = 0;
 };
 
@@ -854,12 +874,10 @@
     h->device = device;
     h->dt = (vk_dtype)cfg->precision;
     if (getenv("VK_PREDICTOR_FP16")) h->pdt = h->dt;
-    const char *env = getenv("VK_HEAD_CHUNK");
-    if (env && atoi(env) > 0) h->head_chunk = atoi(env);
-    if (const char *bs = getenv("VK_BACKBONE_STREAMS"))
-        if (bs[0] >= '1' && bs[0] <= '4') h->backbone_streams = bs[0] - '0';
-    if (const char *hs = getenv("VK_HEAD_STREAMS"))
-        if (hs[0] == '1' || hs[0] == '2') h->head_streams = hs[0] - '0';
+    (void)vk_option_default("head_chunk", &h->head_chunk);
+    (void)vk_option_default("backbone_streams", &h->backbone_streams);
+    (void)vk_option_default("head_streams", &h->head_streams);
+    (void)vk_option_default("forward_lanes", &h->forward_lanes);
     const int di = cfg->depth == 50 ? 0 : (cfg->depth == 101 ? 1 : 2);
     add_conv_names(h->names, "backbone.stem.conv1", true);
     h->stem = ConvLayer{"backbone.stem.conv1", 3, cfg->stem_out_channels, 7, 2, 3, 1, true, true};
@@ -1020,34 +1038,74 @@
     return VK_OK;
 }
 
+int vk_option_check(const char *key, int value) {
+    VK_REQUIRE(key, VK_EINVAL, "option: null key");
+    if (!strcmp(key, "head_chunk")) {
+        VK_REQUIRE(value >= 0, VK_EINVAL, "head_chunk must be >= 0 (0 = all RoIs at once)");
+    } else if (!strcmp(key, "backbone_streams")) {
+        VK_REQUIRE(value >= 1 && value <= 4, VK_EINVAL, "backbone_streams must be 1..4");
+    } else if (!strcmp(key, "head_streams")) {
+        VK_REQUIRE(value == 1 || value == 2, VK_EINVAL, "head_streams must be 1 or 2");
+    } else if (!strcmp(key, "forward_lanes")) {
+        VK_REQUIRE(value == 1 || value == 2, VK_EINVAL, "forward_lanes must be 1 or 2");
+    } else if (!strcmp(key, "head_split_min_rois")) {
+        VK_REQUIRE(value >= 2, VK_EINVAL, "head_split_min_rois must be >= 2");
+    } else if (!strcmp(key, "backbone_split_min_batch")) {
+        VK_REQUIRE(value >= 2, VK_EINVAL, "backbone_split_min_batch must be >= 2");
+    } else {
+        VK_REQUIRE(false, VK_EINVAL, "unknown option '%s'", key);
+    }
+    return VK_OK;
+}
+
+int vk_option_default(const char *key, int *value) {
+    VK_REQUIRE(key && value, VK_EINVAL, "option: null argument");
+    if (!strcmp(key, "head_chunk")) {
+        const char *env = getenv("VK_HEAD_CHUNK");
+        *value = env && atoi(env) > 0 ? atoi(env) : kDefaults.head_chunk;
+    } else if (!strcmp(key, "backbone_streams")) {
+        const char *bs = getenv("VK_BACKBONE_STREAMS");
+        *value = bs && bs[0] >= '1' && bs[0] <= '4' ? bs[0] - '0' : kDefaults.backbone_streams;
+    } else if (!strcmp(key, "head_streams")) {
+        const char *hs = getenv("VK_HEAD_STREAMS");
+        *value = hs && (hs[0] == '1' || hs[0] == '2') ? hs[0] - '0' : kDefaults.head_streams;
+    } else if (!strcmp(key, "forward_lanes")) {
+        const char *fl = getenv("VK_FORWARD_LANES");
+        *value = fl && (fl[0] == '1' || fl[0] == '2') && !fl[1] ? fl[0] - '0' : kDefaults.forward_lanes;
+    } else if (!strcmp(key, "head_split_min_rois")) {
+        *value = kDefaults.head_split_min_rois;
+    } else if (!strcmp(key, "backbone_split_min_batch")) {
+        *value = kDefaults.backbone_split_min_batch;
+    } else {
+        VK_REQUIRE(false, VK_EINVAL, "unknown option '%s'", key);
+    }
+    return VK_OK;
+}
+
+int vk_get_option(vk_handle *h, const char *key, int *value) {
+    VK_REQUIRE(h && key && value, VK_EINVAL, "get_option: null argument");
+    if (!strcmp(key, "head_chunk")) *value = h->head_chunk;
+    else if (!strcmp(key, "backbone_streams")) *value = h->backbone_streams;
+    else if (!strcmp(key, "head_streams")) *value = h->head_streams;
+    else if (!strcmp(key, "forward_lanes")) *value = h->forward_lanes;
+    else if (!strcmp(key, "head_split_min_rois")) *value = h->head_split_min_rois;
+    else if (!strcmp(key, "backbone_split_min_batch")) *value = h->backbone_split_min_batch;
+    else if (!strcmp(key, "working_sets")) *value = (h->sets[0].arena ? 1 : 0) + (h->sets[1].arena ? 1 : 0);
+    else if (!strcmp(key, "lane_forwards")) *value = (int)std::min<int64_t>(h->lane_forwards, INT32_MAX);
+    else VK_REQUIRE(false, VK_EINVAL, "unknown option '%s'", key);
+    return VK_OK;
+}
+
 int vk_set_option(vk_handle *h, const char *key, int value) {
     VK_REQUIRE(h && key, VK_EINVAL, "set_option: null argument");
-    if (!strcmp(key, "head_chunk")) {
-        VK_REQUIRE(value >= 0, VK_EINVAL, "head_chunk must be >= 0 (0 = all RoIs at once)");
-        h->head_chunk = value;
-        return VK_OK;
-    }
-    if (!strcmp(key, "backbone_streams")) {
-        VK_REQUIRE(value >= 1 && value <= 4, VK_EINVAL, "backbone_streams must be 1..4");
-        h->backbone_streams = value;
-        return VK_OK;
-    }
-    if (!strcmp(key, "head_streams")) {
-        VK_REQUIRE(value == 1 || value == 2, VK_EINVAL, "head_streams must be 1 or 2");
-        h->head_streams = value;
-        return VK_OK;
-    }
-    if (!strcmp(key, "head_split_min_rois")) {
-        VK_REQUIRE(value >= 2, VK_EINVAL, "head_split_min_rois must be >= 2");
-        h->head_split_min_rois = value;
-        return VK_OK;
-    }
-    if (!strcmp(key, "backbone_split_min_batch")) {
-        VK_REQUIRE(value >= 2, VK_EINVAL, "backbone_split_min_batch must be >= 2");
-        h->backbone_split_min_batch = value;
-        return VK_OK;
-    }
-    VK_REQUIRE(false, VK_EINVAL, "unknown option '%s'", key);
+    VK_TRY(vk_option_check(key, value));
+    if (!strcmp(key, "head_chunk")) h->head_chunk = value;
+    if (!strcmp(key, "backbone_streams")) h->backbone_streams = value;
+    if (!strcmp(key, "head_streams")) h->head_streams = value;
+    if (!strcmp(key, "forward_lanes")) h->forward_lanes = value;
+    if (!strcmp(key, "head_split_min_rois")) h->head_split_min_rois = value;
+    if (!strcmp(key, "backbone_split_min_batch")) h->backbone_split_min_batch = value;
+    return VK_OK;
 }
 
 int vk_destroy(vk_handle *h) {
@@ -1055,21 +1113,28 @@
     (void)hipSetDevice(h->device);
     (void)hipDeviceSynchronize();
     for (void *p : h->owned) (void)hipFree(p);
-    if (h->arena) (void)hipFree(h->arena);
-    if (h->pc_arena) (void)hipFree(h->pc_arena);
+    for (auto &ws : h->sets) {
+        if (ws.arena) (void)hipFree(ws.arena);
+        if (ws.pc_arena) (void)hipFree(ws.pc_arena);
+    }
     for (auto &e : h->ev)
         if (e) (void)hipEventDestroy(e);
     for (auto &e : h->ev_done)
         if (e) (void)hipEventDestroy(e);
+    for (auto &e : h->ev_in)
+        if (e) (void)hipEventDestroy(e);
     if (h->flag_host) (void)hipHostFree(h->flag_host);
     if (h->meta_host) (void)hipHostFree(h->meta_host);
-    if (h->ev_fork) (void)hipEventDestroy(h->ev_fork);
-    if (h->ev_join) (void)hipEventDestroy(h->ev_join);
+    for (auto &ln : h->lanes) {
+        if (ln.ev_fork) (void)hipEventDestroy(ln.ev_fork);
+        if (ln.ev_join) (void)hipEventDestroy(ln.ev_join);
+        for (auto &e : ln.more_joins)
+            if (e) (void)hipEventDestroy(e);
+        if (ln.main) (void)hipStreamDestroy(ln.main);
+    }
     if (h->side) (void)hipStreamDestroy(h->side);
-    for (int i = 0; i < 2; ++i) {
-        if (h->more_joins[i]) (void)hipEventDestroy(h->more_joins[i]);
-        if (h->more_sides[i]) (void)hipStreamDestroy(h->more_sides[i]);
-    }
+    for (auto &st : h->more_sides)
+        if (st) (void)hipStreamDestroy(st);
     delete h->ktimer;
     delete h;
     return VK_OK;
@@ -1102,6 +1167,10 @@
     VK_REQUIRE(h && name && dev_ptr && dtype && shape && ndim, VK_EINVAL, "null argument");
     auto it = h->stages_out.find(name);
     VK_REQUIRE(it != h->stages_out.end(), VK_EINVAL, "unknown stage '%s' (or no forward has run)", name);
+    if (h->next_ticket > h->oldest_open) {
+        const int slot = (int)((h->next_ticket - 1) % vk_handle::VK_MAX_INFLIGHT);
+        if (h->slot_stream[slot] != h->slot_caller[slot]) VK_CHECK_HIP(hipEventSynchronize(h->ev_done[slot]));
+    }
     *dev_ptr = it->second.ptr;
     *dtype = it->second.dt;
     *ndim = it->second.ndim;
@@ -1121,21 +1190,77 @@
 namespace vk {
 
 
+static int ensure_ticket_state(vk_handle *h) {
+    if (h->flag_host) return VK_OK;
+    for (auto &e : h->ev_done) VK_CHECK_HIP(hipEventCreateWithFlags(&e, hipEventDisableTiming));
+    for (auto &e : h->ev_in) VK_CHECK_HIP(hipEventCreateWithFlags(&e, hipEventDisableTiming));
+    VK_CHECK_HIP(hipHostMalloc((void **)&h->flag_host, sizeof(int32_t) * vk_handle::VK_MAX_INFLIGHT, hipHostMallocDefault));
+    return VK_OK;
+}
+
+static int ensure_arena(vk_handle *h, int set, size_t bytes, bool soft) {
+    vk_handle::WorkSet &ws = h->sets[set];
+    if (bytes <= ws.arena_bytes) return VK_OK;
+    if (ws.arena) {
+        VK_CHECK_HIP(hipDeviceSynchronize());
+        VK_CHECK_HIP(hipFree(ws.arena));
+        ws.arena = nullptr;
+        ws.arena_bytes = 0;
+    }
+    if (soft) {
+        if (hipMalloc((void **)&ws.arena, bytes) != hipSuccess) {
+            (void)hipGetLastError();
+            ws.arena = nullptr;
+            return 1;
+        }
+    } else {
+        VK_CHECK_HIP(hipMalloc((void **)&ws.arena, bytes));
+    }
+    ws.arena_bytes = bytes;
+    return VK_OK;
+}
+
+static int fwd_route(vk_handle *h, size_t arena_need, hipStream_t caller, hipStream_t *s_out) {
+    VK_TRY(ensure_ticket_state(h));
+    const int64_t t = h->next_ticket;
+    const int slot = (int)(t % vk_handle::VK_MAX_INFLIGHT);
+    bool laned = h->forward_lanes == 2 && !h->two_sets_failed && !h->ktimer && !h->timing;
+    if (laned && !h->two_sets && t > h->oldest_open) h->two_sets = true;
+    laned = laned && h->two_sets;
+    int set = laned ? (int)(t & 1) : 0;
+    if (set == 1 && ensure_arena(h, 1, arena_need, true) != VK_OK) {
+        h->two_sets_failed = true;
+        laned = false;
+        set = 0;
+    }
+    VK_TRY(ensure_arena(h, set, arena_need, false));
+    hipStream_t s = caller;
+    if (laned) {
+        vk_handle::Lane &ln = h->lanes[set];
+        if (!ln.main) VK_CHECK_HIP(hipStreamCreateWithFlags(&ln.main, hipStreamNonBlocking));
+        s = ln.main;
+        h->lane_forwards++;
+        VK_CHECK_HIP(hipEventRecord(h->ev_in[slot], caller));
+        VK_CHECK_HIP(hipStreamWaitEvent(s, h->ev_in[slot], 0));
+    }
+    for (int64_t u = h->oldest_open; u < t; ++u) {
+        const int us = (int)(u % vk_handle::VK_MAX_INFLIGHT);
+        if (h->slot_stream[us] == s || (laned && h->slot_set[us] != set)) continue;
+        VK_CHECK_HIP(hipStreamWaitEvent(s, h->ev_done[us], 0));
+    }
+    h->cur_set = set;
+    h->cur_caller = caller;
+    *s_out = s;
+    return VK_OK;
+}
+
 static int fwd_open(vk_handle *h, int N, int H, int W, int R, int D, const int32_t *image_hw, const float *scales_yx,
-                    const int32_t *counts, const vk_ignorey *ig, hipStream_t s, Plan *out) {
+                    const int32_t *counts, const vk_ignorey *ig, hipStream_t caller, Plan *out, hipStream_t *s_out) {
     Plan need = make_plan(h, nullptr, N, H, W, D, R);
-    if (need.total > h->arena_bytes) {
-        if (h->arena) {
-            VK_CHECK_HIP(hipDeviceSynchronize());
-            VK_CHECK_HIP(hipFree(h->arena));
-            h->arena = nullptr;
-            h->arena_bytes = 0;
-        }
-        VK_CHECK_HIP(hipMalloc((void **)&h->arena, need.total));
-        h->arena_bytes = need.total;
-    }
+    VK_TRY(fwd_route(h, need.total, caller, s_out));
+    hipStream_t s = *s_out;
     Plan &p = *out;
-    p = make_plan(h, h->arena, N, H, W, D, R);
+    p = make_plan(h, h->sets[h->cur_set].arena, N, H, W, D, R);
     h->stages_out.clear();
     if (h->timing) VK_CHECK_HIP(hipEventRecord(h->ev[0], s));
 
@@ -1172,9 +1297,23 @@
     return VK_OK;
 }
 
+static int ensure_sides(vk_handle *h, vk_handle::Lane &ln, int ns) {
+    if (!h->side) VK_CHECK_HIP(hipStreamCreateWithFlags(&h->side, hipStreamNonBlocking));
+    if (!ln.ev_fork) {
+        VK_CHECK_HIP(hipEventCreateWithFlags(&ln.ev_fork, hipEventDisableTiming));
+        VK_CHECK_HIP(hipEventCreateWithFlags(&ln.ev_join, hipEventDisableTiming));
+    }
+    for (int i = 0; i < ns - 2; ++i) {
+        if (!h->more_sides[i]) VK_CHECK_HIP(hipStreamCreateWithFlags(&h->more_sides[i], hipStreamNonBlocking));
+        if (!ln.more_joins[i]) VK_CHECK_HIP(hipEventCreateWithFlags(&ln.more_joins[i], hipEventDisableTiming));
+    }
+    return VK_OK;
+}
+
 static int fwd_backbone(vk_handle *h, const Plan &p, const float *images_dev, hipStream_t s, const void **res4_out) {
     const vk_config &c = h->cfg;
     const int N = p.N;
+    vk_handle::Lane &ln = h->lanes[h->cur_set];
     VK_TRY(stem_impl(images_dev, N, p.H, p.W, h->stem.w, h->stem.b, c.stem_out_channels, c.caffe_maxpool, p.bufA, h->dt,
                      p.img_pad, p.stem_out, s, p.nonfinite));
     void *cur = p.bufA, *nxt = p.bufB;
@@ -1185,24 +1324,15 @@
         hipStream_t gs_[4] = {s, nullptr, nullptr, nullptr};
         hipEvent_t gj_[4] = {nullptr, nullptr, nullptr, nullptr};
         if (split) {
-            if (!h->side) {
-                VK_CHECK_HIP(hipStreamCreateWithFlags(&h->side, hipStreamNonBlocking));
-                VK_CHECK_HIP(hipEventCreateWithFlags(&h->ev_fork, hipEventDisableTiming));
-                VK_CHECK_HIP(hipEventCreateWithFlags(&h->ev_join, hipEventDisableTiming));
-            }
-            for (int i = 0; i < ns - 2; ++i)
-                if (!h->more_sides[i]) {
-                    VK_CHECK_HIP(hipStreamCreateWithFlags(&h->more_sides[i], hipStreamNonBlocking));
-                    VK_CHECK_HIP(hipEventCreateWithFlags(&h->more_joins[i], hipEventDisableTiming));
-                }
+            VK_TRY(ensure_sides(h, ln, ns));
             gs_[1] = h->side;
-            gj_[1] = h->ev_join;
+            gj_[1] = ln.ev_join;
             for (int i = 2; i < ns; ++i) {
                 gs_[i] = h->more_sides[i - 2];
-                gj_[i] = h->more_joins[i - 2];
+                gj_[i] = ln.more_joins[i - 2];
             }
-            VK_CHECK_HIP(hipEventRecord(h->ev_fork, s));
-            for (int i = 1; i < ns; ++i) VK_CHECK_HIP(hipStreamWaitEvent(gs_[i], h->ev_fork, 0));
+            VK_CHECK_HIP(hipEventRecord(ln.ev_fork, s));
+            for (int i = 1; i < ns; ++i) VK_CHECK_HIP(hipStreamWaitEvent(gs_[i], ln.ev_fork, 0));
         }
         for (auto &b : h->stages[st]) {
             int ho, wo;
@@ -1235,23 +1365,16 @@
 static int fwd_head(vk_handle *h, const Plan &p, const void *res4, hipStream_t s) {
     const vk_config &c = h->cfg;
     const int N = p.N, P = p.P;
-    auto ensure_side = [&]() -> int {
-        if (!h->side) {
-            VK_CHECK_HIP(hipStreamCreateWithFlags(&h->side, hipStreamNonBlocking));
-            VK_CHECK_HIP(hipEventCreateWithFlags(&h->ev_fork, hipEventDisableTiming));
-            VK_CHECK_HIP(hipEventCreateWithFlags(&h->ev_join, hipEventDisableTiming));
-        }
-        return VK_OK;
-    };
+    vk_handle::Lane &ln = h->lanes[h->cur_set];
     const size_t es5 = dtype_size(h->dt);
     for (int k0 = 0; k0 < p.K; k0 += p.chunk) {
         const int kc = std::min(p.chunk, p.K - k0);
         const bool split = h->head_streams == 2 && kc >= 2 && kc >= h->head_split_min_rois && h->dt == VK_F16;
         const int ka = split ? kc / 2 : kc;
         if (split) {
-            VK_TRY(ensure_side());
-            VK_CHECK_HIP(hipEventRecord(h->ev_fork, s));
-            VK_CHECK_HIP(hipStreamWaitEvent(h->side, h->ev_fork, 0));
+            VK_TRY(ensure_sides(h, ln, 2));
+            VK_CHECK_HIP(hipEventRecord(ln.ev_fork, s));
+            VK_CHECK_HIP(hipStreamWaitEvent(h->side, ln.ev_fork, 0));
         }
         const void *x = p.pooled;
         int hh = P, ww = P;
@@ -1280,8 +1403,8 @@
                                           p.feat + (size_t)(k0 + n0) * h->res5_c, hs));
         }
         if (split) {
-            VK_CHECK_HIP(hipEventRecord(h->ev_join, h->side));
-            VK_CHECK_HIP(hipStreamWaitEvent(s, h->ev_join, 0));
+            VK_CHECK_HIP(hipEventRecord(ln.ev_join, h->side));
+            VK_CHECK_HIP(hipStreamWaitEvent(s, ln.ev_join, 0));
         }
         if (!p.pool_part) VK_TRY(vk_mean_pool(x, kc, hh * ww, h->res5_c, p.feat + (size_t)k0 * h->res5_c, h->dt, s));
     }
@@ -1307,11 +1430,11 @@
         VK_CHECK_HIP(hipEventRecord(h->ev[5], s));
         h->ev_valid = true;
     }
-    if (!h->flag_host) {
-        VK_CHECK_HIP(hipHostMalloc((void **)&h->flag_host, sizeof(int32_t) * vk_handle::VK_MAX_INFLIGHT, hipHostMallocDefault));
-        for (auto &e : h->ev_done) VK_CHECK_HIP(hipEventCreateWithFlags(&e, hipEventDisableTiming));
-    }
+    VK_TRY(ensure_ticket_state(h));
     const int slot = (int)(h->next_ticket % vk_handle::VK_MAX_INFLIGHT);
+    h->slot_stream[slot] = s;
+    h->slot_caller[slot] = h->cur_caller;
+    h->slot_set[slot] = nonfinite ? h->cur_set : -1;
     if (nonfinite)
         VK_CHECK_HIP(hipMemcpyAsync(&h->flag_host[slot], nonfinite, sizeof(int32_t), hipMemcpyDeviceToHost, s));
     else
@@ -1364,6 +1487,7 @@
             VK_CHECK_HIP(hipMemsetAsync(b, 0, (size_t)cp * sizeof(float), s));
             VK_CHECK_HIP(hipMemcpyAsync(w, h->bbox_w, (size_t)nrow * row, hipMemcpyDeviceToDevice, s));
             VK_CHECK_HIP(hipMemcpyAsync(b, h->bbox_b, (size_t)nrow * sizeof(float), hipMemcpyDeviceToDevice, s));
+            VK_CHECK_HIP(hipStreamSynchronize(s));
             h->bbox_lin_w = w;
             h->bbox_lin_b = (const float *)b;
         }
@@ -1377,18 +1501,19 @@
     cv.take((size_t)K * sizeof(unsigned long long));
     const size_t o_conf = cv.off;
     cv.take((size_t)K * sizeof(float));
-    if (cv.off > h->pc_arena_bytes) {
-        if (h->pc_arena) {
+    vk_handle::WorkSet &ws = h->sets[h->cur_set];
+    if (cv.off > ws.pc_arena_bytes) {
+        if (ws.pc_arena) {
             VK_CHECK_HIP(hipDeviceSynchronize());
-            VK_CHECK_HIP(hipFree(h->pc_arena));
-            h->pc_arena = nullptr;
-            h->pc_arena_bytes = 0;
-        }
-        VK_CHECK_HIP(hipMalloc((void **)&h->pc_arena, cv.off));
-        h->pc_arena_bytes = cv.off;
-    }
-    float *scores = (float *)(h->pc_arena + o_scores), *deltas = (float *)(h->pc_arena + o_deltas);
-    float *max_conf = (float *)(h->pc_arena + o_conf);
+            VK_CHECK_HIP(hipFree(ws.pc_arena));
+            ws.pc_arena = nullptr;
+            ws.pc_arena_bytes = 0;
+        }
+        VK_CHECK_HIP(hipMalloc((void **)&ws.pc_arena, cv.off));
+        ws.pc_arena_bytes = cv.off;
+    }
+    float *scores = (float *)(ws.pc_arena + o_scores), *deltas = (float *)(ws.pc_arena + o_deltas);
+    float *max_conf = (float *)(ws.pc_arena + o_conf);
 
     VK_TRY(launch_class_probs(p.cls_logits, ld_cls, K, C + 1, scores, ld_cls, s));
     ConvArgs g;
@@ -1430,7 +1555,7 @@
     a.score_thresh = sp->score_thresh;
     a.mind = sp->roi.min_detections;
     a.maxd = sp->roi.max_detections;
-    a.best = (unsigned long long *)(h->pc_arena + o_best);
+    a.best = (unsigned long long *)(ws.pc_arena + o_best);
     a.max_conf = max_conf;
     a.out = *out;
     a.keep_ids = p.keep_ids;
@@ -1493,14 +1618,14 @@
         VK_REQUIRE(image_hw[2 * n] >= 1 && image_hw[2 * n + 1] >= 1, VK_EINVAL, "forward: image_shapes[%d]=(%d,%d) must be positive",
                    n, image_hw[2 * n], image_hw[2 * n + 1]);
     VK_CHECK_HIP(hipSetDevice(h->device));
-    hipStream_t s = (hipStream_t)stream;
+    hipStream_t s = nullptr;
     const vk_config &c = h->cfg;
     const int D = rp->max_detections;
     TimerScope timer_scope(h->ktimer);
     const bool tm = h->timing;
 
     Plan p;
-    VK_TRY(fwd_open(h, N, H, W, c.post_nms_topk, D, image_hw, scales_yx, nullptr, ig, s, &p));
+    VK_TRY(fwd_open(h, N, H, W, c.post_nms_topk, D, image_hw, scales_yx, nullptr, ig, (hipStream_t)stream, &p, &s));
     const void *res4 = nullptr;
     VK_TRY(fwd_backbone(h, p, images_dev, s, &res4));
 
@@ -1596,6 +1721,7 @@
     if (B == 0) {
         h->stages_out.clear();
         h->ev_valid = false;
+        h->cur_caller = s;
         VK_CHECK_HIP(hipMemsetAsync(out->preds_per_image, 0, sizeof(int64_t) * (size_t)N, s));
         return fwd_close(h, nullptr, s, ticket);
     }
@@ -1603,7 +1729,7 @@
     const bool tm = h->timing;
 
     Plan p;
-    VK_TRY(fwd_open(h, N, H, W, B, B, image_hw, scales_yx, counts, nullptr, s, &p));
+    VK_TRY(fwd_open(h, N, H, W, B, B, image_hw, scales_yx, counts, nullptr, (hipStream_t)stream, &p, &s));
     const void *res4 = nullptr;
     VK_TRY(fwd_backbone(h, p, images_dev, s, &res4));
     if (tm) VK_CHECK_HIP(hipEventRecord(h->ev[2], s));
@@ -1629,6 +1755,7 @@
     const int slot = (int)(ticket % vk_handle::VK_MAX_INFLIGHT);
     h->oldest_open++;
     VK_CHECK_HIP(hipSetDevice(h->device));
+    if (h->slot_stream[slot] != h->slot_caller[slot]) VK_CHECK_HIP(hipStreamWaitEvent(h->slot_caller[slot], h->ev_done[slot], 0));
     VK_CHECK_HIP(hipEventSynchronize(h->ev_done[slot]));
     if (h->ktimer) h->ktimer->collect();
     VK_REQUIRE(h->flag_host[slot] == 0, VK_ENONFINITE, "Box tensor contains infinite or NaN!");
diff --git a/vltk_amd/frcnn.py b/vltk_amd/frcnn.py
--- a/vltk_amd/frcnn.py
+++ b/vltk_amd/frcnn.py
@@ -349,6 +349,11 @@
 
     def set_option(self, key, value):
         L.call("vk_set_option", self._h, key.encode(), int(value))
+
+    def get_option(self, key):
+        v = C.c_int()
+        L.call("vk_get_option", self._h, key.encode(), C.byref(v))
+        return v.value
 
     def enable_stage_timing(self, on=True):
         L.call("vk_enable_stage_timing", self._h, int(on))
diff --git a/vltk_amd/pipeline.py b/vltk_amd/pipeline.py
--- a/vltk_amd/pipeline.py
+++ b/vltk_amd/pipeline.py
@@ -115,6 +115,8 @@
         if self.world > 1:
             gbuf = [torch.empty(self.world * nbytes, dtype=torch.uint8, device=dev) for _ in range(self.depth)]
         on_gpu = dev.type == "cuda"
+        if on_gpu and hasattr(self.model, "set_option"):
+            self.model.set_option("forward_lanes", 1)
         copy_stream = torch.cuda.Stream(device=dev) if on_gpu else None
         upload_stream = torch.cuda.Stream(device=dev) if on_gpu else None
 
```
